# GrafikXxxxxxxYyyyyyyyyyy/StableDiffusion

Hardware: AMD Instinct MI355X
Metric: denoise-loop latents/s (512px, 50-step DDIM, batch 4) (higher is better)
Workload: dtype f16; 1 GPU; SD1.5 512x512, 50-step DDIM, batch 4/GPU, CFG on (UNet batch 8), UNet + VAE decode HIP kernels; global_batch=4, parallelism=dp1

## Files before the change

### include/sd_engine.h

```cpp
#ifndef SD_ENGINE_H
#define SD_ENGINE_H

#include <stdint.h>

#ifdef __cplusplus
extern "C" {
#endif

#define SD_OK 0
#define SD_ERR_INVALID 1
#define SD_ERR_STATE 2
#define SD_ERR_HIP 3
#define SD_ERR_UNSUPPORTED 4

#define SD_DTYPE_F16 0
#define SD_DTYPE_F32 1

#define SD_MAX_BLOCKS 4

typedef struct sd_unet_config {
    int32_t in_channels;
    int32_t out_channels;
    int32_t num_blocks;
    int32_t block_out_channels[SD_MAX_BLOCKS];
    int32_t down_block_has_attn[SD_MAX_BLOCKS];
    int32_t up_block_has_attn[SD_MAX_BLOCKS];
    int32_t num_heads[SD_MAX_BLOCKS];
    int32_t transformer_layers[SD_MAX_BLOCKS];
    int32_t layers_per_block;
    int32_t cross_attention_dim;
    int32_t use_linear_projection;
    int32_t norm_num_groups;
    float   norm_eps;
    int32_t flip_sin_to_cos;
    float   freq_shift;
    int32_t addition_time_embed_dim;
    int32_t projection_class_embeddings_input_dim;
} sd_unet_config;

typedef struct sd_vae_config {
    int32_t in_channels;
    int32_t out_channels;
    int32_t latent_channels;
    int32_t num_blocks;
    int32_t block_out_channels[SD_MAX_BLOCKS];
    int32_t layers_per_block;
    int32_t norm_num_groups;
} sd_vae_config;

typedef struct sd_clip_config {
    int32_t vocab_size;
    int32_t hidden_size;
    int32_t intermediate_size;
    int32_t num_layers;
    int32_t num_heads;
    int32_t max_positions;
    int32_t hidden_act;
    int32_t projection_dim;
    float layer_norm_eps;
} sd_clip_config;

typedef struct sd_unet sd_unet;
typedef struct sd_vae sd_vae;
typedef struct sd_clip sd_clip;
typedef struct sd_ip_adapter sd_ip_adapter;
typedef struct sd_controlnet sd_controlnet;

const char* sd_last_error(void);
int sd_engine_version(void);
const char* sd_engine_arch(void);

int sd_unet_create(const sd_unet_config* cfg, sd_unet** out);
int sd_unet_destroy(sd_unet* u);
int sd_unet_num_weights(const sd_unet* u);
int sd_unet_weight_info(const sd_unet* u, int index, const char** key, int64_t* shape4, int* ndim);
int sd_unet_set_weight(sd_unet* u, const char* diffusers_key, const void* data,
                       const int64_t* shape, int ndim, int dtype);
int sd_unet_finalize(sd_unet* u);
int sd_unet_forward(sd_unet* u, const void* sample, const float* timesteps, const void* ehs,
                    int ehs_len, const void* add_text, const float* add_time_ids, void* out,
                    int B, int H, int W, void* stream);
int sd_unet_use_graph(sd_unet* u, int enable);
int sd_unet_text_kv_cache(sd_unet* u, int enable);
int sd_unet_forward_ex(sd_unet* u, const void* sample, const float* timesteps, const void* ehs, int ehs_len,
                       const void* add_text, const float* add_time_ids, const void* image_embeds, int n_img, void* out,
                       int B, int H, int W, void* stream);
int sd_unet_set_ip_adapter(sd_unet* u, sd_ip_adapter* adapter);
int sd_unet_set_ip_adapter_scale(sd_unet* u, float scale);
int sd_unet_set_controlnet(sd_unet* u, sd_controlnet* cn);
int sd_unet_forward_cn(sd_unet* u, const void* sample, const float* timesteps, const void* ehs, int ehs_len,
                       const void* add_text, const float* add_time_ids, const void* image_embeds, int n_img,
                       const void* control_image, int n_ctrl, float cond_scale, void* out, int B, int H, int W,
                       void* stream);
int sd_unet_memory(const sd_unet* u, int64_t* weight_bytes, int64_t* workspace_bytes);

int sd_ip_adapter_create(const sd_unet* u, int image_embed_dim, int num_tokens, sd_ip_adapter** out);
int sd_ip_adapter_destroy(sd_ip_adapter* a);
int sd_ip_adapter_num_weights(const sd_ip_adapter* a);
int sd_ip_adapter_weight_info(const sd_ip_adapter* a, int index, const char** key, int64_t* shape4, int* ndim);
int sd_ip_adapter_set_weight(sd_ip_adapter* a, const char* key, const void* data, const int64_t* shape, int ndim,
                             int dtype);
int sd_ip_adapter_finalize(sd_ip_adapter* a);

int sd_controlnet_create(const sd_unet* u, const sd_unet_config* cn_cfg, int conditioning_channels, sd_controlnet** out);
int sd_controlnet_destroy(sd_controlnet* cn);
int sd_controlnet_num_weights(const sd_controlnet* cn);
int sd_controlnet_weight_info(const sd_controlnet* cn, int index, const char** key, int64_t* shape4, int* ndim);
int sd_controlnet_set_weight(sd_controlnet* cn, const char* key, const void* data, const int64_t* shape, int ndim,
                             int dtype);
int sd_controlnet_finalize(sd_controlnet* cn);

int sd_vae_create(const sd_vae_config* cfg, sd_vae** out);
int sd_vae_destroy(sd_vae* v);
int sd_vae_num_weights(const sd_vae* v);
int sd_vae_weight_info(const sd_vae* v, int index, const char** key, int64_t* shape4, int* ndim);
int sd_vae_set_weight(sd_vae* v, const char* diffusers_key, const void* data,
                      const int64_t* shape, int ndim, int dtype);
int sd_vae_finalize(sd_vae* v);
int sd_vae_decode(sd_vae* v, const void* z, void* img, int B, int h, int w, void* stream);
int sd_vae_encode(sd_vae* v, const void* img, void* moments, int B, int H, int W, void* stream);
int sd_vae_encode_range_shift(sd_vae* v, int shift);
int sd_vae_memory(const sd_vae* v, int64_t* weight_bytes, int64_t* workspace_bytes);

int sd_clip_create(const sd_clip_config* cfg, sd_clip** out);
int sd_clip_destroy(sd_clip* c);
int sd_clip_num_weights(const sd_clip* c);
int sd_clip_weight_info(const sd_clip* c, int index, const char** key, int64_t* shape4, int* ndim);
int sd_clip_set_weight(sd_clip* c, const char* key, const void* data, const int64_t* shape, int ndim, int dtype);
int sd_clip_finalize(sd_clip* c);
int sd_clip_forward(sd_clip* c, const int32_t* input_ids, const int32_t* eos_index, void* hidden_states,
                    void* last_hidden, void* pooled, void* text_embeds, int B, int T, void* stream);
int sd_clip_final_layer_norm(sd_clip* c, const void* x, void* y, int64_t rows, void* stream);
int sd_clip_memory(const sd_clip* c, int64_t* weight_bytes, int64_t* workspace_bytes);

int sd_cfg_duplicate(const void* latents, void* out2b, int64_t n_per_batch, int B, float in_scale,
                     void* stream);
int sd_cfg_ddim_step(const void* noise_pred_2b, void* latents, int64_t n, float guidance_scale,
                     float c_x, float c_eps, void* stream);

int sd_cfg_linear_step(const void* noise_pred_2b, void* latents, float* hist_f32, int64_t n,
                       float guidance_scale, float c_x, float c_eps, float c_hist, float h_x, float h_eps,
                       void* stream);

int sd_cfg_rescale_linear_step(const void* noise_pred_2b, void* latents, float* hist_f32, int B, int64_t n_per_sample,
                               float guidance_scale, float guidance_rescale, float c_x, float c_eps, float c_hist,
                               float h_x, float h_eps, float* factors_out, void* stream);

int sd_inpaint_blend(void* latents, const void* image_latents, const void* noise, const void* mask,
                     float a, float b, int B, int C, int H, int W, void* stream);

int sd_images_to_uint8(const void* images_nchw_f16, void* out_nhwc_u8, int B, int C, int H, int W, void* stream);

typedef struct sd_prof_entry {
    char kernel[64];
    double flops;
    double bytes;
    double ms;
    int64_t launches;
} sd_prof_entry;
int sd_prof_enable(int on);
int sd_prof_collect(sd_prof_entry* out, int max_entries, int* n_entries);

int sd_probe_mfma(int iters, float* tflops, void* stream);
int sd_probe_copy(int64_t bytes, int iters, float* gbs, void* stream);
int sd_probe_lds_dma(int64_t region_bytes, int passes, int depth, int shared, float* gbs, void* stream);

int sd_igemm_force(int variant, int splits);
int sd_igemm_plan(const int* geom, const int* flags, int64_t* out, char* name);

int sd_op_conv2d(const void* x_nhwc, const void* w_oihw, const void* bias, const void* rowadd,
                 const void* res_nhwc, void* y_nhwc, int N, int H, int W, int Cin, int Cout,
                 int ksize, int stride, int upsample2x, int geglu, void* stream);
int sd_op_conv3x3_small_cout(const void* x_nhwc, const void* w_oihw, const void* bias, void* y_nchw, int N, int H,
                             int W, int Cin, int Cout, void* stream);
int sd_op_conv2d_groupnorm(const void* x_nhwc, const void* w_oihw, const void* bias, const void* rowadd,
                           const void* res_nhwc, void* y_conv_nhwc, const void* gamma, const void* beta,
                           void* y_gn_nhwc, int N, int H, int W, int Cin, int Cout, int ksize, int stride,
                           int upsample2x, int groups, float eps, int silu, int* stats_from_epilogue, void* stream);
int sd_op_groupnorm_conv2d(const void* x_nhwc, const void* gamma, const void* beta, int groups, float eps, int silu,
                           const void* w_oihw, const void* bias, const void* rowadd, const void* res_nhwc, void* y_nhwc,
                           int N, int H, int W, int Cin, int Cout, int ksize, int iters, float* ms_per_launch, int* fused,
                           void* stream);
int sd_op_unet_conv_in(const void* x_nchw, const void* w_oihw, const void* bias, void* y_nhwc, float* gn_summaries, int groups,
                       int N, int Cin, int H, int W, int Cout, int iters, float* ms_per_launch, void* stream);
int sd_op_unet_conv_out(const void* x_nhwc, const void* gamma, const void* beta, int groups, float eps, int silu,
                        const void* w_oihw, const void* bias, void* y_nchw, int N, int H, int W, int C, int Cout, int iters,
                        float* ms_per_launch, void* stream);
int sd_op_ffn_geglu(const void* x, const void* ln_gamma, const void* ln_beta, float ln_eps, const void* w1, const void* b1,
                    const void* w2, const void* b2, void* y, int M, int C, int iters, float* ms_per_launch, int* fused,
                    void* stream);
int sd_op_linear_rowstats(const void* x, const void* w0, const void* b0, const void* res, void* y1, float* stat, int M,
                          int K, int C, int* parts, int* part_w, int* producer, void* stream);
int sd_op_ln_linear(const void* y1, const float* stat, int parts, int part_w, const void* gamma, const void* beta, float eps,
                    const void* w1, const void* b1, void* y2, int M, int C, int O, int geglu, int rows_scaled, float row_scale,
                    int* consumer, void* stream);
int sd_op_ln_ffn_geglu(const void* x, const float* stat, int parts, int part_w, const void* ln_gamma, const void* ln_beta,
                       float ln_eps, const void* w1, const void* b1, const void* w2, const void* b2, void* y, int M, int C,
                       int* fused, void* stream);
int sd_bench_conv2d(const void* x_nhwc, const void* w_oihw, void* y_nhwc, int N, int H, int W, int Cin,
                    int Cout, int ksize, int stride, int upsample2x, int geglu, int iters,
                    float* ms_per_launch, void* stream);
int sd_op_groupnorm(const void* x_nhwc, const void* gamma, const void* beta, void* y_nhwc,
                    int N, int HW, int C, int groups, float eps, int silu, void* stream);
int sd_op_groupnorm_concat(const void* x_nhwc, int Ca, int Cb, const void* gamma, const void* beta, void* y_nhwc, int N, int HW,
                           int groups, float eps, int silu, void* stream);
int sd_bench_groupnorm(const void* x_nhwc, const void* gamma, const void* beta, void* y_nhwc,
                       int N, int HW, int C, int groups, float eps, int silu, int iters,
                       float* ms_per_launch, void* stream);
int sd_op_timestep_sinusoid(const float* t, float* out, int count, int dim, int flip_sin_to_cos, float freq_shift,
                            void* stream);
int sd_op_small_linear(const float* x, const void* w_f16, const float* bias, float* y, int B, int K, int n_out,
                       int silu_in, int silu_out, void* stream);
int sd_op_layernorm(const void* x, const void* gamma, const void* beta, void* y, int rows, int C,
                    float eps, void* stream);
int sd_op_attention(const void* q, const void* k, const void* v, void* out, int B, int Tq, int Tk,
                    int heads, int d, int ldq, int ldk, int ldv, int ldo, void* stream);
int sd_op_attention_ex(const void* q, const void* k, const void* v, void* out, int B, int Tq, int Tk,
                       int heads, int d, int ldq, int ldk, int ldv, int ldo, int causal, int prescaled,
                       void* stream);
int sd_attention_plan(int B, int Tq, int Tk, int heads, int d, int causal, int prescaled, int* out5);
int sd_op_ip_cross_attention(const void* q, const void* k, const void* v, const void* k_ip, const void* v_ip, void* out,
                             int B, int Tq, int L, int T_ip, int heads, int d, int ldq, int ldk, int ldv, int ldk_ip,
                             int ldv_ip, int ldo, float ip_scale, int prescaled, int iters, float* ms_per_launch,
                             void* stream);

typedef struct sd_cn_problem {
    const void* x; int64_t ldx;
    const void* w;
    const float* bias;
    void* y; int64_t ldy;
    int M, C;
} sd_cn_problem;
int sd_op_controlnet_residuals(const sd_cn_problem* problems, int count, float scale, int mode, int iters,
                               float* ms_per_launch, void* stream);
int sd_op_controlnet_cond_embed(sd_controlnet* cn, const void* image, int n, int H, int W, void* out, int iters,
                                float* ms_per_launch, void* stream);

#ifdef __cplusplus
}
#endif
#endif
```

### stablediffusion_amd/_lib.py

```python
from __future__ import annotations

import ctypes as C
import os

_HERE = os.path.dirname(os.path.abspath(__file__))
LIB_PATH = os.path.join(_HERE, "libsd_engine.so")

SD_MAX_BLOCKS = 4
SD_DTYPE_F16 = 0
SD_DTYPE_F32 = 1


class SdUNetConfig(C.Structure):
    _fields_ = [
        ("in_channels", C.c_int32),
        ("out_channels", C.c_int32),
        ("num_blocks", C.c_int32),
        ("block_out_channels", C.c_int32 * SD_MAX_BLOCKS),
        ("down_block_has_attn", C.c_int32 * SD_MAX_BLOCKS),
        ("up_block_has_attn", C.c_int32 * SD_MAX_BLOCKS),
        ("num_heads", C.c_int32 * SD_MAX_BLOCKS),
        ("transformer_layers", C.c_int32 * SD_MAX_BLOCKS),
        ("layers_per_block", C.c_int32),
        ("cross_attention_dim", C.c_int32),
        ("use_linear_projection", C.c_int32),
        ("norm_num_groups", C.c_int32),
        ("norm_eps", C.c_float),
        ("flip_sin_to_cos", C.c_int32),
        ("freq_shift", C.c_float),
        ("addition_time_embed_dim", C.c_int32),
        ("projection_class_embeddings_input_dim", C.c_int32),
    ]


class SdVAEConfig(C.Structure):
    _fields_ = [
        ("in_channels", C.c_int32),
        ("out_channels", C.c_int32),
        ("latent_channels", C.c_int32),
        ("num_blocks", C.c_int32),
        ("block_out_channels", C.c_int32 * SD_MAX_BLOCKS),
        ("layers_per_block", C.c_int32),
        ("norm_num_groups", C.c_int32),
    ]


class SdClipConfig(C.Structure):
    _fields_ = [
        ("vocab_size", C.c_int32),
        ("hidden_size", C.c_int32),
        ("intermediate_size", C.c_int32),
        ("num_layers", C.c_int32),
        ("num_heads", C.c_int32),
        ("max_positions", C.c_int32),
        ("hidden_act", C.c_int32),
        ("projection_dim", C.c_int32),
        ("layer_norm_eps", C.c_float),
    ]


class SdProfEntry(C.Structure):
    _fields_ = [("kernel", C.c_char * 64), ("flops", C.c_double), ("bytes", C.c_double),
                ("ms", C.c_double), ("launches", C.c_int64)]


class SdCnProblem(C.Structure):
    _fields_ = [("x", C.c_void_p), ("ldx", C.c_int64), ("w", C.c_void_p), ("bias", C.c_void_p),
                ("y", C.c_void_p), ("ldy", C.c_int64), ("M", C.c_int), ("C", C.c_int)]


_P = C.c_void_p
_I = C.c_int
_I64 = C.c_int64
_F = C.c_float
SIGNATURES = {
    "sd_last_error": (C.c_char_p, []),
    "sd_engine_version": (_I, []),
    "sd_engine_arch": (C.c_char_p, []),
    "sd_unet_create": (_I, [C.POINTER(SdUNetConfig), C.POINTER(_P)]),
    "sd_unet_destroy": (_I, [_P]),
    "sd_unet_num_weights": (_I, [_P]),
    "sd_unet_weight_info": (_I, [_P, _I, C.POINTER(C.c_char_p), C.POINTER(_I64), C.POINTER(_I)]),
    "sd_unet_set_weight": (_I, [_P, C.c_char_p, _P, C.POINTER(_I64), _I, _I]),
    "sd_unet_finalize": (_I, [_P]),
    "sd_unet_forward": (_I, [_P, _P, _P, _P, _I, _P, _P, _P, _I, _I, _I, _P]),
    "sd_unet_use_graph": (_I, [_P, _I]),
    "sd_unet_text_kv_cache": (_I, [_P, _I]),
    "sd_unet_memory": (_I, [_P, C.POINTER(_I64), C.POINTER(_I64)]),
    "sd_unet_forward_ex": (_I, [_P, _P, _P, _P, _I, _P, _P, _P, _I, _P, _I, _I, _I, _P]),
    "sd_unet_set_ip_adapter": (_I, [_P, _P]),
    "sd_unet_set_ip_adapter_scale": (_I, [_P, _F]),
    "sd_ip_adapter_create": (_I, [_P, _I, _I, C.POINTER(_P)]),
    "sd_ip_adapter_destroy": (_I, [_P]),
    "sd_ip_adapter_num_weights": (_I, [_P]),
    "sd_ip_adapter_weight_info": (_I, [_P, _I, C.POINTER(C.c_char_p), C.POINTER(_I64), C.POINTER(_I)]),
    "sd_ip_adapter_set_weight": (_I, [_P, C.c_char_p, _P, C.POINTER(_I64), _I, _I]),
    "sd_ip_adapter_finalize": (_I, [_P]),
    "sd_unet_set_controlnet": (_I, [_P, _P]),
    "sd_unet_forward_cn": (_I, [_P, _P, _P, _P, _I, _P, _P, _P, _I, _P, _I, _F, _P, _I, _I, _I, _P]),
    "sd_controlnet_create": (_I, [_P, C.POINTER(SdUNetConfig), _I, C.POINTER(_P)]),
    "sd_controlnet_destroy": (_I, [_P]),
    "sd_controlnet_num_weights": (_I, [_P]),
    "sd_controlnet_weight_info": (_I, [_P, _I, C.POINTER(C.c_char_p), C.POINTER(_I64), C.POINTER(_I)]),
    "sd_controlnet_set_weight": (_I, [_P, C.c_char_p, _P, C.POINTER(_I64), _I, _I]),
    "sd_controlnet_finalize": (_I, [_P]),
    "sd_vae_create": (_I, [C.POINTER(SdVAEConfig), C.POINTER(_P)]),
    "sd_vae_destroy": (_I, [_P]),
    "sd_vae_num_weights": (_I, [_P]),
    "sd_vae_weight_info": (_I, [_P, _I, C.POINTER(C.c_char_p), C.POINTER(_I64), C.POINTER(_I)]),
    "sd_vae_set_weight": (_I, [_P, C.c_char_p, _P, C.POINTER(_I64), _I, _I]),
    "sd_vae_finalize": (_I, [_P]),
    "sd_vae_decode": (_I, [_P, _P, _P, _I, _I, _I, _P]),
    "sd_vae_encode": (_I, [_P, _P, _P, _I, _I, _I, _P]),
    "sd_vae_encode_range_shift": (_I, [_P, _I]),
    "sd_vae_memory": (_I, [_P, C.POINTER(_I64), C.POINTER(_I64)]),
    "sd_clip_create": (_I, [C.POINTER(SdClipConfig), C.POINTER(_P)]),
    "sd_clip_destroy": (_I, [_P]),
    "sd_clip_num_weights": (_I, [_P]),
    "sd_clip_weight_info": (_I, [_P, _I, C.POINTER(C.c_char_p), C.POINTER(_I64), C.POINTER(_I)]),
    "sd_clip_set_weight": (_I, [_P, C.c_char_p, _P, C.POINTER(_I64), _I, _I]),
    "sd_clip_finalize": (_I, [_P]),
    "sd_clip_forward": (_I, [_P, _P, _P, _P, _P, _P, _P, _I, _I, _P]),
    "sd_clip_final_layer_norm": (_I, [_P, _P, _P, _I64, _P]),
    "sd_clip_memory": (_I, [_P, C.POINTER(_I64), C.POINTER(_I64)]),
    "sd_op_attention_ex": (_I, [_P, _P, _P, _P, _I, _I, _I, _I, _I, _I, _I, _I, _I, _I, _I, _P]),
    "sd_cfg_duplicate": (_I, [_P, _P, _I64, _I, _F, _P]),
    "sd_cfg_ddim_step": (_I, [_P, _P, _I64, _F, _F, _F, _P]),
    "sd_inpaint_blend": (_I, [_P, _P, _P, _P, _F, _F, _I, _I, _I, _I, _P]),
    "sd_images_to_uint8": (_I, [_P, _P, _I, _I, _I, _I, _P]),
    "sd_cfg_linear_step": (_I, [_P, _P, _P, _I64, _F, _F, _F, _F, _F, _F, _P]),
    "sd_cfg_rescale_linear_step": (_I, [_P, _P, _P, _I, _I64, _F, _F, _F, _F, _F, _F, _F, _P, _P]),
    "sd_igemm_force": (_I, [_I, _I]),
    "sd_igemm_plan": (_I, [C.POINTER(_I), C.POINTER(_I), C.POINTER(_I64), C.c_char_p]),
    "sd_probe_mfma": (_I, [_I, C.POINTER(_F), _P]),
    "sd_probe_lds_dma": (_I, [_I64, _I, _I, _I, C.POINTER(_F), _P]),
    "sd_probe_copy": (_I, [_I64, _I, C.POINTER(_F), _P]),
    "sd_prof_enable": (_I, [_I]),
    "sd_prof_collect": (_I, [C.POINTER(SdProfEntry), _I, C.POINTER(_I)]),
    "sd_op_conv2d": (_I, [_P, _P, _P, _P, _P, _P, _I, _I, _I, _I, _I, _I, _I, _I, _I, _P]),
    "sd_op_conv3x3_small_cout": (_I, [_P, _P, _P, _P, _I, _I, _I, _I, _I, _P]),
    "sd_op_conv2d_groupnorm": (_I, [_P, _P, _P, _P, _P, _P, _P, _P, _P, _I, _I, _I, _I, _I, _I, _I, _I, _I, _F, _I,
                                    C.POINTER(_I), _P]),
    "sd_op_groupnorm_conv2d": (_I, [_P, _P, _P, _I, _F, _I, _P, _P, _P, _P, _P, _I, _I, _I, _I, _I, _I, _I, C.POINTER(_F),
                                    C.POINTER(_I), _P]),
    "sd_op_unet_conv_in": (_I, [_P, _P, _P, _P, _P, _I, _I, _I, _I, _I, _I, _I, C.POINTER(_F), _P]),
    "sd_op_unet_conv_out": (_I, [_P, _P, _P, _I, _F, _I, _P, _P, _P, _I, _I, _I, _I, _I, _I, C.POINTER(_F), _P]),
    "sd_op_ffn_geglu": (_I, [_P, _P, _P, _F, _P, _P, _P, _P, _P, _I, _I, _I, C.POINTER(_F), C.POINTER(_I), _P]),
    "sd_op_linear_rowstats": (_I, [_P, _P, _P, _P, _P, _P, _I, _I, _I, C.POINTER(_I), C.POINTER(_I), C.POINTER(_I), _P]),
    "sd_op_ln_linear": (_I, [_P, _P, _I, _I, _P, _P, _F, _P, _P, _P, _I, _I, _I, _I, _I, _F, C.POINTER(_I), _P]),
    "sd_op_ln_ffn_geglu": (_I, [_P, _P, _I, _I, _P, _P, _F, _P, _P, _P, _P, _P, _I, _I, C.POINTER(_I), _P]),
    "sd_bench_conv2d": (_I, [_P, _P, _P, _I, _I, _I, _I, _I, _I, _I, _I, _I, _I, C.POINTER(_F), _P]),
    "sd_op_groupnorm": (_I, [_P, _P, _P, _P, _I, _I, _I, _I, _F, _I, _P]),
    "sd_op_groupnorm_concat": (_I, [_P, _I, _I, _P, _P, _P, _I, _I, _I, _F, _I, _P]),
    "sd_bench_groupnorm": (_I, [_P, _P, _P, _P, _I, _I, _I, _I, _F, _I, _I, C.POINTER(_F), _P]),
    "sd_op_timestep_sinusoid": (_I, [_P, _P, _I, _I, _I, _F, _P]),
    "sd_op_small_linear": (_I, [_P, _P, _P, _P, _I, _I, _I, _I, _I, _P]),
    "sd_op_layernorm": (_I, [_P, _P, _P, _P, _I, _I, _F, _P]),
    "sd_op_attention": (_I, [_P, _P, _P, _P, _I, _I, _I, _I, _I, _I, _I, _I, _I, _P]),
    "sd_attention_plan": (_I, [_I, _I, _I, _I, _I, _I, _I, C.POINTER(_I)]),
    "sd_op_ip_cross_attention": (_I, [_P, _P, _P, _P, _P, _P, _I, _I, _I, _I, _I, _I, _I, _I, _I, _I, _I, _I, _F, _I, _I,
                                      C.POINTER(_F), _P]),
    "sd_op_controlnet_residuals": (_I, [C.POINTER(SdCnProblem), _I, _F, _I, _I, C.POINTER(_F), _P]),
    "sd_op_controlnet_cond_embed": (_I, [_P, _P, _I, _I, _I, _P, _I, C.POINTER(_F), _P]),
}

_lib = None


class EngineError(RuntimeError):
    pass


def load():
    global _lib
    if _lib is not None:
        return _lib
    if not os.path.exists(LIB_PATH):
        raise EngineError(
            f"{LIB_PATH} not found: build it with `python -m stablediffusion_amd.build` "
            "(hipcc --offload-arch=gfx950). The HIP engine is mandatory; there is no CPU fallback.")
    import torch
    lib = C.CDLL(LIB_PATH)
    for name, (res, args) in SIGNATURES.items():
        fn = getattr(lib, name)
        fn.restype = res
        fn.argtypes = args
    _lib = lib
    return lib


def check(rc: int, what: str = ""):
    if rc != 0:
        msg = load().sd_last_error()
        raise EngineError(f"{what}: error {rc}: {msg.decode() if msg else '?'}")


def require_gpu():
    import torch
    if not torch.cuda.is_available():
        raise EngineError("no HIP device visible: the gfx950 engine cannot run (and nothing else will run in its place)")
```

### stablediffusion_amd/csrc/capi.cpp

```cpp
#include <cstdio>
#include <new>

#include "model.h"
#include <cstdlib>

using namespace sd;

struct sd_unet { UNet impl; explicit sd_unet(const sd_unet_config& c) : impl(c) {} };
struct sd_vae { VAE impl; explicit sd_vae(const sd_vae_config& c) : impl(c) {} };
struct sd_clip { CLIP impl; explicit sd_clip(const sd_clip_config& c) : impl(c) {} };
struct sd_controlnet {
    ControlNet impl;
    sd_controlnet(const sd_unet_config& c, int cc) : impl(c, cc) {}
};
struct sd_ip_adapter {
    IPAdapter impl;
    sd_ip_adapter(const sd_unet_config& c, int d, int n) : impl(c, d, n) {}
    ~sd_ip_adapter() { if (impl.attached) impl.attached->set_ip_adapter(nullptr); }
};

namespace {

int weight_info(const WeightStore& ws, int index, const char** key, int64_t* shape4, int* ndim) {
    if (index < 0 || index >= (int)ws.order.size()) { set_error("weight index out of range"); return SD_ERR_INVALID; }
// ... 2 lines not shown
    *key = k.c_str();
    *ndim = (int)t.shape.size();
    for (int i = 0; i < 4; ++i) shape4[i] = i < *ndim ? t.shape[(size_t)i] : 1;
    return SD_OK;
}

bool bad_cfg(const sd_unet_config* c) {
    if (!c || c->num_blocks < 1 || c->num_blocks > SD_MAX_BLOCKS) return true;
    for (int i = 0; i < c->num_blocks; ++i) {
        if (c->block_out_channels[i] % 64 != 0 || c->block_out_channels[i] % c->norm_num_groups != 0) return true;
        if (c->num_heads[i] <= 0 || c->block_out_channels[i] % c->num_heads[i] != 0) return true;
        if ((c->down_block_has_attn[i] || c->up_block_has_attn[c->num_blocks - 1 - i]) &&
            !attention_supported(c->block_out_channels[i] / c->num_heads[i])) return true;
    }
    if (c->addition_time_embed_dim > 0) {
        const int ad = c->addition_time_embed_dim, pin = c->projection_class_embeddings_input_dim;
        if ((ad & 1) || pin % 64 != 0 || pin - 6 * ad <= 0) return true;
    }
    return c->cross_attention_dim % 64 != 0 || c->in_channels <= 0 || c->in_channels > 16;
}

bool same_topology(const sd_unet_config& a, const sd_unet_config& b) {
    if (a.in_channels != b.in_channels || a.out_channels != b.out_channels || a.num_blocks != b.num_blocks ||
        a.layers_per_block != b.layers_per_block || a.cross_attention_dim != b.cross_attention_dim ||
        a.use_linear_projection != b.use_linear_projection || a.norm_num_groups != b.norm_num_groups ||
        a.norm_eps != b.norm_eps || a.flip_sin_to_cos != b.flip_sin_to_cos || a.freq_shift != b.freq_shift ||
        a.addition_time_embed_dim != b.addition_time_embed_dim ||
        a.projection_class_embeddings_input_dim != b.projection_class_embeddings_input_dim)
        return false;
    for (int i = 0; i < SD_MAX_BLOCKS; ++i)
        if (a.block_out_channels[i] != b.block_out_channels[i] || a.down_block_has_attn[i] != b.down_block_has_attn[i] ||
            a.up_block_has_attn[i] != b.up_block_has_attn[i] || a.num_heads[i] != b.num_heads[i] ||
            a.transformer_layers[i] != b.transformer_layers[i])
            return false;
    return true;
}

bool controlnet_fits(const sd_unet_config& u, const sd_unet_config& n, std::string* why) {
    if (n.num_blocks != u.num_blocks || n.layers_per_block != u.layers_per_block) {
        *why = "num_blocks / layers_per_block differ from the UNet's";
        return false;
    }
    for (int i = 0; i < u.num_blocks; ++i)
        if (n.block_out_channels[i] != u.block_out_channels[i]) { *why = "block_out_channels differ from the UNet's"; return false; }
    if (n.cross_attention_dim != u.cross_attention_dim) { *why = "cross_attention_dim differs from the UNet's"; return false; }
    if (n.in_channels != u.in_channels) { *why = "in_channels differs from the UNet's (9-channel inpaint UNets take no ControlNet)"; return false; }
    if (n.addition_time_embed_dim != u.addition_time_embed_dim ||
        n.projection_class_embeddings_input_dim != u.projection_class_embeddings_input_dim) {
        *why = "text_time conditioning differs from the UNet's";
        return false;
    }
    return true;
}

}

extern "C" {

const char* sd_last_error(void) { return sd::last_error().c_str(); }
int sd_engine_version(void) { return 1; }
const char* sd_engine_arch(void) { return "gfx950"; }

int sd_unet_create(const sd_unet_config* cfg, sd_unet** out) {
    if (!out) { set_error("null out"); return SD_ERR_INVALID; }
    if (bad_cfg(cfg)) {
        set_error("sd_unet_create: unsupported config (channels must be multiples of 64 and of the group "
                  "count, head dims in {32,40,64,80,128,160}, cross_attention_dim % 64 == 0, text_time: even "
                  "addition_time_embed_dim and projection_class_embeddings_input_dim % 64 == 0 and > 6 x it)");
        return SD_ERR_UNSUPPORTED;
    }
    *out = new (std::nothrow) sd_unet(*cfg);
    if (!*out) { set_error("out of host memory"); return SD_ERR_INVALID; }
    return SD_OK;
}
int sd_unet_destroy(sd_unet* u) { delete u; return SD_OK; }
int sd_unet_num_weights(const sd_unet* u) { return u ? (int)u->impl.ws.order.size() : 0; }
int sd_unet_weight_info(const sd_unet* u, int index, const char** key, int64_t* shape4, int* ndim) {
    if (!u) { set_error("null handle"); return SD_ERR_INVALID; }
    return weight_info(u->impl.ws, index, key, shape4, ndim);
}
int sd_unet_set_weight(sd_unet* u, const char* key, const void* data, const int64_t* shape, int ndim, int dtype) {
    if (!u || !key || !data || !shape) { set_error("null argument"); return SD_ERR_INVALID; }
    if (u->impl.finalized) { set_error("set_weight after finalize"); return SD_ERR_STATE; }
    return u->impl.ws.set(key, data, shape, ndim, dtype);
}
int sd_unet_finalize(sd_unet* u) {
    if (!u) { set_error("null handle"); return SD_ERR_INVALID; }
    return u->impl.finalize();
}
int sd_unet_forward(sd_unet* u, const void* sample, const float* timesteps, const void* ehs, int ehs_len,
                    const void* add_text, const float* add_time_ids, void* out, int B, int H, int W,
                    void* stream) {
    if (!u || !sample || !timesteps || !ehs || !out) { set_error("null argument"); return SD_ERR_INVALID; }
    return u->impl.forward(static_cast<const half_t*>(sample), timesteps, static_cast<const half_t*>(ehs),
                           ehs_len, static_cast<const half_t*>(add_text), add_time_ids,
                           static_cast<half_t*>(out), B, H, W, static_cast<hipStream_t>(stream));
}
int sd_unet_use_graph(sd_unet* u, int enable) {
    if (!u) { set_error("null handle"); return SD_ERR_INVALID; }
    u->impl.graph_enabled = enable != 0;
    return SD_OK;
}
int sd_unet_text_kv_cache(sd_unet* u, int enable) {
    if (!u) { set_error("null handle"); return SD_ERR_INVALID; }
    u->impl.kv_cache_on = enable != 0;
    u->impl.kv_valid = false;
    u->impl.ipkv_valid = false;
    u->impl.cond_valid = false;
    u->impl.cnkv_valid = false;
    return SD_OK;
}
int sd_unet_forward_ex(sd_unet* u, const void* sample, const float* timesteps, const void* ehs, int ehs_len,
                       const void* add_text, const float* add_time_ids, const void* image_embeds, int n_img, void* out,
                       int B, int H, int W, void* stream) {
    if (!u || !sample || !timesteps || !ehs || !out) { set_error("null argument"); return SD_ERR_INVALID; }
    return u->impl.forward(static_cast<const half_t*>(sample), timesteps, static_cast<const half_t*>(ehs),
                           ehs_len, static_cast<const half_t*>(add_text), add_time_ids,
                           static_cast<half_t*>(out), B, H, W, static_cast<hipStream_t>(stream),
                           static_cast<const half_t*>(image_embeds), image_embeds ? n_img : 0);
}
int sd_unet_set_ip_adapter(sd_unet* u, sd_ip_adapter* a) {
    if (!u) { set_error("null handle"); return SD_ERR_INVALID; }
    if (a) {
        if (!a->impl.finalized) { set_error("sd_unet_set_ip_adapter: adapter not finalized"); return SD_ERR_STATE; }
        if (!same_topology(a->impl.cfg, u->impl.cfg)) {
            set_error("sd_unet_set_ip_adapter: the adapter was created for another UNet configuration");
            return SD_ERR_INVALID;
        }
    }
    u->impl.set_ip_adapter(a ? &a->impl : nullptr);
    return SD_OK;
}
int sd_unet_set_controlnet(sd_unet* u, sd_controlnet* cn) {
    if (!u) { set_error("null handle"); return SD_ERR_INVALID; }
    if (cn) {
        if (!cn->impl.finalized) { set_error("sd_unet_set_controlnet: ControlNet not finalized"); return SD_ERR_STATE; }
        std::string why;
        if (!controlnet_fits(u->impl.cfg, cn->impl.cfg, &why)) { set_error("sd_unet_set_controlnet: " + why); return SD_ERR_INVALID; }
    }
    u->impl.set_controlnet(cn ? &cn->impl : nullptr);
    return SD_OK;
}
int sd_unet_forward_cn(sd_unet* u, const void* sample, const float* timesteps, const void* ehs, int ehs_len,
                       const void* add_text, const float* add_time_ids, const void* image_embeds, int n_img,
                       const void* control_image, int n_ctrl, float cond_scale, void* out, int B, int H, int W,
                       void* stream) {
    if (!u || !sample || !timesteps || !ehs || !out) { set_error("null argument"); return SD_ERR_INVALID; }
    return u->impl.forward(static_cast<const half_t*>(sample), timesteps, static_cast<const half_t*>(ehs),
                           ehs_len, static_cast<const half_t*>(add_text), add_time_ids,
                           static_cast<half_t*>(out), B, H, W, static_cast<hipStream_t>(stream),
                           static_cast<const half_t*>(image_embeds), image_embeds ? n_img : 0,
                           static_cast<const half_t*>(control_image), control_image ? n_ctrl : 0, cond_scale);
}
int sd_unet_set_ip_adapter_scale(sd_unet* u, float scale) {
    if (!u) { set_error("null handle"); return SD_ERR_INVALID; }
    if (!(scale == scale)) { set_error("sd_unet_set_ip_adapter_scale: NaN"); return SD_ERR_INVALID; }
    u->impl.ip_scale = scale;
    return SD_OK;
}

int sd_ip_adapter_create(const sd_unet* u, int image_embed_dim, int num_tokens, sd_ip_adapter** out) {
    if (!u || !out) { set_error("null argument"); return SD_ERR_INVALID; }
    const sd_unet_config& c = u->impl.cfg;
    if (c.cross_attention_dim % 64 != 0) { set_error("sd_ip_adapter_create: cross_attention_dim % 64 != 0"); return SD_ERR_UNSUPPORTED; }
    if (num_tokens < 1 || num_tokens > 16) { set_error("sd_ip_adapter_create: num_tokens must be in [1, 16]"); return SD_ERR_UNSUPPORTED; }
    if (image_embed_dim <= 0 || image_embed_dim % 64 != 0) {
        set_error("sd_ip_adapter_create: image_embed_dim must be a positive multiple of 64");
        return SD_ERR_UNSUPPORTED;
    }
    for (const auto& site : unet_xattn_sites(c, true)) {
        int heads = 0;
        for (int i = 0; i < c.num_blocks; ++i)
            if (c.block_out_channels[i] == site.second) heads = c.num_heads[i];
        if (heads <= 0 || !ip_attention_supported(site.second / heads)) {
            set_error("sd_ip_adapter_create: head dim of " + site.first + " not in {32, 40, 64, 80, 160}");
            return SD_ERR_UNSUPPORTED;
        }
    }
    *out = new (std::nothrow) sd_ip_adapter(c, image_embed_dim, num_tokens);
    if (!*out) { set_error("out of host memory"); return SD_ERR_INVALID; }
    return SD_OK;
}
int sd_ip_adapter_destroy(sd_ip_adapter* a) { delete a; return SD_OK; }
int sd_ip_adapter_num_weights(const sd_ip_adapter* a) { return a ? (int)a->impl.ws.order.size() : 0; }
int sd_ip_adapter_weight_info(const sd_ip_adapter* a, int index, const char** key, int64_t* shape4, int* ndim) {
    if (!a) { set_error("null handle"); return SD_ERR_INVALID; }
    return weight_info(a->impl.ws, index, key, shape4, ndim);
}
int sd_ip_adapter_set_weight(sd_ip_adapter* a, const char* key, const void* data, const int64_t* shape, int ndim,
                             int dtype) {
    if (!a || !key || !data || !shape) { set_error("null argument"); return SD_ERR_INVALID; }
    if (a->impl.finalized) { set_error("set_weight after finalize"); return SD_ERR_STATE; }
    return a->impl.ws.set(key, data, shape, ndim, dtype);
}
int sd_ip_adapter_finalize(sd_ip_adapter* a) {
    if (!a) { set_error("null handle"); return SD_ERR_INVALID; }
    return a->impl.finalize();
}
int sd_controlnet_create(const sd_unet* u, const sd_unet_config* cn_cfg, int conditioning_channels, sd_controlnet** out) {
    if (!u || !cn_cfg || !out) { set_error("null argument"); return SD_ERR_INVALID; }
    if (conditioning_channels != 3) { set_error("sd_controlnet_create: conditioning_channels must be 3"); return SD_ERR_UNSUPPORTED; }
    sd_unet_config c = *cn_cfg;
    for (int i = 0; i < SD_MAX_BLOCKS; ++i) c.up_block_has_attn[i] = 0;
    if (bad_cfg(&c)) { set_error("sd_controlnet_create: unsupported encoder configuration"); return SD_ERR_UNSUPPORTED; }
    std::string why;
    if (!controlnet_fits(u->impl.cfg, c, &why)) { set_error("sd_controlnet_create: " + why); return SD_ERR_INVALID; }
    if (u->impl.cfg.in_channels != 4) { set_error("sd_controlnet_create: the UNet must take 4 latent channels"); return SD_ERR_INVALID; }
    if (1 + c.num_blocks * c.layers_per_block + (c.num_blocks - 1) + 1 > kCnMaxProblems) {
        set_error("sd_controlnet_create: more residual sites than one grouped launch takes (16)");
        return SD_ERR_UNSUPPORTED;
    }
    *out = new (std::nothrow) sd_controlnet(c, conditioning_channels);
    if (!*out) { set_error("out of host memory"); return SD_ERR_INVALID; }
    return SD_OK;
}
int sd_controlnet_destroy(sd_controlnet* cn) { delete cn; return SD_OK; }
int sd_controlnet_num_weights(const sd_controlnet* cn) { return cn ? (int)cn->impl.ws.order.size() : 0; }
int sd_controlnet_weight_info(const sd_controlnet* cn, int index, const char** key, int64_t* shape4, int* ndim) {
    if (!cn) { set_error("null handle"); return SD_ERR_INVALID; }
    return weight_info(cn->impl.ws, index, key, shape4, ndim);
}
int sd_controlnet_set_weight(sd_controlnet* cn, const char* key, const void* data, const int64_t* shape, int ndim,
                             int dtype) {
    if (!cn || !key || !data || !shape) { set_error("null argument"); return SD_ERR_INVALID; }
    if (cn->impl.finalized) { set_error("set_weight after finalize"); return SD_ERR_STATE; }
    return cn->impl.ws.set(key, data, shape, ndim, dtype);
}
int sd_controlnet_finalize(sd_controlnet* cn) {
    if (!cn) { set_error("null handle"); return SD_ERR_INVALID; }
    return cn->impl.finalize();
}
int sd_unet_memory(const sd_unet* u, int64_t* weight_bytes, int64_t* workspace_bytes) {
    if (!u) { set_error("null handle"); return SD_ERR_INVALID; }
    if (weight_bytes) *weight_bytes = u->impl.ws.packed_bytes();
    if (workspace_bytes) *workspace_bytes = (int64_t)u->impl.arena.capacity();
    return SD_OK;
}

int sd_vae_create(const sd_vae_config* cfg, sd_vae** out) {
    if (!out || !cfg) { set_error("null argument"); return SD_ERR_INVALID; }
    bool bad = cfg->num_blocks < 1 || cfg->num_blocks > SD_MAX_BLOCKS || cfg->latent_channels > 8;
    for (int i = 0; !bad && i < cfg->num_blocks; ++i)
        bad = cfg->block_out_channels[i] % 64 != 0;
    if (!bad) bad = !attention_supported(cfg->block_out_channels[cfg->num_blocks - 1]);
    if (bad) { set_error("sd_vae_create: unsupported config"); return SD_ERR_UNSUPPORTED; }
    *out = new (std::nothrow) sd_vae(*cfg);
    if (!*out) { set_error("out of host memory"); return SD_ERR_INVALID; }
    return SD_OK;
}
int sd_vae_destroy(sd_vae* v) { delete v; return SD_OK; }
int sd_vae_num_weights(const sd_vae* v) { return v ? (int)v->impl.ws.order.size() : 0; }
int sd_vae_weight_info(const sd_vae* v, int index, const char** key, int64_t* shape4, int* ndim) {
    if (!v) { set_error("null handle"); return SD_ERR_INVALID; }
    return weight_info(v->impl.ws, index, key, shape4, ndim);
}
int sd_vae_set_weight(sd_vae* v, const char* key, const void* data, const int64_t* shape, int ndim, int dtype) {
    if (!v || !key || !data || !shape) { set_error("null argument"); return SD_ERR_INVALID; }
    if (v->impl.finalized) { set_error("set_weight after finalize"); return SD_ERR_STATE; }
    return v->impl.ws.set(key, data, shape, ndim, dtype);
}
int sd_vae_finalize(sd_vae* v) {
    if (!v) { set_error("null handle"); return SD_ERR_INVALID; }
    return v->impl.finalize();
}
int sd_vae_decode(sd_vae* v, const void* z, void* img, int B, int h, int w, void* stream) {
    if (!v || !z || !img) { set_error("null argument"); return SD_ERR_INVALID; }
    return v->impl.decode(static_cast<const half_t*>(z), static_cast<half_t*>(img), B, h, w,
                          static_cast<hipStream_t>(stream));
}
int sd_vae_encode(sd_vae* v, const void* img, void* moments, int B, int H, int W, void* stream) {
    if (!v || !img || !moments) { set_error("null argument"); return SD_ERR_INVALID; }
    return v->impl.encode(static_cast<const half_t*>(img), static_cast<half_t*>(moments), B, H, W,
                          static_cast<hipStream_t>(stream));
}
int sd_vae_encode_range_shift(sd_vae* v, int shift) {
    if (!v || shift < 0 || shift > 14) { set_error("sd_vae_encode_range_shift: shift in 0..14"); return SD_ERR_INVALID; }
    v->impl.encode_shift = shift;
    return SD_OK;
}
int sd_vae_memory(const sd_vae* v, int64_t* weight_bytes, int64_t* workspace_bytes) {
    if (!v) { set_error("null handle"); return SD_ERR_INVALID; }
    if (weight_bytes) *weight_bytes = v->impl.ws.packed_bytes();
    if (workspace_bytes) *workspace_bytes = (int64_t)v->impl.arena.capacity();
    return SD_OK;
}

int sd_clip_create(const sd_clip_config* cfg, sd_clip** out) {
    if (!out || !cfg) { set_error("null argument"); return SD_ERR_INVALID; }
    const bool bad = cfg->vocab_size < 1 || cfg->num_layers < 1 || cfg->num_heads < 1 || cfg->max_positions < 1 ||
                     cfg->hidden_size % 64 != 0 || cfg->intermediate_size % 64 != 0 || cfg->hidden_size > 2048 ||
                     cfg->hidden_size % cfg->num_heads != 0 || !attention_supported(cfg->hidden_size / cfg->num_heads) ||
                     (cfg->hidden_act != 0 && cfg->hidden_act != 1) || cfg->projection_dim < 0;
    if (bad) { set_error("sd_clip_create: unsupported config (hidden / intermediate % 64, head dim, activation)"); return SD_ERR_UNSUPPORTED; }
    *out = new (std::nothrow) sd_clip(*cfg);
    if (!*out) { set_error("out of host memory"); return SD_ERR_INVALID; }
    return SD_OK;
}
int sd_clip_destroy(sd_clip* c) { delete c; return SD_OK; }
int sd_clip_num_weights(const sd_clip* c) { return c ? (int)c->impl.ws.order.size() : 0; }
int sd_clip_weight_info(const sd_clip* c, int index, const char** key, int64_t* shape4, int* ndim) {
    if (!c) { set_error("null handle"); return SD_ERR_INVALID; }
    return weight_info(c->impl.ws, index, key, shape4, ndim);
}
int sd_clip_set_weight(sd_clip* c, const char* key, const void* data, const int64_t* shape, int ndim, int dtype) {
    if (!c || !key || !data || !shape) { set_error("null argument"); return SD_ERR_INVALID; }
    if (c->impl.finalized) { set_error("set_weight after finalize"); return SD_ERR_STATE; }
// ... 911 lines not shown
```

### stablediffusion_amd/csrc/kernels.h

```cpp
#pragma once
#include "common.h"

namespace sd {

struct IGemmParams {
    const half_t* x; long ldx;
    const half_t* w;
    const float* bias;
    const float* rowadd; int rowadd_ld;
    const half_t* res; long ldres;
    half_t* y; long ldy;
    int N, H, W, Cin;
    int OH, OW, Cout;
    int KS, stride, pad, up;
    int M, K;
    int geglu;
    int mfast = 0;
    int act = 0;
    float* rowstat_out = nullptr;
    int rowstat_parts = 0;
    const float* ln_stat = nullptr;
    int ln_parts = 0, ln_C = 0, ln_part_w = 0;
    float ln_eps = 0.f;
    const float* ln_wsum = nullptr;
// ... 8 lines not shown
    const float* gni_gb = nullptr;
    int dbg_unchecked = 0;
    float acc_scale = 1.f, bias_scale = 1.f;
};
bool igemm2_gn_fusable(const IGemmParams& p, int groups);
int launch_igemm(const IGemmParams& p, hipStream_t s);
const char* igemm_variant(const IGemmParams& p);
bool igemm2_supported(const IGemmParams& p);
void igemm2_force(int variant, int splits);
struct IGemmRequest {
    float* rowstat = nullptr;
    float* gnstat = nullptr;
    int gn_groups = 0;
    bool no_workspace = false;
};
constexpr int kKindPgemmGeglu = 100;
constexpr int kKindIgemm1 = -1;
constexpr int kKindBadVariant = -2;
struct IGemmPlan {
    int kind = kKindIgemm1;
    int variant = -1;
    int splits = 1;
    long partial_floats = 0;
    int bm = 0, bn = 0;
    bool rowstats = false;
    int rs_parts = 1, rs_part_w = 0;
    bool gnstats = false;
    int gn_rows = 0;
    bool scales_ok = false;
    char name[64] = "";
};
IGemmPlan igemm2_plan(IGemmParams& p, const IGemmRequest& rq = IGemmRequest());
int launch_igemm2(const IGemmParams& p, float* partial, hipStream_t s, const IGemmPlan* plan = nullptr);
bool igemm3_supported(const IGemmParams& p);
int launch_igemm3(const IGemmParams& p, int mfast, hipStream_t s);
constexpr int kWeightRowPad = 256;
bool wsgemm_supported(const IGemmParams& p);
int wsgemm_rowstat_parts(const IGemmParams& p);
int launch_wsgemm(const IGemmParams& p, hipStream_t s);
bool pgemm_geglu_supported(const IGemmParams& p);
int launch_pgemm_geglu(const IGemmParams& p, hipStream_t s);

struct FfnParams {
    const half_t* x; long ldx;
    half_t* y; long ldy;
    const half_t* w1; const float* b1; const float* wsum1; int w1_rows;
    const half_t* w2; const float* b2; int w2_rows;
    const float* ln_stat; int ln_parts; float ln_eps;
    int M, C, hidden;
    int ln_part_w;
};
bool ffn_fused_supported(const FfnParams& p);
int launch_ffn_fused(const FfnParams& p, hipStream_t s);

long gn_scratch_floats(int N, long HW, int C, int G);
struct GnStats {
    const float* part = nullptr;
    int S = 0;
    long rows = 0;
};
bool gn_wants_stats(long HW, int C, int G);
int launch_groupnorm(const half_t* x, long ldx, const float* gamma, const float* beta,
                     half_t* y, long ldy, int N, long HW, int C, int G, float eps, int silu,
                     float* scratch, hipStream_t s, const GnStats* pre = nullptr);
int launch_gn_stats(const half_t* x, long ldx, int N, long HW, int C, int G, float* scratch, GnStats* st, hipStream_t s);
int launch_gn_finalize(GnStats* st, float* out, int N, long HW, int C, int G, hipStream_t s);
int gn_cat_unit(int Ca, int Cb, int G);
int launch_gn_cat_finalize(const GnStats& sa, int Ga, int Ca, const GnStats& sb, int Gb, int Cb, float* out, int N, long HW, int G,
                           hipStream_t s);
int launch_layernorm(const half_t* x, long ldx, const float* gamma, const float* beta,
                     half_t* y, long ldy, long rows, int C, float eps, hipStream_t s);
int launch_row_stats(const half_t* x, long ldx, float* stat, long rows, int C, hipStream_t s);
int launch_ln_fold(half_t* w, long K, int rows, const float* gamma, const float* beta, const float* bias_in,
                   float* bias, float* wsum, int rows_scaled, float row_scale, hipStream_t s);

int launch_attention(const half_t* q, const half_t* k, const half_t* v, half_t* out,
                     int B, int Tq, int Tk, int heads, int d,
                     long ldq, long ldk, long ldv, long ldo, hipStream_t s, int causal = 0, int prescaled = 0);
bool attention_supported(int d);
struct AttnPlan { int D, QT, KT, PRESC, NWV; };
AttnPlan attention_plan(int B, int Tq, int Tk, int heads, int d, int causal, int prescaled);
int launch_ip_attention(const half_t* q, const half_t* k, const half_t* v, const half_t* kip, const half_t* vip,
                        half_t* out, int B, int Tq, int L, int Tip, int heads, int d, long ldq, long ldk, long ldv,
                        long ldki, long ldvi, long ldo, float ip_scale, int prescaled, hipStream_t s);
bool ip_attention_supported(int d);
int launch_axpy_f16(half_t* y, long ldy, const half_t* x, long ldx, long rows, int cols, float a, hipStream_t s);

constexpr int kCnMaxProblems = 16;
struct CnResProblem {
    const half_t* x = nullptr; long ldx = 0;
    const half_t* w = nullptr;
    const float* bias = nullptr;
    half_t* y = nullptr; long ldy = 0;
    int M = 0, C = 0;
    int first = 0;
};
struct CnResParams {
    CnResProblem p[kCnMaxProblems];
    int count = 0, total = 0;
    float scale = 1.f;
};
int cn_residual_tiles(int M, int C);
bool cn_residual_supported(const CnResParams& p);
int launch_cn_residual(const CnResParams& p, hipStream_t s);
struct CnCondConvParams {
    const half_t* x = nullptr; int nchw = 0;
    const float* w = nullptr; const float* bias = nullptr;
    half_t* y = nullptr;
    int N = 0, IH = 0, IW = 0, Cin = 0, OH = 0, OW = 0, Cout = 0, stride = 1, silu = 1;
};
bool cn_cond_conv_supported(const CnCondConvParams& p);
int launch_cn_cond_conv(const CnCondConvParams& p, hipStream_t s);
int launch_cn_pack_cond(const half_t* w_oihw, float* out, int O, int I, hipStream_t s);

int launch_timestep_sinusoid(const float* t, int t_stride, float* out, int count, int dim, int flip, float shift,
                             long out_ld, hipStream_t s);
int launch_small_linear(const float* x, long ldx, const half_t* w, const float* bias, float* y,
                        long ldy, int B, int K, int Nout, int silu_in, int silu_out, hipStream_t s);
int launch_add_f32(float* y, const float* x, long n, int silu, hipStream_t s);
int launch_f16_to_f32(const half_t* x, float* y, long n, hipStream_t s);
int launch_f32_to_f16(const float* x, half_t* y, long n, hipStream_t s);
int launch_im2col_nchw3x3(const half_t* x, half_t* col, int N, int C, int H, int W, int Kpad,
                          hipStream_t s);
int launch_nhwc_to_nchw(const half_t* x, long ldx, half_t* y, int N, long HW, int C, hipStream_t s);
int launch_nchw_to_nhwc(const half_t* x, half_t* y, long ldy, int N, long HW, int C, hipStream_t s);
int launch_pointwise_nchw(const half_t* x, const half_t* w, const float* bias, half_t* y, int N,
                          int Cin, int Cout, long HW, hipStream_t s);
constexpr long kSmallCoutMinPixels = 131072;
int launch_conv3x3_small_cout(const half_t* x, long ldx, const half_t* w, long K, const float* bias, half_t* y_nchw,
                              int N, int H, int W, int Cin, int Cout, hipStream_t s);
struct HeadParams {
    const half_t* x_nchw = nullptr;
    const half_t* w = nullptr; long K = 0;
    const float* bias = nullptr;
    half_t* y = nullptr; long ldy = 0;
    float* gnstat_out = nullptr; int G = 0;
    int N = 0, Cin = 0, H = 0, W = 0, Cout = 0;
};
bool conv_head_supported(const HeadParams& p);
int launch_conv_head(const HeadParams& p, hipStream_t s);
struct TailParams {
    const half_t* x = nullptr; long ldx = 0;
    const float* gn_part = nullptr; int gn_S = 0; long gn_rows = 0;
    int G = 0; float eps = 0.f; const float* gamma = nullptr; const float* beta = nullptr; int silu = 0;
    const half_t* w = nullptr; long K = 0; const float* bias = nullptr;
    half_t* y = nullptr;
    int N = 0, H = 0, W = 0, C = 0, Cout = 0;
};
bool conv_tail_supported(const TailParams& p);
int launch_conv_tail(const TailParams& p, hipStream_t s);
int launch_pack_conv(const half_t* w_oihw, half_t* wp, int O, int I, int KH, int KW, long Kpad,
                     hipStream_t s);
int launch_cfg_duplicate(const half_t* lat, half_t* out, long n_total, float scale, hipStream_t s);
int launch_clip_embed(const int* ids, const half_t* tok, const half_t* pos, half_t* out, int B, int T, int H, int vocab,
                      hipStream_t s);
int launch_gather_rows(const half_t* x, long ldx, const int* idx, half_t* out16, float* out32, int B, int T, int H,
                       hipStream_t s);
int launch_inpaint_blend(half_t* lat, const half_t* img, const half_t* noise, const half_t* mask, float a, float b, int B,
                         int C, long HW, hipStream_t s);
int launch_scale_f16(half_t* x, long n, float scale, hipStream_t s);
int launch_image_to_uint8(const half_t* img, unsigned char* out, int B, int C, long HW, hipStream_t s);
int launch_cfg_linear(const half_t* eps2b, half_t* lat, float* hist, long n, float g, float cx, float ce, float ch,
                      float hx, float he, hipStream_t s);
int launch_cfg_ddim(const half_t* eps2b, half_t* lat, long n, float g, float cx, float ce,
                    hipStream_t s);
int launch_cfg_rescale_linear(const half_t* eps2b, half_t* lat, float* hist, int B, long n, float g, float phi, float cx,
                              float ce, float ch, float hx, float he, float* factors, hipStream_t s);

int probe_mfma(int iters, float* tflops, hipStream_t s);
int probe_copy(long bytes, int iters, float* gbs, hipStream_t s);
int probe_dma(long region_bytes, int passes, int depth, int shared, float* gbs, hipStream_t s);

}
```

### stablediffusion_amd/csrc/misc.hip

```cpp
#include <cstdint>
#include <cstdlib>
#include <map>
#include <mutex>
#include <utility>

#include "kernels.h"

namespace sd {
namespace {

__global__ void sinusoid_kernel(const float* __restrict__ t, int t_stride, float* __restrict__ out, int count,
                                int dim, int flip, float shift, long out_ld) {
    const int half = dim >> 1;
    const int i = blockIdx.x * blockDim.x + threadIdx.x;
    if (i >= count * half) return;
    const int b = i / half, f = i - b * half;
    const float freq = __expf(-9.210340371976184f * (float)f / ((float)half - shift));
    const float ang = t[(long)b * t_stride] * freq;
    float sn, cs;
    sincosf(ang, &sn, &cs);
    float* o = out + (long)b * out_ld;
    if (flip) { o[f] = cs; o[half + f] = sn; } else { o[f] = sn; o[half + f] = cs; }
}

// ... 4 lines not shown
                                                           const float* __restrict__ bias,
                                                           float* __restrict__ y, long ldy, int B,
                                                           int K, int Nout, int silu_in, int silu_out) {
    const int lane = threadIdx.x & 63;
    const int n0 = (blockIdx.x * 4 + (threadIdx.x >> 6)) * SL_COLS;
    if (n0 >= Nout) return;
    for (int b0 = 0; b0 < B; b0 += SL_MAXB) {
        float acc[SL_COLS][SL_MAXB];
#pragma unroll
        for (int c = 0; c < SL_COLS; ++c)
#pragma unroll
            for (int b = 0; b < SL_MAXB; ++b) acc[c][b] = 0.f;
        for (int k0 = lane * 8; k0 < K; k0 += 64 * 8) {
            h8 wv[SL_COLS];
#pragma unroll
            for (int c = 0; c < SL_COLS; ++c) {
                const int n = n0 + c < Nout ? n0 + c : Nout - 1;
                wv[c] = *reinterpret_cast<const h8*>(w + (long)n * K + k0);
            }
#pragma unroll
            for (int b = 0; b < SL_MAXB; ++b) {
                if (b0 + b < B) {
                    const float* xr = x + (long)(b0 + b) * ldx + k0;
                    const f4 x0 = *reinterpret_cast<const f4*>(xr);
                    const f4 x1 = *reinterpret_cast<const f4*>(xr + 4);
                    float a[8];
#pragma unroll
                    for (int e = 0; e < 4; ++e) {
                        a[e] = silu_in ? silu_f(x0[e]) : x0[e];
                        a[e + 4] = silu_in ? silu_f(x1[e]) : x1[e];
                    }
#pragma unroll
                    for (int c = 0; c < SL_COLS; ++c)
#pragma unroll
                        for (int e = 0; e < 8; ++e) acc[c][b] += a[e] * (float)wv[c][e];
                }
            }
        }
#pragma unroll
        for (int c = 0; c < SL_COLS; ++c)
#pragma unroll
            for (int b = 0; b < SL_MAXB; ++b) {
                float a = acc[c][b];
#pragma unroll
                for (int off = 32; off > 0; off >>= 1) a += __shfl_xor(a, off);
                if (lane == 0 && b0 + b < B && n0 + c < Nout) {
                    a += bias ? bias[n0 + c] : 0.f;
                    if (silu_out) a = silu_f(a);
                    y[(long)(b0 + b) * ldy + n0 + c] = a;
                }
            }
    }
}

__global__ void add_f32_kernel(float* y, const float* x, long n, int silu) {
    const long i = (long)blockIdx.x * blockDim.x + threadIdx.x;
    if (i < n) {
        float v = y[i] + (x ? x[i] : 0.f);
        y[i] = silu ? silu_f(v) : v;
    }
}
__global__ void f16_to_f32_kernel(const half_t* x, float* y, long n) {
    const long i = (long)blockIdx.x * blockDim.x + threadIdx.x;
    if (i < n) y[i] = (float)x[i];
}
__global__ void f32_to_f16_kernel(const float* x, half_t* y, long n) {
    const long i = (long)blockIdx.x * blockDim.x + threadIdx.x;
    if (i < n) y[i] = (half_t)x[i];
}

__global__ void im2col_nchw3x3_kernel(const half_t* __restrict__ x, half_t* __restrict__ col, int N,
                                      int C, int H, int W, int Kpad) {
    const long i = (long)blockIdx.x * blockDim.x + threadIdx.x;
    const long total = (long)N * H * W * Kpad;
    if (i >= total) return;
    const int kq = (int)(i % Kpad);
    const long m = i / Kpad;
    half_t val = (half_t)0.f;
    if (kq < 9 * C) {
        const int tap = kq / C, c = kq - tap * C;
        const int kh = tap / 3, kw = tap - kh * 3;
        const int w_ = (int)(m % W);
        const int h_ = (int)((m / W) % H);
        const int n = (int)(m / ((long)W * H));
        const int ih = h_ + kh - 1, iw = w_ + kw - 1;
        if (ih >= 0 && ih < H && iw >= 0 && iw < W) val = x[(((long)n * C + c) * H + ih) * W + iw];
    }
    col[i] = val;
}

__global__ void nhwc_to_nchw_kernel(const half_t* __restrict__ x, long ldx, half_t* __restrict__ y,
                                    int N, long HW, int C) {
    const long i = (long)blockIdx.x * blockDim.x + threadIdx.x;
    if (i >= (long)N * C * HW) return;
    const long pix = i % HW;
    const int c = (int)((i / HW) % C);
    const long n = i / (HW * C);
    y[i] = x[(n * HW + pix) * ldx + c];
}

__global__ void nchw_to_nhwc_kernel(const half_t* __restrict__ x, half_t* __restrict__ y, long ldy,
                                    int N, long HW, int C) {
    const long i = (long)blockIdx.x * blockDim.x + threadIdx.x;
    if (i >= (long)N * C * HW) return;
    const int c = (int)(i % C);
    const long pix = (i / C) % HW;
    const long n = i / (HW * C);
    y[(n * HW + pix) * ldy + c] = x[(n * C + c) * HW + pix];
}

__global__ void pointwise_nchw_kernel(const half_t* __restrict__ x, const half_t* __restrict__ w,
                                      const float* __restrict__ bias, half_t* __restrict__ y, int N,
                                      int Cin, int Cout, long HW) {
    const long i = (long)blockIdx.x * blockDim.x + threadIdx.x;
    if (i >= (long)N * Cout * HW) return;
    const long pix = i % HW;
    const int co = (int)((i / HW) % Cout);
    const long n = i / (HW * Cout);
    float acc = bias ? bias[co] : 0.f;
    for (int ci = 0; ci < Cin; ++ci)
        acc += (float)x[(n * Cin + ci) * HW + pix] * (float)w[co * Cin + ci];
    y[i] = (half_t)acc;
}

__global__ void pack_conv_kernel(const half_t* __restrict__ w, half_t* __restrict__ wp, int O, int I,
                                 int KH, int KW, long Kpad) {
    const long i = (long)blockIdx.x * blockDim.x + threadIdx.x;
    if (i >= (long)O * Kpad) return;
    const long kq = i % Kpad;
    const long o = i / Kpad;
    half_t val = (half_t)0.f;
    if (kq < (long)KH * KW * I) {
        int ci, tap;
        if (I % 64 == 0) {
            const int slab = (int)(kq >> 6), cl = (int)(kq & 63);
            const int cs = slab / (KH * KW);
            tap = slab - cs * (KH * KW);
            ci = cs * 64 + cl;
        } else {
            ci = (int)(kq % I);
            tap = (int)(kq / I);
        }
        const int kh = tap / KW, kw = tap - kh * KW;
        val = w[((o * I + ci) * KH + kh) * KW + kw];
    }
    wp[i] = val;
}

__global__ void cfg_duplicate_kernel(const half_t* __restrict__ lat, half_t* __restrict__ out, long n,
                                     float scale) {
    const long i = (long)blockIdx.x * blockDim.x + threadIdx.x;
    if (i >= n) return;
    const half_t v = (half_t)((float)lat[i] * scale);
    out[i] = v;
    out[n + i] = v;
}
__global__ void cfg_ddim_kernel(const half_t* __restrict__ eps2b, half_t* __restrict__ lat, long n,
                                float g, float cx, float ce) {
    const long i = (long)blockIdx.x * blockDim.x + threadIdx.x;
    if (i >= n) return;
    const float eu = (float)eps2b[i], et = (float)eps2b[n + i];
    const float e = (float)(half_t)(g * (et - eu) + eu);
    lat[i] = (half_t)(cx * (float)lat[i] + ce * e);
}

__global__ void cfg_linear_kernel(const half_t* __restrict__ eps2b, half_t* __restrict__ lat,
                                  float* __restrict__ hist, long n, float g, float cx, float ce, float ch,
                                  float hx, float he) {
    const long i = (long)blockIdx.x * blockDim.x + threadIdx.x;
    if (i >= n) return;
    const float eu = (float)eps2b[i], et = (float)eps2b[n + i];
    const float e = (float)(half_t)(g * (et - eu) + eu);
    const float x = (float)lat[i];
    float out = cx * x + ce * e;
    if (hist) {
        out += ch * hist[i];
        hist[i] = hx * x + he * e;
    }
    lat[i] = (half_t)out;
}

constexpr int RS_MAX_PARTS = 64;
constexpr int RS_MIN_CHUNK = 2048;

struct RsStat { float n, mean, m2; };

__device__ __forceinline__ RsStat rs_merge(const RsStat a, const RsStat b) {
    RsStat r;
    r.n = a.n + b.n;
    const float d = b.mean - a.mean;
    const float w = r.n > 0.f ? b.n / r.n : 0.f;
    r.mean = a.mean + d * w;
    r.m2 = a.m2 + b.m2 + d * d * a.n * w;
    return r;
}
__device__ __forceinline__ RsStat rs_wave_merge(RsStat s) {
#pragma unroll
    for (int off = 1; off < 64; off <<= 1) {
        RsStat o;
        o.n = __shfl_xor(s.n, off);
        o.mean = __shfl_xor(s.mean, off);
        o.m2 = __shfl_xor(s.m2, off);
        s = (threadIdx.x & off) ? rs_merge(o, s) : rs_merge(s, o);
    }
    return s;
}
__device__ __forceinline__ float rs_cfg(float eu, float et, float g) { return (float)(half_t)(g * (et - eu) + eu); }
__device__ __forceinline__ float rs_axpby(float a, float x, float b, float e) { return __builtin_fmaf(a, x, b * e); }

template <bool VEC>
__global__ __launch_bounds__(256) void rs_stats_kernel(const half_t* __restrict__ eps2b, RsStat* __restrict__ part, long n,
                                                       long chunk, long total, float g) {
    const int b = blockIdx.y, p = blockIdx.x;
    const half_t* u = eps2b + (long)b * n;
    const half_t* t = u + total;
    const long lo = (long)p * chunk, hi = lo + chunk < n ? lo + chunk : n;
    RsStat st = {0.f, 0.f, 0.f}, se = {0.f, 0.f, 0.f};
    if (VEC) {
        for (long i = lo + (long)threadIdx.x * 8; i < hi; i += 256 * 8) {
            const h8 vu = *reinterpret_cast<const h8*>(u + i);
            const h8 vt = *reinterpret_cast<const h8*>(t + i);
            float ft[8], fe[8], sumt = 0.f, sume = 0.f;
#pragma unroll
            for (int k = 0; k < 8; ++k) {
                ft[k] = (float)vt[k];
                fe[k] = rs_cfg((float)vu[k], ft[k], g);
                sumt += ft[k];
                sume += fe[k];
            }
            RsStat vt8 = {8.f, sumt * 0.125f, 0.f}, ve8 = {8.f, sume * 0.125f, 0.f};
#pragma unroll
            for (int k = 0; k < 8; ++k) {
                const float dt = ft[k] - vt8.mean, de = fe[k] - ve8.mean;
                vt8.m2 += dt * dt;
                ve8.m2 += de * de;
            }
            st = rs_merge(st, vt8);
            se = rs_merge(se, ve8);
        }
    } else {
        for (long i = lo + threadIdx.x; i < hi; i += 256) {
            const float ft = (float)t[i];
            const RsStat a = {1.f, ft, 0.f}, c = {1.f, rs_cfg((float)u[i], ft, g), 0.f};
            st = rs_merge(st, a);
            se = rs_merge(se, c);
        }
    }
    st = rs_wave_merge(st);
    se = rs_wave_merge(se);
    __shared__ RsStat sh[4][2];
    const int wave = threadIdx.x >> 6;
    if ((threadIdx.x & 63) == 0) { sh[wave][0] = st; sh[wave][1] = se; }
    __syncthreads();
    if (threadIdx.x == 0) {
        RsStat* o = part + ((long)b * gridDim.x + p) * 2;
        o[0] = rs_merge(rs_merge(sh[0][0], sh[1][0]), rs_merge(sh[2][0], sh[3][0]));
        o[1] = rs_merge(rs_merge(sh[0][1], sh[1][1]), rs_merge(sh[2][1], sh[3][1]));
    }
}

template <bool VEC>
__global__ __launch_bounds__(256) void rs_apply_kernel(const half_t* __restrict__ eps2b, half_t* __restrict__ lat,
                                                       float* __restrict__ hist, const RsStat* __restrict__ part, int parts,
                                                       long n, long total, float g, float phi, float cx, float ce, float ch,
                                                       float hx, float he, float* __restrict__ factors) {
    const int b = blockIdx.y, lane = threadIdx.x & 63;
    RsStat st = {0.f, 0.f, 0.f}, se = {0.f, 0.f, 0.f};
    if (lane < parts) {
        const RsStat* q = part + ((long)b * parts + lane) * 2;
        st = q[0];
        se = q[1];
    }
    st = rs_wave_merge(st);
    se = rs_wave_merge(se);
    const float k = 1.f + phi * (sqrtf(st.m2 / se.m2) - 1.f);
    if (factors && blockIdx.x == 0 && threadIdx.x == 0) factors[b] = k;
    const long base = (long)b * n;
    const half_t* u = eps2b + base;
    const half_t* t = u + total;
    half_t* x = lat + base;
    float* h = hist ? hist + base : nullptr;
    if (VEC) {
        const long i = ((long)blockIdx.x * 256 + threadIdx.x) * 8;
        if (i >= n) return;
        const h8 vu = *reinterpret_cast<const h8*>(u + i);
        const h8 vt = *reinterpret_cast<const h8*>(t + i);
        const h8 vx = *reinterpret_cast<const h8*>(x + i);
        float hv[8], x0[8];
        if (h) {
            const f4 h0 = *reinterpret_cast<const f4*>(h + i), h1 = *reinterpret_cast<const f4*>(h + i + 4);
#pragma unroll
            for (int j = 0; j < 4; ++j) { hv[j] = h0[j]; hv[j + 4] = h1[j]; }
        }
        h8 o;
#pragma unroll
        for (int j = 0; j < 8; ++j) {
            const float e = k * rs_cfg((float)vu[j], (float)vt[j], g);
            const float xf = (float)vx[j];
            float out = rs_axpby(cx, xf, ce, e);
            if (h) {
                out = __builtin_fmaf(ch, hv[j], out);
                x0[j] = rs_axpby(hx, xf, he, e);
            }
            o[j] = (half_t)out;
        }
        *reinterpret_cast<h8*>(x + i) = o;
// ... 181 lines not shown
}

inline dim3 grid1d(long n, int block = 256) { return dim3((unsigned)((n + block - 1) / block)); }

}

int launch_timestep_sinusoid(const float* t, int t_stride, float* out, int count, int dim, int flip, float shift,
                             long out_ld, hipStream_t s) {
    hipLaunchKernelGGL(sinusoid_kernel, grid1d((long)count * (dim / 2)), dim3(256), 0, s, t, t_stride, out, count,
                       dim, flip, shift, out_ld);
    SD_HIP_CHECK(hipGetLastError());
    return 0;
}

constexpr int SK_MAXKS = 10;
__global__ __launch_bounds__(256) void skinny_linear_kernel(const float* __restrict__ x, long ldx, const half_t* __restrict__ w,
                                                            const float* __restrict__ bias, float* __restrict__ y, long ldy,
                                                            int B, int K, int Nout, int silu_in, int silu_out) {
    __shared__ float red[2][4][256];
    const int tid = threadIdx.x, lane = tid & 63, wave = tid >> 6;
    const int fr = lane & 15, fq = lane >> 4;
    const int KS = K / 32;
    const int tiles = Nout / 16;
    h8 xh[SK_MAXKS], xl[SK_MAXKS];
#pragma unroll
    for (int j = 0; j < SK_MAXKS; ++j) {
        const int ks = wave + 4 * j;
        h8 hi = {0, 0, 0, 0, 0, 0, 0, 0}, lo = {0, 0, 0, 0, 0, 0, 0, 0};
        if (ks < KS && fr < B) {
            const float* xr = x + (long)fr * ldx + ks * 32 + fq * 8;
            const f4 a = *reinterpret_cast<const f4*>(xr), b = *reinterpret_cast<const f4*>(xr + 4);
#pragma unroll
            for (int e = 0; e < 8; ++e) {
                float v = e < 4 ? a[e] : b[e - 4];
                if (silu_in) v = silu_f(v);
                hi[e] = (half_t)v;
                lo[e] = (half_t)(v - (float)hi[e]);
            }
        }
        xh[j] = hi; xl[j] = lo;
    }
    auto fetch = [&](int t, h8* wf) {
        const int tt = t < tiles ? t : tiles - 1;
        const half_t* wr = w + ((long)tt * 16 + fr) * K + fq * 8;
#pragma unroll
        for (int j = 0; j < SK_MAXKS; ++j) {
            const int ks = wave + 4 * j;
            wf[j] = *reinterpret_cast<const h8*>(wr + (ks < KS ? ks : KS - 1) * 32);
        }
    };
    h8 wcur[SK_MAXKS], wnext[SK_MAXKS];
    int t = blockIdx.x;
    fetch(t, wcur);
    int par = 0;
    for (; t < tiles; t += gridDim.x, par ^= 1) {
        fetch(t + gridDim.x, wnext);
        f4 acc = {0.f, 0.f, 0.f, 0.f};
#pragma unroll
        for (int j = 0; j < SK_MAXKS; ++j) {
            if (wave + 4 * j < KS) {
                acc = __builtin_amdgcn_mfma_f32_16x16x32_f16(wcur[j], xh[j], acc, 0, 0, 0);
                acc = __builtin_amdgcn_mfma_f32_16x16x32_f16(wcur[j], xl[j], acc, 0, 0, 0);
            }
        }
#pragma unroll
        for (int e = 0; e < 4; ++e) red[par][wave][(fq * 4 + e) * 16 + fr] = acc[e];
        __syncthreads();
        {
            const int col = tid >> 4, row = tid & 15;
            if (row < B) {
                float v = red[par][0][tid] + red[par][1][tid] + red[par][2][tid] + red[par][3][tid];
                v += bias ? bias[t * 16 + col] : 0.f;
                if (silu_out) v = silu_f(v);
                y[(long)row * ldy + t * 16 + col] = v;
            }
        }
#pragma unroll
        for (int j = 0; j < SK_MAXKS; ++j) wcur[j] = wnext[j];
    }
}

int launch_small_linear(const float* x, long ldx, const half_t* w, const float* bias, float* y, long ldy,
                        int B, int K, int Nout, int silu_in, int silu_out, hipStream_t s) {
    if (K % 8 != 0 || ldx % 4 != 0) { set_error("small_linear: K%8, ldx%4"); return 1; }
    static const bool no_skinny = getenv("SD_NO_SKINNY_LINEAR") != nullptr;
    if (!no_skinny && B <= 16 && K % 32 == 0 && K <= 4 * SK_MAXKS * 32 && Nout % 16 == 0) {
        const int tiles = Nout / 16;
        hipLaunchKernelGGL(skinny_linear_kernel, dim3(tiles < 512 ? tiles : 512), dim3(256), 0, s, x, ldx, w, bias, y, ldy, B, K, Nout,
                           silu_in, silu_out);
        SD_HIP_CHECK(hipGetLastError());
        return 0;
    }
    hipLaunchKernelGGL(small_linear_kernel, dim3(cdiv(Nout, 4 * SL_COLS)), dim3(256), 0, s, x, ldx, w, bias, y, ldy, B, K,
                       Nout, silu_in, silu_out);
    SD_HIP_CHECK(hipGetLastError());
    return 0;
}

int launch_add_f32(float* y, const float* x, long n, int silu, hipStream_t s) {
    hipLaunchKernelGGL(add_f32_kernel, grid1d(n), dim3(256), 0, s, y, x, n, silu);
    SD_HIP_CHECK(hipGetLastError());
    return 0;
}
int launch_f16_to_f32(const half_t* x, float* y, long n, hipStream_t s) {
    hipLaunchKernelGGL(f16_to_f32_kernel, grid1d(n), dim3(256), 0, s, x, y, n);
    SD_HIP_CHECK(hipGetLastError());
    return 0;
}
int launch_f32_to_f16(const float* x, half_t* y, long n, hipStream_t s) {
    hipLaunchKernelGGL(f32_to_f16_kernel, grid1d(n), dim3(256), 0, s, x, y, n);
    SD_HIP_CHECK(hipGetLastError());
    return 0;
}
int launch_im2col_nchw3x3(const half_t* x, half_t* col, int N, int C, int H, int W, int Kpad, hipStream_t s) {
    hipLaunchKernelGGL(im2col_nchw3x3_kernel, grid1d((long)N * H * W * Kpad), dim3(256), 0, s, x, col, N, C, H,
                       W, Kpad);
    SD_HIP_CHECK(hipGetLastError());
    return 0;
}
int launch_nhwc_to_nchw(const half_t* x, long ldx, half_t* y, int N, long HW, int C, hipStream_t s) {
    hipLaunchKernelGGL(nhwc_to_nchw_kernel, grid1d((long)N * C * HW), dim3(256), 0, s, x, ldx, y, N, HW, C);
    SD_HIP_CHECK(hipGetLastError());
    return 0;
}
int launch_nchw_to_nhwc(const half_t* x, half_t* y, long ldy, int N, long HW, int C, hipStream_t s) {
    hipLaunchKernelGGL(nchw_to_nhwc_kernel, grid1d((long)N * C * HW), dim3(256), 0, s, x, y, ldy, N, HW, C);
    SD_HIP_CHECK(hipGetLastError());
    return 0;
}
int launch_pointwise_nchw(const half_t* x, const half_t* w, const float* bias, half_t* y, int N, int Cin,
                          int Cout, long HW, hipStream_t s) {
    hipLaunchKernelGGL(pointwise_nchw_kernel, grid1d((long)N * Cout * HW), dim3(256), 0, s, x, w, bias, y, N,
                       Cin, Cout, HW);
    SD_HIP_CHECK(hipGetLastError());
    return 0;
}
int launch_conv3x3_small_cout(const half_t* x, long ldx, const half_t* w, long K, const float* bias, half_t* y_nchw,
                              int N, int H, int W, int Cin, int Cout, hipStream_t s) {
    if (Cout < 1 || Cout > 4 || Cin % 64 != 0 || K != 9L * Cin) { set_error("conv3x3_small_cout: Cout in 1..4, Cin % 64 == 0"); return 1; }
    const long tiles = (long)N * ((H + CO_TH - 1) / CO_TH) * ((W + CO_TW - 1) / CO_TW);
    if (tiles == 0) return 0;
    hipLaunchKernelGGL(conv3x3_small_cout_kernel<4>, dim3((unsigned)tiles), dim3(256), 0, s, x, ldx, w, K, bias, y_nchw, N, H, W,
                       Cin, Cout);
    SD_HIP_CHECK(hipGetLastError());
    return 0;
}
int launch_pack_conv(const half_t* w, half_t* wp, int O, int I, int KH, int KW, long Kpad, hipStream_t s) {
    hipLaunchKernelGGL(pack_conv_kernel, grid1d((long)O * Kpad), dim3(256), 0, s, w, wp, O, I, KH, KW, Kpad);
    SD_HIP_CHECK(hipGetLastError());
    return 0;
}
int launch_cfg_duplicate(const half_t* lat, half_t* out, long n, float scale, hipStream_t s) {
    hipLaunchKernelGGL(cfg_duplicate_kernel, grid1d(n), dim3(256), 0, s, lat, out, n, scale);
    SD_HIP_CHECK(hipGetLastError());
    return 0;
}
int launch_cfg_ddim(const half_t* eps2b, half_t* lat, long n, float g, float cx, float ce, hipStream_t s) {
    hipLaunchKernelGGL(cfg_ddim_kernel, grid1d(n), dim3(256), 0, s, eps2b, lat, n, g, cx, ce);
    SD_HIP_CHECK(hipGetLastError());
    return 0;
}
int launch_cfg_linear(const half_t* eps2b, half_t* lat, float* hist, long n, float g, float cx, float ce, float ch,
                      float hx, float he, hipStream_t s) {
    hipLaunchKernelGGL(cfg_linear_kernel, grid1d(n), dim3(256), 0, s, eps2b, lat, hist, n, g, cx, ce, ch, hx, he);
    SD_HIP_CHECK(hipGetLastError());
    return 0;
}
static RsStat* rs_workspace(int B, hipStream_t s) {
    struct Buf { RsStat* p = nullptr; int B = 0; };
    static std::mutex mu;
    static std::map<std::pair<int, hipStream_t>, Buf> bufs;
    int dev = 0;
    if (hipGetDevice(&dev) != hipSuccess) return nullptr;
    std::lock_guard<std::mutex> lock(mu);
    Buf& b = bufs[{dev, s}];
    if (b.B < B) {
        if (b.p) (void)hipFree(b.p);
        b.p = nullptr;
        b.B = 0;
        if (hipMalloc(reinterpret_cast<void**>(&b.p), (size_t)B * RS_MAX_PARTS * 2 * sizeof(RsStat)) != hipSuccess) {
            b.p = nullptr;
            return nullptr;
        }
        b.B = B;
    }
    return b.p;
}
int launch_cfg_rescale_linear(const half_t* eps2b, half_t* lat, float* hist, int B, long n, float g, float phi, float cx,
                              float ce, float ch, float hx, float he, float* factors, hipStream_t s) {
    RsStat* part = rs_workspace(B, s);
    if (!part) { set_error("cfg_rescale_linear: no device memory for the chunk summaries"); return 1; }
    const long total = (long)B * n;
    const bool vec = n % 8 == 0 && ((reinterpret_cast<uintptr_t>(eps2b) | reinterpret_cast<uintptr_t>(lat) |
                                     reinterpret_cast<uintptr_t>(hist)) & 15) == 0;
    long parts = (n + RS_MIN_CHUNK - 1) / RS_MIN_CHUNK;
    if (parts > RS_MAX_PARTS) parts = RS_MAX_PARTS;
    long chunk = (n + parts - 1) / parts;
    chunk = (chunk + 7) / 8 * 8;
    parts = (n + chunk - 1) / chunk;
    const long per_block = vec ? 256 * 8 : 256;
    const long blocks = (n + per_block - 1) / per_block;
    if (blocks > 0x7fffffffL) { set_error("cfg_rescale_linear: sample too large"); return 1; }
    const dim3 gs((unsigned)parts, (unsigned)B), ga((unsigned)blocks, (unsigned)B);
    if (vec) {
        hipLaunchKernelGGL(rs_stats_kernel<true>, gs, dim3(256), 0, s, eps2b, part, n, chunk, total, g);
        hipLaunchKernelGGL(rs_apply_kernel<true>, ga, dim3(256), 0, s, eps2b, lat, hist, part, (int)parts, n, total, g, phi, cx,
                           ce, ch, hx, he, factors);
    } else {
        hipLaunchKernelGGL(rs_stats_kernel<false>, gs, dim3(256), 0, s, eps2b, part, n, chunk, total, g);
        hipLaunchKernelGGL(rs_apply_kernel<false>, ga, dim3(256), 0, s, eps2b, lat, hist, part, (int)parts, n, total, g, phi, cx,
                           ce, ch, hx, he, factors);
    }
    SD_HIP_CHECK(hipGetLastError());
    return 0;
}
int launch_clip_embed(const int* ids, const half_t* tok, const half_t* pos, half_t* out, int B, int T, int H, int vocab,
                      hipStream_t s) {
    if (H % 8 != 0) { set_error("clip_embed: hidden size must be a multiple of 8"); return 1; }
    const long n = (long)B * T * (H / 8);
    hipLaunchKernelGGL(clip_embed_kernel, grid1d(n), dim3(256), 0, s, ids, tok, pos, out, (long)B * T, T, H / 8, vocab);
    SD_HIP_CHECK(hipGetLastError());
    return 0;
}
int launch_gather_rows(const half_t* x, long ldx, const int* idx, half_t* out16, float* out32, int B, int T, int H,
                       hipStream_t s) {
    hipLaunchKernelGGL(gather_rows_kernel, grid1d((long)B * H), dim3(256), 0, s, x, ldx, idx, out16, out32, B, T, H);
    SD_HIP_CHECK(hipGetLastError());
    return 0;
}
int launch_inpaint_blend(half_t* lat, const half_t* img, const half_t* noise, const half_t* mask, float a, float b, int B,
                         int C, long HW, hipStream_t s) {
    const long n = (long)B * C * HW;
    if (n == 0) return 0;
    hipLaunchKernelGGL(inpaint_blend_kernel, grid1d(n), dim3(256), 0, s, lat, img, noise, mask, a, b, C, HW, n);
    SD_HIP_CHECK(hipGetLastError());
    return 0;
}
int launch_ln_fold(half_t* w, long K, int rows, const float* gamma, const float* beta, const float* bias_in,
                   float* bias, float* wsum, int rows_scaled, float row_scale, hipStream_t s) {
    if (rows <= 0) return 0;
    hipLaunchKernelGGL(ln_fold_kernel, dim3((rows + 3) / 4), dim3(256), 0, s, w, K, rows, gamma, beta, bias_in, bias, wsum,
                       rows_scaled, row_scale);
    SD_HIP_CHECK(hipGetLastError());
    return 0;
}
int launch_scale_f16(half_t* x, long n, float scale, hipStream_t s) {
    if (n <= 0) return 0;
    hipLaunchKernelGGL(scale_f16_kernel, grid1d(n), dim3(256), 0, s, x, n, scale);
    SD_HIP_CHECK(hipGetLastError());
    return 0;
}
int launch_image_to_uint8(const half_t* img, unsigned char* out, int B, int C, long HW, hipStream_t s) {
    const long total = (long)B * HW;
    if (total == 0) return 0;
    hipLaunchKernelGGL(image_to_uint8_kernel, grid1d(total), dim3(256), 0, s, img, out, C, HW, total);
    SD_HIP_CHECK(hipGetLastError());
    return 0;
}

}
```

### stablediffusion_amd/csrc/model.h

```cpp
#pragma once
#include "../../include/sd_engine.h"
#include "engine.h"

#include <functional>

namespace sd {

const std::string& last_error();

struct Resnet {
    NormW n1, n2;
    ConvW c1, c2, sc;
    bool has_sc = false;
    int temb_off = -1;
    int cin = 0, cout = 0;
};
struct TBlock {
    NormW ln1, ln2, ln3;
    ConvW qkv, out1, q2, out2, ff1, ff2;
    int kv_off = 0;
    int ip_kv_off = 0;
    bool fold = false;
};
struct Xformer {
    NormW gn;
    ConvW pin, pout;
    std::vector<TBlock> blocks;
    int C = 0, heads = 1;
};
struct VaeAttn {
    NormW gn;
    ConvW qkv, out;
    int C = 0;
};

void run_resnet(Ctx& c, const Resnet& r, View x, int N, int H, int W, View out, int G, float eps,
                const float* tproj, int tproj_ld, const GnStatBuf* x_stats = nullptr, GnStatBuf** out_stats = nullptr,
                float stream_scale = 1.f, GnStatBuf* out_buf = nullptr, int out_groups = 0);
void run_xformer(Ctx& c, const Xformer& t, View x, int N, int H, int W, View out, int G, View text_kv, int L,
                 const GnStatBuf* x_stats = nullptr, GnStatBuf** out_stats = nullptr, GnStatBuf* out_buf = nullptr,
                 int out_groups = 0);

struct UNet;

std::vector<std::pair<std::string, int>> unet_xattn_sites(const sd_unet_config& cfg, bool mid_last);

struct IPAdapter {
    IPAdapter(const sd_unet_config& c, int image_embed_dim, int num_tokens);
    int finalize();

    sd_unet_config cfg;
    int d_img = 0, n_tok = 0;
    WeightStore ws;
    bool finalized = false;
    ConvW proj;
    NormW norm;
    ConvW kv_all;
    int kv_total = 0;
    UNet* attached = nullptr;
};

struct Encoder {
    explicit Encoder(const sd_unet_config& c) : cfg(c) {}

    sd_unet_config cfg;
    WeightStore ws;
    ConvW conv_in, te1, te2, ae1, ae2, temb_stack;
    ConvW kv_all;
    std::vector<std::string> kv_keys;
    std::vector<std::vector<Resnet>> down_res;
    std::vector<std::vector<Xformer>> down_att;
    std::vector<ConvW> down_ds;
    Resnet mid_r0, mid_r1;
    Xformer mid_att;
    int temb_total = 0;
    int kv_total = 0;

    int num_skips() const;
    using SkipDst = std::function<View(int si)>;
    using SkipStat = std::function<GnStatBuf*(int si, long HW, int C)>;

  protected:
    void declare_encoder();
    int pack_encoder(std::vector<std::string>* tw, std::vector<std::string>* tb);
    int pack_resnet(const std::string& p, Resnet* r, std::vector<std::string>* tw, std::vector<std::string>* tb);
    int pack_xformer(const std::string& p, Xformer* x, int heads, int depth);
    int run_temb(Ctx& c, const float* timesteps, const half_t* add_text, const float* add_time_ids, int B, float** tproj);
    void run_conv_in(Ctx& c, const half_t* sample, int B, int H, int W, View y0, GnStatBuf* gb, const View* res,
                     GnStatBuf** xs);
    View run_down(Ctx& c, View x, GnStatBuf*& xs, int B, int& h, int& w, View text_kv, int L, const float* tproj,
                  const SkipDst& dst, const SkipStat& stat);
    void run_mid(Ctx& c, View x, GnStatBuf* xs, int B, int h, int w, View text_kv, int L, const float* tproj, View dst);
};

struct ControlNet : Encoder {
    ControlNet(const sd_unet_config& c, int conditioning_channels);
    ~ControlNet();
    int finalize();

    int cond_channels = 3;
    bool finalized = false;
    static constexpr int kCondLayers = 7;
    float* cond_w[kCondLayers] = {};
    float* cond_b[kCondLayers] = {};
    int cond_cin[kCondLayers] = {}, cond_cout[kCondLayers] = {}, cond_stride[kCondLayers] = {};
    ConvW cond_out;
    std::vector<ConvW> zero;
    ConvW zero_mid;
    UNet* attached = nullptr;

    void run_cond_embed(Ctx& c, const half_t* image, int n, int H, int W, View out);
    int run(Ctx& c, const half_t* sample, const float* timesteps, View text_kv, int L, const half_t* add_text,
            const float* add_time_ids, int B, int H, int W, View emb, const std::vector<View>& sites, View mid);
};

struct UNet : Encoder {
    explicit UNet(const sd_unet_config& c);
    int finalize();
    int forward(const half_t* sample, const float* timesteps, const half_t* ehs, int L,
                const half_t* add_text, const float* add_time_ids, half_t* out, int B, int H, int W,
                hipStream_t stream, const half_t* image_embeds = nullptr, int n_img = 0,
                const half_t* control = nullptr, int n_ctrl = 0, float cn_scale = 0.f);
    void set_ip_adapter(IPAdapter* a);
    void set_controlnet(ControlNet* n);

    Arena arena;
    bool finalized = false;
    long planned_key = -1;
    long planned_cn = -1;

    bool graph_enabled = false;
    hipStream_t gstream = nullptr;
    hipEvent_t ev_in = nullptr, ev_out = nullptr;
    hipGraphExec_t gexec = nullptr;
    long graph_key = -1;
    char* io_slab = nullptr;
    size_t io_cap = 0;
    int forward_graph(const half_t* sample, const float* timesteps, const half_t* ehs, int L, const half_t* add_text,
                      const float* add_time_ids, half_t* out, int B, int H, int W, hipStream_t stream);
    ~UNet();

    bool kv_cache_on = false, kv_valid = false;
    half_t* kv_cache = nullptr;
    size_t kv_cap = 0;
    const half_t* kv_src = nullptr;
    int kv_B = 0, kv_L = 0;

    IPAdapter* ip = nullptr;
    float ip_scale = 1.f;
    bool ipkv_valid = false;
    half_t* ipkv_cache = nullptr;
    size_t ipkv_cap = 0;
    const half_t* ipkv_src = nullptr;
    int ipkv_B = 0, ipkv_n = 0;

    ControlNet* cn = nullptr;
    bool cond_valid = false, cnkv_valid = false;
    half_t* cond_cache = nullptr;
    size_t cond_cap = 0;
    const half_t* cond_src = nullptr;
    int cond_B = 0, cond_n = 0, cond_H = 0, cond_W = 0;
    half_t* cnkv_cache = nullptr;
    size_t cnkv_cap = 0;
    const half_t* cnkv_src = nullptr;
    int cnkv_B = 0, cnkv_L = 0;

    ConvW conv_out;
    NormW norm_out;
    std::vector<std::vector<Resnet>> up_res;
    std::vector<std::vector<Xformer>> up_att;
    std::vector<ConvW> up_us;

  private:
    int run(Ctx& c, const half_t* sample, const float* timesteps, const half_t* ehs, int L,
            const half_t* add_text, const float* add_time_ids, half_t* out, int B, int H, int W,
            const half_t* image_embeds = nullptr, int n_img = 0, const half_t* control = nullptr, int n_ctrl = 0,
            float cn_scale = 0.f);
    int run_controlnet(Ctx& c, const half_t* sample, const float* timesteps, const half_t* ehs, int L,
                       const half_t* add_text, const float* add_time_ids, int B, int H, int W, const half_t* control,
                       int n_ctrl, const std::vector<View>& sites, View mid);
};

struct VAE {
    explicit VAE(const sd_vae_config& c);
    int finalize();
    int decode(const half_t* z, half_t* img, int B, int h, int w, hipStream_t stream);
    int encode(const half_t* img, half_t* moments, int B, int H, int W, hipStream_t stream);
    int encode_shift = 0;

    sd_vae_config cfg;
    WeightStore ws;
    Arena arena;
    bool finalized = false;
    long planned_key = -1;

    half_t* pq_w = nullptr; float* pq_b = nullptr;
    ConvW d_conv_in, d_conv_out;
    NormW d_norm_out;
    Resnet d_mid0, d_mid1;
    VaeAttn d_attn;
    std::vector<std::vector<Resnet>> d_up;
    std::vector<ConvW> d_us;
    half_t* q_w = nullptr; float* q_b = nullptr;
    ConvW e_conv_in, e_conv_out;
    NormW e_norm_out;
    Resnet e_mid0, e_mid1;
    VaeAttn e_attn;
    std::vector<std::vector<Resnet>> e_down;
    std::vector<ConvW> e_ds;

  private:
    int pack_resnet(const std::string& p, Resnet* r);
    int pack_attn(const std::string& p, VaeAttn* a);
    int pack_pointwise(const std::string& p, half_t** w, float** b);
    void run_attn(Ctx& c, const VaeAttn& a, View x, int N, int H, int W, View out, const GnStatBuf* x_stats,
                  GnStatBuf** out_stats, float stream_scale = 1.f);
    int run_decode(Ctx& c, const half_t* z, half_t* img, int B, int h, int w);
    int run_encode(Ctx& c, const half_t* img, half_t* moments, int B, int H, int W, float stream_scale);
};

struct ClipLayer {
    NormW ln1, ln2;
    ConvW qkv, out, fc1, fc2;
};
struct CLIP {
    explicit CLIP(const sd_clip_config& c);
    int finalize();
    int forward(const int* ids, const int* eos_index, half_t* hidden_states, half_t* last_hidden, half_t* pooled,
                half_t* text_embeds, int B, int T, hipStream_t stream);
    int final_layer_norm(const half_t* x, half_t* y, long rows, hipStream_t stream);

    sd_clip_config cfg;
    WeightStore ws;
    Arena arena;
    bool finalized = false;
    long planned_key = -1;
    half_t* tok = nullptr;
    half_t* pos = nullptr;
    half_t* proj = nullptr;
    std::vector<ClipLayer> layers;
    NormW final_ln;

  private:
    int run(Ctx& c, const int* ids, const int* eos_index, half_t* hidden_states, half_t* last_hidden, half_t* pooled,
            half_t* text_embeds, int B, int T);
};

}
```

### stablediffusion_amd/csrc/unet.cpp

```cpp
#include <algorithm>
#include <vector>

#include "model.h"
#include <cmath>
#include <cstdlib>

namespace sd {

void declare_resnet(WeightStore& ws, const std::string& p, int cin, int cout, int temb) {
    ws.declare(p + ".norm1.weight", {cin});
    ws.declare(p + ".norm1.bias", {cin});
    ws.declare(p + ".conv1.weight", {cout, cin, 3, 3});
    ws.declare(p + ".conv1.bias", {cout});
    if (temb) {
        ws.declare(p + ".time_emb_proj.weight", {cout, temb});
        ws.declare(p + ".time_emb_proj.bias", {cout});
    }
    ws.declare(p + ".norm2.weight", {cout});
    ws.declare(p + ".norm2.bias", {cout});
    ws.declare(p + ".conv2.weight", {cout, cout, 3, 3});
    ws.declare(p + ".conv2.bias", {cout});
    if (cin != cout) {
        ws.declare(p + ".conv_shortcut.weight", {cout, cin, 1, 1});
        ws.declare(p + ".conv_shortcut.bias", {cout});
// ... 188 lines not shown
                                   cfg.transformer_layers[i]))) return rc;
        }
        if (i != nb - 1 && (rc = ws.pack_conv(p + ".downsamplers.0.conv", &down_ds[i]))) return rc;
    }
    if ((rc = pack_resnet("mid_block.resnets.0", &mid_r0, tw, tb))) return rc;
    if ((rc = pack_xformer("mid_block.attentions.0", &mid_att, cfg.num_heads[nb - 1], cfg.transformer_layers[nb - 1]))) return rc;
    if ((rc = pack_resnet("mid_block.resnets.1", &mid_r1, tw, tb))) return rc;
    return 0;
}

int UNet::finalize() {
    if (finalized) return 0;
    std::string missing;
    if (!ws.complete(&missing)) { set_error("finalize: weight not set: " + missing); return 2; }
    const int nb = cfg.num_blocks;
    int rc;
    std::vector<std::string> tw, tb;
    temb_total = 0;
    kv_total = 0;
    kv_keys.clear();
    if ((rc = pack_encoder(&tw, &tb))) return rc;
    up_res.assign((size_t)nb, {}); up_att.assign((size_t)nb, {}); up_us.assign((size_t)nb, ConvW());
    for (int i = 0; i < nb; ++i) {
        const std::string p = "up_blocks." + std::to_string(i);
        up_res[i].resize((size_t)cfg.layers_per_block + 1);
        if (cfg.up_block_has_attn[i]) up_att[i].resize((size_t)cfg.layers_per_block + 1);
        for (int j = 0; j < cfg.layers_per_block + 1; ++j) {
            if ((rc = pack_resnet(p + ".resnets." + std::to_string(j), &up_res[i][j], &tw, &tb))) return rc;
            if (cfg.up_block_has_attn[i] &&
                (rc = pack_xformer(p + ".attentions." + std::to_string(j), &up_att[i][j], cfg.num_heads[nb - 1 - i],
                                   cfg.transformer_layers[nb - 1 - i]))) return rc;
        }
        if (i != nb - 1 && (rc = ws.pack_conv(p + ".upsamplers.0.conv", &up_us[i]))) return rc;
    }
    if ((rc = ws.pack_norm("conv_norm_out", &norm_out))) return rc;
    if ((rc = ws.pack_conv("conv_out", &conv_out))) return rc;
    if ((rc = ws.pack_rows(tw, tb, &temb_stack))) return rc;
    if (!kv_keys.empty() && (rc = ws.pack_rows(kv_keys, {}, &kv_all))) return rc;
    kv_keys.clear();
    SD_HIP_CHECK(hipDeviceSynchronize());
    ws.free_raw();
    finalized = true;
    return 0;
}

std::vector<std::pair<std::string, int>> unet_xattn_sites(const sd_unet_config& cfg, bool mid_last) {
    const int nb = cfg.num_blocks;
    const int* boc = cfg.block_out_channels;
    std::vector<std::pair<std::string, int>> down, up, mid;
    auto add = [](std::vector<std::pair<std::string, int>>& v, const std::string& p, int depth, int C) {
        for (int k = 0; k < depth; ++k) v.emplace_back(p + ".transformer_blocks." + std::to_string(k), C);
    };
    for (int i = 0; i < nb; ++i)
        if (cfg.down_block_has_attn[i])
            for (int j = 0; j < cfg.layers_per_block; ++j)
                add(down, "down_blocks." + std::to_string(i) + ".attentions." + std::to_string(j), cfg.transformer_layers[i], boc[i]);
    add(mid, "mid_block.attentions.0", cfg.transformer_layers[nb - 1], boc[nb - 1]);
    for (int i = 0; i < nb; ++i)
        if (cfg.up_block_has_attn[i])
            for (int j = 0; j < cfg.layers_per_block + 1; ++j)
                add(up, "up_blocks." + std::to_string(i) + ".attentions." + std::to_string(j),
                    cfg.transformer_layers[nb - 1 - i], boc[nb - 1 - i]);
    std::vector<std::pair<std::string, int>> all = down;
    const auto& second = mid_last ? up : mid;
    const auto& third = mid_last ? mid : up;
    all.insert(all.end(), second.begin(), second.end());
    all.insert(all.end(), third.begin(), third.end());
    return all;
}

namespace {
const char* kIpProj = "encoder_hid_proj.image_projection_layers.0";
}

IPAdapter::IPAdapter(const sd_unet_config& c, int image_embed_dim, int num_tokens)
    : cfg(c), d_img(image_embed_dim), n_tok(num_tokens) {
    const int ctx = cfg.cross_attention_dim;
    const std::string p = kIpProj;
    ws.declare(p + ".image_embeds.weight", {(int64_t)n_tok * ctx, d_img});
    ws.declare(p + ".image_embeds.bias", {(int64_t)n_tok * ctx});
    ws.declare(p + ".norm.weight", {ctx});
    ws.declare(p + ".norm.bias", {ctx});
    for (const auto& site : unet_xattn_sites(cfg, true)) {
        ws.declare(site.first + ".attn2.processor.to_k_ip.0.weight", {site.second, ctx});
        ws.declare(site.first + ".attn2.processor.to_v_ip.0.weight", {site.second, ctx});
    }
}

int IPAdapter::finalize() {
    if (finalized) return 0;
    std::string missing;
    if (!ws.complete(&missing)) { set_error("ip adapter finalize: weight not set: " + missing); return 2; }
    const std::string p = kIpProj;
    int rc;
    if ((rc = ws.pack_conv(p + ".image_embeds", &proj))) return rc;
    if ((rc = ws.pack_norm(p + ".norm", &norm))) return rc;
    std::vector<std::string> keys;
    kv_total = 0;
    for (const auto& site : unet_xattn_sites(cfg, false)) {
        keys.push_back(site.first + ".attn2.processor.to_k_ip.0.weight");
        keys.push_back(site.first + ".attn2.processor.to_v_ip.0.weight");
        kv_total += 2 * site.second;
    }
    if ((rc = ws.pack_rows(keys, {}, &kv_all))) return rc;
    SD_HIP_CHECK(hipDeviceSynchronize());
    ws.free_raw();
    finalized = true;
    return 0;
}

void UNet::set_ip_adapter(IPAdapter* a) {
    if (ip == a) return;
    if (ip) ip->attached = nullptr;
    if (a) {
        if (a->attached && a->attached != this) a->attached->set_ip_adapter(nullptr);
        a->attached = this;
    }
    ip = a;
    ipkv_valid = false;
    planned_key = -1;
}

void run_resnet(Ctx& c, const Resnet& r, View x, int N, int H, int W, View out, int G, float eps,
                const float* tproj, int tproj_ld, const GnStatBuf* x_stats, GnStatBuf** out_stats, float stream_scale,
                GnStatBuf* out_buf, int out_groups) {
    Arena& a = *c.arena;
    const size_t mk = a.mark();
    const long M = (long)N * H * W;
    const float s = stream_scale, eps_s = eps * s * s;
    View h2(a.alloc_h(M * r.cout), r.cout, r.cout);
    const long HW = (long)H * W;
    ConvFuse f1;
    f1.gn_out = gn_wants_stats(HW, r.cout, G) ? ctx_gnbuf(c) : nullptr;
    f1.gn_groups = G;
    f1.acc_scale = s; f1.bias_scale = s;
    op_gn_conv(c, r.n1, r.c1, x, N, H, W, h2, G, eps_s, 1, x_stats, tproj ? tproj + r.temb_off : nullptr, tproj_ld, nullptr, &f1);
    View res = x;
    if (r.has_sc) {
        res = View(a.alloc_h(M * r.cout), r.cout, r.cout);
        ConvFuse fs;
        fs.bias_scale = s;
        op_conv(c, r.sc, x, N, H, W, res, 1, 0, nullptr, 0, nullptr, 0, -1, 0, s != 1.f ? &fs : nullptr);
    }
    ConvFuse f2;
    f2.gn_out = (out_stats && gn_wants_stats(HW, r.cout, G)) ? (out_buf ? out_buf : ctx_gnbuf(c)) : nullptr;
    f2.gn_groups = out_groups > 0 ? out_groups : G;
    f2.acc_scale = s; f2.bias_scale = s;
    op_gn_conv(c, r.n2, r.c2, h2, N, H, W, out, G, eps_s, 1, f1.gn_out, nullptr, 0, &res, &f2);
    if (out_stats) *out_stats = f2.gn_out;
    a.release(mk);
}

void run_xformer(Ctx& c, const Xformer& t, View x, int N, int H, int W, View out, int G, View text_kv, int L,
                 const GnStatBuf* x_stats, GnStatBuf** out_stats, GnStatBuf* out_buf, int out_groups) {
    Arena& a = *c.arena;
    const size_t mk = a.mark();
    const int C = t.C;
    const int T = H * W;
    const long M = (long)N * T;
    const int d = C / t.heads;
    const bool fold = !t.blocks.empty() && t.blocks[0].fold;
    View hn(a.alloc_h(M * C), C, C);
    op_groupnorm(c, t.gn, x, hn, N, T, G, 1e-6f, 0, x_stats);
    View cur(a.alloc_h(M * C), C, C), nxt(a.alloc_h(M * C), C, C);
    RowStat st_cur, st_t2, st_t3;
    if (fold) {
        st_cur.p = a.alloc_f(rowstat_floats(M, C));
        st_t2.p = a.alloc_f(rowstat_floats(M, C));
        st_t3.p = a.alloc_f(rowstat_floats(M, C));
    }
    ConvFuse f_cur, f_t2, f_t3, f_ln1, f_ln2, f_ln3;
    f_cur.stat_out = &st_cur; f_t2.stat_out = &st_t2; f_t3.stat_out = &st_t3;
    f_ln1.ln_in = &st_cur; f_ln2.ln_in = &st_t2; f_ln3.ln_in = &st_t3;
    f_ln1.ln_eps = f_ln2.ln_eps = f_ln3.ln_eps = 1e-5f;
    op_conv(c, t.pin, hn, N, H, W, cur, 1, 0, nullptr, 0, nullptr, 0, -1, 0, fold ? &f_cur : nullptr);
    for (size_t bi = 0; bi < t.blocks.size(); ++bi) {
        const TBlock& b = t.blocks[bi];
        const bool more = bi + 1 < t.blocks.size();
        const size_t mb = a.mark();
        View n(fold ? nullptr : a.alloc_h(M * C), C, C);
        View qkv(a.alloc_h(M * 3 * C), 3 * C, 3 * C);
        if (fold) {
            op_conv(c, b.qkv, cur, N, H, W, qkv, 1, 0, nullptr, 0, nullptr, 0, -1, 0, &f_ln1);
        } else {
            op_layernorm(c, b.ln1, cur, n, M, 1e-5f);
            op_conv(c, b.qkv, n, N, H, W, qkv);
        }
        View att(a.alloc_h(M * C), C, C);
        op_attention(c, qkv.slice(0, C), qkv.slice(C, C), qkv.slice(2 * C, C), att, N, T, T, t.heads, d, 0, 1);
        View t2(a.alloc_h(M * C), C, C);
        op_conv(c, b.out1, att, N, H, W, t2, 1, 0, nullptr, 0, &cur, 0, -1, 0, fold ? &f_t2 : nullptr);
        View q(a.alloc_h(M * C), C, C);
        if (fold) {
            op_conv(c, b.q2, t2, N, H, W, q, 1, 0, nullptr, 0, nullptr, 0, -1, 0, &f_ln2);
        } else {
            op_layernorm(c, b.ln2, t2, n, M, 1e-5f);
            op_conv(c, b.q2, n, N, H, W, q);
        }
        if (c.ip_kv.p && c.ip_scale != 0.f)
            op_ip_attention(c, q, text_kv.slice(b.kv_off, C), text_kv.slice(b.kv_off + C, C), c.ip_kv.slice(b.ip_kv_off, C),
                            c.ip_kv.slice(b.ip_kv_off + C, C), att, N, T, L, c.ip_T, t.heads, d, c.ip_scale);
        else
            op_attention(c, q, text_kv.slice(b.kv_off, C), text_kv.slice(b.kv_off + C, C), att, N, T, L, t.heads, d, 0, 1);
        View t3(a.alloc_h(M * C), C, C);
        op_conv(c, b.out2, att, N, H, W, t3, 1, 0, nullptr, 0, &t2, 0, -1, 0, fold ? &f_t3 : nullptr);
        if (!(fold && !more && op_ffn_fused(c, b.ff1, b.ff2, t3, st_t3, 1e-5f, M, nxt))) {
            View g(a.alloc_h(M * 4 * C), 4 * C, 4 * C);
            if (fold) {
                op_conv(c, b.ff1, t3, N, H, W, g, 1, 0, nullptr, 0, nullptr, 1, -1, 0, &f_ln3);
            } else {
                op_layernorm(c, b.ln3, t3, n, M, 1e-5f);
                op_conv(c, b.ff1, n, N, H, W, g, 1, 0, nullptr, 0, nullptr, 1);
            }
            op_conv(c, b.ff2, g, N, H, W, nxt, 1, 0, nullptr, 0, &t3, 0, -1, 0, (fold && more) ? &f_cur : nullptr);
        }
        a.release(mb);
        View tmp = cur; cur = nxt; nxt = tmp;
    }
    ConvFuse fo;
    fo.gn_out = (out_stats && gn_wants_stats(T, C, G)) ? (out_buf ? out_buf : ctx_gnbuf(c)) : nullptr;
    fo.gn_groups = out_groups > 0 ? out_groups : G;
    op_conv(c, t.pout, cur, N, H, W, out, 1, 0, nullptr, 0, &x, 0, -1, 0, &fo);
    if (out_stats) *out_stats = fo.gn_out;
    a.release(mk);
}

int Encoder::run_temb(Ctx& c, const float* timesteps, const half_t* add_text, const float* add_time_ids, int B,
                      float** tproj_out) {
    Arena& a = *c.arena;
    const int* boc = cfg.block_out_channels;
    const int temb = boc[0] * 4;
    hipStream_t s = c.stream;
    const bool go = !c.dry;
    float* sinus = a.alloc_f((long)B * boc[0]);
    float* e1 = a.alloc_f((long)B * temb);
    float* emb = a.alloc_f((long)B * temb);
    float* tproj = a.alloc_f((long)B * temb_total);
    *tproj_out = tproj;
    if (go && !c.err) c.err = launch_timestep_sinusoid(timesteps, 1, sinus, B, boc[0], cfg.flip_sin_to_cos, cfg.freq_shift, boc[0], s);
    if (go && !c.err) c.err = launch_small_linear(sinus, boc[0], te1.w, te1.bias, e1, temb, B, boc[0], temb, 0, 1, s);
    const bool aug_path = cfg.addition_time_embed_dim > 0;
    if (go && !c.err) c.err = launch_small_linear(e1, temb, te2.w, te2.bias, emb, temb, B, temb, temb, 0, aug_path ? 0 : 1, s);
    if (aug_path) {
        const int ad = cfg.addition_time_embed_dim;
        const int pin = cfg.projection_class_embeddings_input_dim;
        const int tdim = pin - 6 * ad;
        if (!add_text || !add_time_ids) { set_error("unet: add_text / add_time_ids required for text_time conditioning"); return 1; }
        float* addin = a.alloc_f((long)B * pin);
        float* a1 = a.alloc_f((long)B * temb);
        float* aug = a.alloc_f((long)B * temb);
        float* txt = a.alloc_f((long)B * tdim);
        if (go && !c.err) c.err = launch_f16_to_f32(add_text, txt, (long)B * tdim, s);
        if (go && !c.err) {
            hipError_t e = hipMemcpy2DAsync(addin, (size_t)pin * 4, txt, (size_t)tdim * 4, (size_t)tdim * 4, (size_t)B,
                                            hipMemcpyDeviceToDevice, s);
            if (e != hipSuccess) { set_error(hipGetErrorString(e)); c.err = 3; }
        }
        if (go && !c.err) {
            for (int j = 0; j < 6 && !c.err; ++j)
                c.err = launch_timestep_sinusoid(add_time_ids + j, 6, addin + tdim + j * ad, B, ad,
                                                         cfg.flip_sin_to_cos, cfg.freq_shift, pin, s);
        }
        if (go && !c.err) c.err = launch_small_linear(addin, pin, ae1.w, ae1.bias, a1, temb, B, pin, temb, 0, 1, s);
        if (go && !c.err) c.err = launch_small_linear(a1, temb, ae2.w, ae2.bias, aug, temb, B, temb, temb, 0, 0, s);
        if (go && !c.err) c.err = launch_add_f32(emb, aug, (long)B * temb, 1, s);
    }
    if (go && !c.err) c.err = launch_small_linear(emb, temb, temb_stack.w, temb_stack.bias, tproj, temb_total, B, temb, temb_total, 0, 0, s);

    return c.err;
}

void Encoder::run_conv_in(Ctx& c, const half_t* sample, int B, int H, int W, View y0, GnStatBuf* gb, const View* res,
                          GnStatBuf** xs) {
    Arena& a = *c.arena;
    const int* boc = cfg.block_out_channels;
    const int G = cfg.norm_num_groups;
    hipStream_t s = c.stream;
    const bool go = !c.dry;
    const size_t mk = a.mark();
    const long M = (long)B * H * W;
    HeadParams hp;
    hp.x_nchw = sample; hp.w = conv_in.w; hp.K = conv_in.K; hp.bias = conv_in.bias; hp.y = y0.p; hp.ldy = y0.ld;
    hp.gnstat_out = (gb && gb->buf) ? gb->buf : nullptr; hp.G = G;
    hp.N = B; hp.Cin = cfg.in_channels; hp.H = H; hp.W = W; hp.Cout = boc[0];
    if (!res && conv_head_supported(hp)) {
        if (gb) {
            gb->st = GnStats();
            if (hp.gnstat_out) { gb->st.part = gb->buf; gb->st.rows = 128; gb->st.S = (int)((long)H * W / 128); }
        }
        if (go && !c.err) {
            prof_open(s, "conv_head_kernel", 2.0 * M * boc[0] * 9.0 * cfg.in_channels, 2.0 * M * (boc[0] + cfg.in_channels));
            c.err = launch_conv_head(hp, s);
            prof_close(s);
        }
        *xs = gb;
    } else {
        half_t* col = a.alloc_h(M * conv_in.K);
        if (go && !c.err) c.err = launch_im2col_nchw3x3(sample, col, B, cfg.in_channels, H, W, (int)conv_in.K, s);
        ConvW pw = conv_in; pw.ks = 1;
        ConvFuse f;
        f.gn_out = gb;
        f.gn_groups = G;
        op_conv(c, pw, View(col, conv_in.K, (int)conv_in.K), B, H, W, y0, 1, 0, nullptr, 0, res, 0, -1, 0, &f);
        *xs = f.gn_out;
    }
    a.release(mk);
}

View Encoder::run_down(Ctx& c, View x, GnStatBuf*& xs, int B, int& h, int& w, View text_kv, int L, const float* tproj,
                       const SkipDst& skip_view, const SkipStat& skip_stat) {
    Arena& a = *c.arena;
    const int nb = cfg.num_blocks;
    const int G = cfg.norm_num_groups;
    const float eps = cfg.norm_eps;
    int skip_i = 1;
    for (int i = 0; i < nb; ++i) {
        for (int j = 0; j < cfg.layers_per_block; ++j) {
            const Resnet& r = down_res[i][j];
            if (cfg.down_block_has_attn[i]) {
                const size_t mk = a.mark();
                View tmp(a.alloc_h((long)B * h * w * r.cout), r.cout, r.cout);
                GnStatBuf* rs = nullptr;
                run_resnet(c, r, x, B, h, w, tmp, G, eps, tproj, temb_total, xs, &rs);
                View dst = skip_view(skip_i);
                run_xformer(c, down_att[i][j], tmp, B, h, w, dst, G, text_kv, L, rs, &xs, skip_stat(skip_i, (long)h * w, r.cout));
                a.release(mk);
                x = dst;
            } else {
                View dst = skip_view(skip_i);
                run_resnet(c, r, x, B, h, w, dst, G, eps, tproj, temb_total, xs, &xs, 1.f, skip_stat(skip_i, (long)h * w, r.cout));
                x = dst;
            }
            ++skip_i;
        }
        if (i != nb - 1) {
            ConvFuse f;
            f.gn_out = skip_stat(skip_i, (long)(h / 2) * (w / 2), down_ds[i].cout);
            View dst = skip_view(skip_i++);
            f.gn_groups = G;
            op_conv(c, down_ds[i], x, B, h, w, dst, 2, 0, nullptr, 0, nullptr, 0, -1, 0, &f);
            xs = f.gn_out;
            h /= 2; w /= 2;
            x = dst;
        }
    }

    return x;
}

void Encoder::run_mid(Ctx& c, View x, GnStatBuf* xs, int B, int h, int w, View text_kv, int L, const float* tproj,
                      View dst) {
    Arena& a = *c.arena;
    const int nb = cfg.num_blocks;
    const int* boc = cfg.block_out_channels;
    const int G = cfg.norm_num_groups;
    const float eps = cfg.norm_eps;
    const int C = boc[nb - 1];
    const long M = (long)B * h * w;
    View m0(a.alloc_h(M * C), C, C), m1(a.alloc_h(M * C), C, C);
    GnStatBuf *s0 = nullptr, *s1 = nullptr;
    run_resnet(c, mid_r0, x, B, h, w, m0, G, eps, tproj, temb_total, xs, &s0);
    run_xformer(c, mid_att, m0, B, h, w, m1, G, text_kv, L, s0, &s1);
    run_resnet(c, mid_r1, m1, B, h, w, dst, G, eps, tproj, temb_total, s1);
}

int Encoder::num_skips() const { return 1 + cfg.num_blocks * cfg.layers_per_block + (cfg.num_blocks - 1); }

int UNet::run(Ctx& c, const half_t* sample, const float* timesteps, const half_t* ehs, int L,
              const half_t* add_text, const float* add_time_ids, half_t* out, int B, int H, int W,
              const half_t* image_embeds, int n_img, const half_t* control, int n_ctrl, float cn_scale) {
    Arena& a = *c.arena;
    const int nb = cfg.num_blocks;
    const int* boc = cfg.block_out_channels;
    const int G = cfg.norm_num_groups;
    const float eps = cfg.norm_eps;
    hipStream_t s = c.stream;
    const bool go = !c.dry;

    float* tproj = nullptr;
    if (int rc = run_temb(c, timesteps, add_text, add_time_ids, B, &tproj)) return rc;

    const bool kv_cached = kv_cache_on && !graph_enabled && kv_cache != nullptr;
    View text_kv(kv_cached ? kv_cache : a.alloc_h((long)B * L * kv_total), kv_total, kv_total);
    if (!(kv_cached && kv_valid && kv_src == ehs && kv_B == B && kv_L == L)) {
        op_conv(c, kv_all, View(const_cast<half_t*>(ehs), cfg.cross_attention_dim, cfg.cross_attention_dim), B, L, 1, text_kv);
        if (kv_cached && go && !c.err) { kv_valid = true; kv_src = ehs; kv_B = B; kv_L = L; }
    }

    if (ip && image_embeds) {
        const int ctx = cfg.cross_attention_dim, T_ip = n_img * ip->n_tok;
        const long rows = (long)B * n_img, ntc = (long)ip->n_tok * ctx;
        const bool ip_cached = kv_cache_on && !graph_enabled && ipkv_cache != nullptr;
        View ip_kv(ip_cached ? ipkv_cache : a.alloc_h((long)B * T_ip * ip->kv_total), ip->kv_total, ip->kv_total);
        const bool hit = ip_cached && ipkv_valid && ipkv_src == image_embeds && ipkv_B == B && ipkv_n == n_img;
        if (c.dry || !hit) {
            const size_t mk = a.mark();
            float* e32 = a.alloc_f(rows * ip->d_img);
            float* p32 = a.alloc_f(rows * ntc);
            half_t* p16 = a.alloc_h(rows * ntc);
            half_t* tok = a.alloc_h(rows * ntc);
            if (go && !c.err) c.err = launch_f16_to_f32(image_embeds, e32, rows * ip->d_img, s);
            if (go && !c.err) {
                prof_open(s, "small_linear_kernel", 2.0 * rows * ntc * ip->d_img, 2.0 * ntc * ip->d_img);
                c.err = launch_small_linear(e32, ip->d_img, ip->proj.w, ip->proj.bias, p32, ntc, (int)rows, ip->d_img,
                                            (int)ntc, 0, 0, s);
                prof_close(s);
            }
            if (go && !c.err) c.err = launch_f32_to_f16(p32, p16, rows * ntc, s);
            op_layernorm(c, ip->norm, View(p16, ctx, ctx), View(tok, ctx, ctx), rows * ip->n_tok, 1e-5f);
            op_conv(c, ip->kv_all, View(tok, ctx, ctx), B, T_ip, 1, ip_kv);
            a.release(mk);
            if (ip_cached && go && !c.err) { ipkv_valid = true; ipkv_src = image_embeds; ipkv_B = B; ipkv_n = n_img; }
        }
        c.ip_kv = ip_kv;
        c.ip_T = T_ip;
        c.ip_scale = ip_scale;
    }

    struct Cat { half_t* p; int c1, c2, h, w; };
    std::vector<Cat> cats;
    {
        int out_ch = boc[nb - 1];
        int h = H >> (nb - 1), w = W >> (nb - 1);
        for (int i = 0; i < nb; ++i) {
            const int prev = out_ch;
            out_ch = boc[nb - 1 - i];
            const int in_ch = boc[nb - 1 - (i + 1 < nb ? i + 1 : nb - 1)];
            for (int j = 0; j < cfg.layers_per_block + 1; ++j) {
                Cat ct;
                ct.c2 = (j == cfg.layers_per_block) ? in_ch : out_ch;
                ct.c1 = (j == 0) ? prev : out_ch;
                ct.h = h; ct.w = w;
                ct.p = a.alloc_h((long)B * h * w * (ct.c1 + ct.c2));
                cats.push_back(ct);
            }
            if (i != nb - 1) { h *= 2; w *= 2; }
        }
    }
    const int nskip = (int)cats.size();
    int skip_i = 0;
    auto skip_view = [&](int si) {
        const Cat& ct = cats[(size_t)(nskip - 1 - si)];
        return View(ct.p + ct.c1, ct.c1 + ct.c2, ct.c2);
    };

    ctx_gnpool_init(c, B, (long)H * W, G);
    GnStatBuf* xs = nullptr;
    std::vector<GnStatBuf> sst((size_t)nskip);
    GnStatBuf hid;
    if (c.gnpool[0].buf) {
        for (auto& b : sst) b.buf = a.alloc_f(gnstat_floats(B, (long)H * W, G));
        hid.buf = a.alloc_f(gnstat_floats(B, (long)H * W, 128));
    }
    auto skip_stat = [&](int si, long HWs, int C) -> GnStatBuf* {
        return (sst[(size_t)si].buf && gn_wants_stats(HWs, C, G)) ? &sst[(size_t)si] : nullptr;
    };

    const bool use_cn = cn && control && cn_scale != 0.f;
    const size_t cn_mark = a.mark();
    std::vector<View> cn_sites;
    std::vector<int> cn_rows;
    View cn_mid;
    if (use_cn) {
        int hh = H, ww = W;
        auto site = [&](int C) {
            cn_sites.emplace_back(a.alloc_h((long)B * hh * ww * C), C, C);
            cn_rows.push_back(B * hh * ww);
        };
        site(boc[0]);
        for (int i = 0; i < nb; ++i) {
            for (int j = 0; j < cfg.layers_per_block; ++j) site(boc[i]);
            if (i != nb - 1) { hh /= 2; ww /= 2; site(boc[i]); }
        }
        cn_mid = View(a.alloc_h((long)B * hh * ww * boc[nb - 1]), boc[nb - 1], boc[nb - 1]);
        cn_rows.push_back(B * hh * ww);
        GnStatBuf ring[Ctx::kGnPool];
        for (int i = 0; i < Ctx::kGnPool; ++i) ring[i] = c.gnpool[i];
        const int ring_next = c.gn_next, ring_groups = c.gn_groups;
        if (int rc = run_controlnet(c, sample, timesteps, ehs, L, add_text, add_time_ids, B, H, W, control, n_ctrl, cn_sites,
                                    cn_mid)) return rc;
        for (int i = 0; i < Ctx::kGnPool; ++i) c.gnpool[i] = ring[i];
        c.gn_next = ring_next; c.gn_groups = ring_groups;
    }

    int h = H, w = W;
    run_conv_in(c, sample, B, H, W, skip_view(skip_i), skip_stat(skip_i, (long)H * W, boc[0]), nullptr, &xs);
    View x = skip_view(skip_i++);

    x = run_down(c, x, xs, B, h, w, text_kv, L, tproj, [&](int si) { return skip_view(si); },
                 [&](int si, long HWs, int C) { return skip_stat(si, HWs, C); });

    run_mid(c, x, xs, B, h, w, text_kv, L, tproj, View(cats[0].p, cats[0].c1 + cats[0].c2, cats[0].c1));

    if (use_cn) {
        ConvFuse f;
        f.acc_scale = cn_scale; f.bias_scale = cn_scale;
        for (int si = 0; si <= nskip; ++si) {
            const View xh = si < nskip ? cn_sites[(size_t)si] : cn_mid;
            const View y = si < nskip ? skip_view(si) : View(cats[0].p, cats[0].c1 + cats[0].c2, cats[0].c1);
            const ConvW& zw = si < nskip ? cn->zero[(size_t)si] : cn->zero_mid;
            op_conv(c, zw, xh, 1, cn_rows[(size_t)si], 1, y, 1, 0, nullptr, 0, &y, 0, -1, 0, &f);
        }
    }
    if (use_cn) a.release(cn_mark);

    View final_x;
    int k = 0;
    const GnStatBuf* hid_ready = nullptr;
    int hid_groups = 0;
    static const bool no_cat_env = getenv("SD_GN_CAT") == nullptr;
    const bool no_cat_stats = no_cat_env || use_cn;
    for (int i = 0; i < nb; ++i) {
        for (int j = 0; j < cfg.layers_per_block + 1; ++j, ++k) {
            const Cat& ct = cats[(size_t)k];
            const Resnet& r = up_res[i][j];
            View xin(ct.p, ct.c1 + ct.c2, ct.c1 + ct.c2);
            const bool last_in_block = (j == cfg.layers_per_block);
            const bool last = last_in_block && i == nb - 1;
            View dst;
            const size_t mk = a.mark();
            if (!last_in_block) {
                const Cat& nx = cats[(size_t)k + 1];
                dst = View(nx.p, nx.c1 + nx.c2, nx.c1);
            } else {
                dst = View(a.alloc_h((long)B * h * w * r.cout), r.cout, r.cout);
            }
            const long HWc = (long)h * w;
            const int Ccat = ct.c1 + ct.c2, si = nskip - 1 - k;
            GnStatBuf catst;
            const GnStatBuf* xin_stats = nullptr;
            if (!no_cat_stats && hid_ready && hid_ready->st.part && sst[(size_t)si].st.part && gn_wants_stats(HWc, Ccat, G) &&
                ct.c2 % G == 0 && (Ccat / G) % (ct.c2 / G) == 0 && ct.c1 % (ct.c2 / G) == 0) {
                float* fin = a.alloc_f((long)B * G * 2);
                if (go && !c.err) {
                    prof_open(s, "gn_cat_finalize_kernel", 0.0, 8.0 * B * (hid_ready->st.S * hid_groups + sst[(size_t)si].st.S * G));
                    c.err = launch_gn_cat_finalize(hid_ready->st, hid_groups, ct.c1, sst[(size_t)si].st, G, ct.c2, fin, B, HWc, G, s);
                    prof_close(s);
                }
                catst.buf = fin;
                catst.st.part = fin; catst.st.S = 1; catst.st.rows = HWc;
                xin_stats = &catst;
            }
            hid_ready = nullptr;
            int nx_groups = 0;
            if (!last && hid.buf && !no_cat_stats) {
                const Cat& nx = cats[(size_t)k + 1];
                const int u = gn_cat_unit(nx.c1, nx.c2, G);
                if (gn_wants_stats(last_in_block ? HWc * 4 : HWc, nx.c1 + nx.c2, G) && (u >= 8 || u == 4) && nx.c1 / u <= 128) nx_groups = nx.c1 / u;
            }
            const bool hid_here = nx_groups > 0 && !last_in_block;
            GnStatBuf* outp = nullptr;
            xs = nullptr;
            if (cfg.up_block_has_attn[i]) {
                View tmp(a.alloc_h((long)B * h * w * r.cout), r.cout, r.cout);
                GnStatBuf* rs = nullptr;
                run_resnet(c, r, xin, B, h, w, tmp, G, eps, tproj, temb_total, xin_stats, &rs);
                if (last) run_xformer(c, up_att[i][j], tmp, B, h, w, dst, G, text_kv, L, rs, &xs);
                else if (hid_here) run_xformer(c, up_att[i][j], tmp, B, h, w, dst, G, text_kv, L, rs, &outp, &hid, nx_groups);
                else run_xformer(c, up_att[i][j], tmp, B, h, w, dst, G, text_kv, L, rs, nullptr);
            } else {
                if (last) run_resnet(c, r, xin, B, h, w, dst, G, eps, tproj, temb_total, xin_stats, &xs);
                else if (hid_here) run_resnet(c, r, xin, B, h, w, dst, G, eps, tproj, temb_total, xin_stats, &outp, 1.f, &hid, nx_groups);
                else run_resnet(c, r, xin, B, h, w, dst, G, eps, tproj, temb_total, xin_stats, nullptr);
            }
            if (last) {
                final_x = dst;
            } else {
                if (last_in_block) {
                    const Cat& nx = cats[(size_t)k + 1];
                    View up_dst(nx.p, nx.c1 + nx.c2, nx.c1);
                    ConvFuse fu;
                    fu.gn_out = nx_groups > 0 ? &hid : nullptr;
                    fu.gn_groups = nx_groups;
                    op_conv(c, up_us[i], dst, B, h, w, up_dst, 1, 1, nullptr, 0, nullptr, 0, -1, 0, nx_groups > 0 ? &fu : nullptr);
                    outp = fu.gn_out;
                    h *= 2; w *= 2;
                }
                hid_ready = outp;
                hid_groups = nx_groups;
                a.release(mk);
            }
        }
    }

    {
        const int C = boc[0];
        const long M = (long)B * h * w;
        TailParams tp;
        tp.x = final_x.p; tp.ldx = final_x.ld;
        if (xs && xs->st.part) { tp.gn_part = xs->st.part; tp.gn_S = xs->st.S; tp.gn_rows = xs->st.rows; }
        tp.G = G; tp.eps = eps; tp.gamma = norm_out.gamma; tp.beta = norm_out.beta; tp.silu = 1;
        tp.w = conv_out.w; tp.K = conv_out.K; tp.bias = conv_out.bias; tp.y = out;
        tp.N = B; tp.H = h; tp.W = w; tp.C = C; tp.Cout = cfg.out_channels;
        if (go && !c.err && conv_tail_supported(tp)) {
            prof_open(s, "conv_tail_kernel", 2.0 * M * cfg.out_channels * 9.0 * C, 2.0 * M * (C + cfg.out_channels));
            c.err = launch_conv_tail(tp, s);
            prof_close(s);
            return c.err;
        }
        View hn(a.alloc_h(M * C), C, C);
        op_groupnorm(c, norm_out, final_x, hn, B, (long)h * w, G, eps, 1, xs);
        if (cfg.out_channels <= 4 && conv_out.ks == 3 && conv_out.K == 9L * C && M >= kSmallCoutMinPixels) {
            if (go && !c.err) {
                prof_open(s, "conv3x3_small_cout_kernel", 2.0 * M * cfg.out_channels * 9.0 * C, 2.0 * M * (C + cfg.out_channels));
                c.err = launch_conv3x3_small_cout(hn.p, hn.ld, conv_out.w, conv_out.K, conv_out.bias, out, B, h, w, C,
                                                  cfg.out_channels, s);
                prof_close(s);
            }
        } else {
            View y(a.alloc_h(M * cfg.out_channels), cfg.out_channels, cfg.out_channels);
            op_conv(c, conv_out, hn, B, h, w, y);
            if (go && !c.err) c.err = launch_nhwc_to_nchw(y.p, y.ld, out, B, (long)h * w, cfg.out_channels, s);
        }
    }
    return c.err;
}

UNet::~UNet() {
    if (gexec) (void)hipGraphExecDestroy(gexec);
    if (ev_in) (void)hipEventDestroy(ev_in);
    if (ev_out) (void)hipEventDestroy(ev_out);
    if (gstream) (void)hipStreamDestroy(gstream);
    if (io_slab) (void)hipFree(io_slab);
    if (kv_cache) (void)hipFree(kv_cache);
    if (ipkv_cache) (void)hipFree(ipkv_cache);
    if (cond_cache) (void)hipFree(cond_cache);
    if (cnkv_cache) (void)hipFree(cnkv_cache);
    if (ip) ip->attached = nullptr;
    if (cn) cn->attached = nullptr;
}

int UNet::forward_graph(const half_t* sample, const float* timesteps, const half_t* ehs, int L,
                        const half_t* add_text, const float* add_time_ids, half_t* out, int B, int H, int W,
                        hipStream_t stream) {
    const bool sdxl = cfg.addition_time_embed_dim > 0;
    const int pdim = sdxl ? cfg.projection_class_embeddings_input_dim - 6 * cfg.addition_time_embed_dim : 0;
    auto up = [](size_t v) { return (v + 255) & ~size_t(255); };
    const size_t n_sample = up((size_t)B * cfg.in_channels * H * W * 2), n_t = up((size_t)B * 4);
    const size_t n_ehs = up((size_t)B * L * cfg.cross_attention_dim * 2), n_text = up((size_t)B * pdim * 2);
    const size_t n_ids = up((size_t)B * 6 * 4), n_out = up((size_t)B * cfg.out_channels * H * W * 2);
    const size_t need = n_sample + n_t + n_ehs + n_text + n_ids + n_out;
    if (!gstream) {
        SD_HIP_CHECK(hipStreamCreateWithFlags(&gstream, hipStreamNonBlocking));
        SD_HIP_CHECK(hipEventCreateWithFlags(&ev_in, hipEventDisableTiming));
        SD_HIP_CHECK(hipEventCreateWithFlags(&ev_out, hipEventDisableTiming));
    }
    if (need > io_cap) {
        SD_HIP_CHECK(hipDeviceSynchronize());
        if (io_slab) (void)hipFree(io_slab);
        io_slab = nullptr; io_cap = 0; graph_key = -1;
        SD_HIP_CHECK(hipMalloc(reinterpret_cast<void**>(&io_slab), need));
        io_cap = need;
    }
    char* ptr = io_slab;
    half_t* g_sample = reinterpret_cast<half_t*>(ptr); ptr += n_sample;
    float* g_t = reinterpret_cast<float*>(ptr); ptr += n_t;
    half_t* g_ehs = reinterpret_cast<half_t*>(ptr); ptr += n_ehs;
    half_t* g_text = sdxl ? reinterpret_cast<half_t*>(ptr) : nullptr; ptr += n_text;
    float* g_ids = sdxl ? reinterpret_cast<float*>(ptr) : nullptr; ptr += n_ids;
    half_t* g_out = reinterpret_cast<half_t*>(ptr);
    SD_HIP_CHECK(hipMemcpyAsync(g_sample, sample, (size_t)B * cfg.in_channels * H * W * 2, hipMemcpyDeviceToDevice, stream));
    SD_HIP_CHECK(hipMemcpyAsync(g_t, timesteps, (size_t)B * 4, hipMemcpyDeviceToDevice, stream));
    SD_HIP_CHECK(hipMemcpyAsync(g_ehs, ehs, (size_t)B * L * cfg.cross_attention_dim * 2, hipMemcpyDeviceToDevice, stream));
    if (sdxl) {
        if (!add_text || !add_time_ids) { set_error("unet: add_text / add_time_ids required for text_time conditioning"); return 1; }
        SD_HIP_CHECK(hipMemcpyAsync(g_text, add_text, (size_t)B * pdim * 2, hipMemcpyDeviceToDevice, stream));
        SD_HIP_CHECK(hipMemcpyAsync(g_ids, add_time_ids, (size_t)B * 6 * 4, hipMemcpyDeviceToDevice, stream));
    }
    const long key = ((long)B << 40) ^ ((long)H << 20) ^ (long)W ^ ((long)L << 52);
    int rc = 0;
    if (key != graph_key || !gexec) {
        graph_enabled = false;
        rc = forward(g_sample, g_t, g_ehs, L, g_text, g_ids, g_out, B, H, W, stream);
        graph_enabled = true;
        if (rc) return rc;
        if (gexec) { (void)hipGraphExecDestroy(gexec); gexec = nullptr; }
        hipGraph_t graph = nullptr;
        SD_HIP_CHECK(hipStreamBeginCapture(gstream, hipStreamCaptureModeRelaxed));
        Ctx ctx{&arena, gstream, false};
        arena.begin(false);
        rc = run(ctx, g_sample, g_t, g_ehs, L, g_text, g_ids, g_out, B, H, W);
        hipError_t e = hipStreamEndCapture(gstream, &graph);
        if (rc) { if (graph) (void)hipGraphDestroy(graph); return rc; }
        if (e != hipSuccess) { set_error(std::string("hipStreamEndCapture: ") + hipGetErrorString(e)); return 3; }
        e = hipGraphInstantiate(&gexec, graph, nullptr, nullptr, 0);
        (void)hipGraphDestroy(graph);
        if (e != hipSuccess) { gexec = nullptr; set_error(std::string("hipGraphInstantiate: ") + hipGetErrorString(e)); return 3; }
        graph_key = key;
    } else {
        SD_HIP_CHECK(hipEventRecord(ev_in, stream));
        SD_HIP_CHECK(hipStreamWaitEvent(gstream, ev_in, 0));
        SD_HIP_CHECK(hipGraphLaunch(gexec, gstream));
        SD_HIP_CHECK(hipEventRecord(ev_out, gstream));
        SD_HIP_CHECK(hipStreamWaitEvent(stream, ev_out, 0));
    }
    SD_HIP_CHECK(hipMemcpyAsync(out, g_out, (size_t)B * cfg.out_channels * H * W * 2, hipMemcpyDeviceToDevice, stream));
    return 0;
}

int UNet::forward(const half_t* sample, const float* timesteps, const half_t* ehs, int L, const half_t* add_text,
                  const float* add_time_ids, half_t* out, int B, int H, int W, hipStream_t stream,
                  const half_t* image_embeds, int n_img, const half_t* control, int n_ctrl, float cn_scale) {
    if (!finalized) { set_error("unet: forward before finalize"); return 2; }
    const int div = 1 << (cfg.num_blocks - 1);
    if (B <= 0 || H % div != 0 || W % div != 0) { set_error("unet: H and W must be divisible by 2^(blocks-1)"); return 1; }
    if (ip && !image_embeds) { set_error("unet: an IP-Adapter is attached: image_embeds required"); return 1; }
    if (!ip && image_embeds) { set_error("unet: image_embeds given but no IP-Adapter is attached"); return 1; }
    if (ip) {
        if (n_img < 1 || n_img * ip->n_tok > 64) { set_error("unet: images per prompt x adapter tokens must be in [1, 64]"); return 4; }
        if (L < 1 || L > 160) { set_error("unet: with an IP-Adapter the text length must be in [1, 160]"); return 4; }
        if (graph_enabled) { set_error("unet: graph replay with an IP-Adapter attached is not supported"); return 4; }
    } else {
        n_img = 0;
    }
    if (cn && !control) { set_error("unet: a ControlNet is attached: control image required"); return 1; }
    if (!cn && control) { set_error("unet: control image given but no ControlNet is attached"); return 1; }
    if (cn) {
        if (n_ctrl < 1 || B % n_ctrl != 0) { set_error("unet: the control image count must divide the batch"); return 1; }
        if (!(cn_scale == cn_scale)) { set_error("unet: conditioning scale is NaN"); return 1; }
        if (graph_enabled) { set_error("unet: graph replay with a ControlNet attached is not supported"); return 4; }
    } else {
        n_ctrl = 0;
        cn_scale = 0.f;
    }
    const bool use_cn = cn && cn_scale != 0.f;
    if (graph_enabled && !prof_enabled())
        return forward_graph(sample, timesteps, ehs, L, add_text, add_time_ids, out, B, H, W, stream);
    if (kv_cache_on) {
        const size_t need = (size_t)B * L * kv_total * sizeof(half_t);
        if (need > kv_cap) {
            SD_HIP_CHECK(hipDeviceSynchronize());
            if (kv_cache) (void)hipFree(kv_cache);
            kv_cache = nullptr; kv_cap = 0; kv_valid = false;
            SD_HIP_CHECK(hipMalloc(reinterpret_cast<void**>(&kv_cache), need));
            kv_cap = need;
        }
        if (ip) {
            const size_t ineed = (size_t)B * n_img * ip->n_tok * ip->kv_total * sizeof(half_t);
            if (ineed > ipkv_cap) {
                SD_HIP_CHECK(hipDeviceSynchronize());
                if (ipkv_cache) (void)hipFree(ipkv_cache);
                ipkv_cache = nullptr; ipkv_cap = 0; ipkv_valid = false;
                SD_HIP_CHECK(hipMalloc(reinterpret_cast<void**>(&ipkv_cache), ineed));
                ipkv_cap = ineed;
            }
        }
        if (use_cn) {
            const size_t cneed = (size_t)B * H * W * cn->cfg.block_out_channels[0] * sizeof(half_t);
            if (cneed > cond_cap) {
                SD_HIP_CHECK(hipDeviceSynchronize());
                if (cond_cache) (void)hipFree(cond_cache);
                cond_cache = nullptr; cond_cap = 0; cond_valid = false;
                SD_HIP_CHECK(hipMalloc(reinterpret_cast<void**>(&cond_cache), cneed));
                cond_cap = cneed;
            }
            const size_t kneed = (size_t)B * L * cn->kv_total * sizeof(half_t);
            if (kneed > cnkv_cap) {
                SD_HIP_CHECK(hipDeviceSynchronize());
                if (cnkv_cache) (void)hipFree(cnkv_cache);
                cnkv_cache = nullptr; cnkv_cap = 0; cnkv_valid = false;
                SD_HIP_CHECK(hipMalloc(reinterpret_cast<void**>(&cnkv_cache), kneed));
                cnkv_cap = kneed;
            }
        }
    }
    const long key = ((long)B << 40) ^ ((long)H << 20) ^ (long)W ^ ((long)L << 52) ^ (kv_cache_on ? (1L << 62) : 0) ^
                     (ip ? (long)(n_img * ip->n_tok) << 32 : 0);
    const long cn_key = use_cn ? n_ctrl : 0;
    if (key != planned_key || cn_key != planned_cn) {
        Ctx dry{&arena, stream, true};
        arena.begin(true);
        int rc = run(dry, sample, timesteps, ehs, L, add_text, add_time_ids, out, B, H, W, image_embeds, n_img, control,
                     n_ctrl, cn_scale);
        if (rc) return rc;
        if (arena.peak() > arena.capacity()) {
            SD_HIP_CHECK(hipDeviceSynchronize());
            rc = arena.reserve(arena.peak());
            if (rc) return rc;
        }
        planned_key = key;
        planned_cn = cn_key;
    }
    Ctx ctx{&arena, stream, false};
    arena.begin(false);
    int rc = run(ctx, sample, timesteps, ehs, L, add_text, add_time_ids, out, B, H, W, image_embeds, n_img, control, n_ctrl,
                 cn_scale);
    if (!rc && arena.overflow()) { set_error("unet: workspace overflow (planner bug)"); return 2; }
    return rc;
}

}
```

### stablediffusion_amd/models.py

```python
from __future__ import annotations

import ctypes as C
import weakref
from types import SimpleNamespace
from typing import Dict, Optional

import torch

from . import _lib
from .config import UNetConfig, VAEConfig


def _stream_ptr() -> int:
    return torch.cuda.current_stream().cuda_stream


def _as_f16(x: torch.Tensor, device) -> torch.Tensor:
    return x.to(device=device, dtype=torch.float16).contiguous()


class _Config(SimpleNamespace):
    def get(self, k, d=None):
        return getattr(self, k, d)

# ... 104 lines not shown
    def text_kv_cache(self, enable: bool = True):
        _lib.check(self._lib.sd_unet_text_kv_cache(self._h, int(bool(enable))), "sd_unet_text_kv_cache")
        return self

    def attach_ip_adapter(self, adapter: Optional["HipIPAdapter"]):
        if adapter is not None and adapter.cfg.to_dict() != self.cfg.to_dict():
            raise ValueError("IP-Adapter was built for another UNet configuration")
        _lib.check(self._lib.sd_unet_set_ip_adapter(self._h, adapter._h if adapter is not None else None),
                   "sd_unet_set_ip_adapter")
        if self._ip is not None and self._ip is not adapter:
            self._ip._unet = None
        if adapter is not None:
            old = adapter._unet() if adapter._unet is not None else None
            if old is not None and old is not self:
                old._ip = None
            adapter._unet = weakref.ref(self)
        self._ip = adapter
        return self

    def make_ip_adapter(self, state_dict: Dict[str, torch.Tensor], image_embed_dim: int, num_tokens: int):
        return HipIPAdapter(self, image_embed_dim, num_tokens).load_state_dict(state_dict)

    @property
    def ip_adapter(self):
        return self._ip

    def set_ip_adapter_scale(self, scale: float):
        _lib.check(self._lib.sd_unet_set_ip_adapter_scale(self._h, float(scale)), "sd_unet_set_ip_adapter_scale")
        self._ip_scale = float(scale)
        return self

    def attach_controlnet(self, controlnet: Optional["HipControlNetModel"]):
        _lib.check(self._lib.sd_unet_set_controlnet(self._h, controlnet._h if controlnet is not None else None),
                   "sd_unet_set_controlnet")
        if self._cn is not None and self._cn is not controlnet:
            self._cn._unet = None
        if controlnet is not None:
            old = controlnet._unet() if controlnet._unet is not None else None
            if old is not None and old is not self:
                old._cn = None
            controlnet._unet = weakref.ref(self)
        self._cn = controlnet
        return self

    def make_controlnet(self, cn_config: UNetConfig, state_dict: Dict[str, torch.Tensor]):
        return HipControlNetModel(self, cn_config).load_state_dict(state_dict)

    @property
    def controlnet(self):
        return self._cn

    def _control(self, controlnet_cond, scale, B, H, W, dev):
        if self._cn is None:
            if controlnet_cond is not None or scale is not None:
                raise ValueError("controlnet_cond / controlnet_conditioning_scale given but no ControlNet is attached")
            return None, 0.0
        if controlnet_cond is None or scale is None:
            raise ValueError("a ControlNet is attached: controlnet_cond and controlnet_conditioning_scale are required")
        if isinstance(controlnet_cond, (list, tuple)) or isinstance(scale, (list, tuple)):
            raise NotImplementedError("MultiControlNet (lists of control images / scales) is not supported")
        cond = _as_f16(controlnet_cond, dev)
        n = cond.shape[0]
        if cond.ndim != 4 or cond.shape[1] != 3 or cond.shape[2] != 8 * H or cond.shape[3] != 8 * W:
            raise ValueError(f"controlnet_cond: expected [n, 3, {8 * H}, {8 * W}], got {tuple(cond.shape)}")
        if n < 1 or B % n:
            raise ValueError(f"controlnet_cond: {n} images do not divide the batch {B}")
        return cond, float(scale)

    def _image_embeds(self, added_cond_kwargs, B, dev):
        embeds = (added_cond_kwargs or {}).get("image_embeds")
        if self._ip is None:
            if embeds is not None:
                raise ValueError("added_cond_kwargs['image_embeds'] given but no IP-Adapter is attached")
            return None
        if embeds is None:
            raise ValueError("an IP-Adapter is attached: added_cond_kwargs['image_embeds'] is required")
        if isinstance(embeds, (list, tuple)):
            if len(embeds) != 1:
                raise ValueError(f"one IP-Adapter is attached, got image_embeds for {len(embeds)}")
            embeds = embeds[0]
        if embeds.ndim == 2:
            embeds = embeds[:, None]
        if embeds.ndim != 3 or embeds.shape[0] != B or embeds.shape[2] != self._ip.image_embed_dim:
            raise ValueError(f"image_embeds: expected [{B}, n_img, {self._ip.image_embed_dim}], got {tuple(embeds.shape)}")
        return _as_f16(embeds, dev)

    def to(self, device=None, dtype=None):
        if device is not None and torch.device(device).type != "cuda":
            raise _lib.EngineError("HipUNet2DConditionModel lives on the HIP device only")
        return self

    def eval(self):
        return self

    def __call__(self, sample, timestep, encoder_hidden_states, cross_attention_kwargs=None,
                 added_cond_kwargs=None, return_dict=False, controlnet_cond=None, controlnet_conditioning_scale=None,
                 **unused):
        for k in ("down_block_additional_residuals", "mid_block_additional_residual", "down_intrablock_additional_residuals",
                  "guess_mode"):
            v = unused.get(k)
            if v is not None and v is not False:
                raise NotImplementedError(f"HipUNet2DConditionModel: {k} is not supported; attach the ControlNet to the "
                                          "engine (attach_controlnet) and pass controlnet_cond=")
        if not self._finalized:
            raise _lib.EngineError("weights not loaded")
        dev = self.device
        sample = _as_f16(sample, dev)
        B, _, H, W = sample.shape
        ehs = _as_f16(encoder_hidden_states, dev)
        if ehs.shape[0] != B:
            raise ValueError(f"encoder_hidden_states batch {ehs.shape[0]} != sample batch {B}")
        if ehs.shape[2] != self.cfg.cross_attention_dim:
            raise ValueError("encoder_hidden_states width != cross_attention_dim")
        if isinstance(timestep, (int, float)):
            t = torch.full((B,), float(timestep), device=dev, dtype=torch.float32)
        else:
            t = torch.as_tensor(timestep, device=dev).to(torch.float32).reshape(-1)
            t = t.expand(B).contiguous() if t.numel() == 1 else t.contiguous()
        add_text = add_ids = None
        pt = pi = None
        if self.cfg.addition_embed_type == "text_time":
            if not added_cond_kwargs or "text_embeds" not in added_cond_kwargs or "time_ids" not in added_cond_kwargs:
                raise ValueError("added_cond_kwargs needs text_embeds and time_ids for text_time conditioning")
            add_text = _as_f16(added_cond_kwargs["text_embeds"], dev)
            add_ids = added_cond_kwargs["time_ids"].to(device=dev, dtype=torch.float32).contiguous()
            pt, pi = C.c_void_p(add_text.data_ptr()), C.c_void_p(add_ids.data_ptr())
        img = self._image_embeds(added_cond_kwargs, B, dev)
        ctrl, cscale = self._control(controlnet_cond, controlnet_conditioning_scale, B, H, W, dev)
        out = torch.empty((B, self.cfg.out_channels, H, W), device=dev, dtype=torch.float16)
        with torch.cuda.device(dev):
            if ctrl is not None:
                rc = self._lib.sd_unet_forward_cn(self._h, C.c_void_p(sample.data_ptr()), C.c_void_p(t.data_ptr()),
                                                  C.c_void_p(ehs.data_ptr()), ehs.shape[1], pt, pi,
                                                  C.c_void_p(img.data_ptr()) if img is not None else None,
                                                  img.shape[1] if img is not None else 0,
                                                  C.c_void_p(ctrl.data_ptr()), ctrl.shape[0], cscale,
                                                  C.c_void_p(out.data_ptr()), B, H, W, C.c_void_p(_stream_ptr()))
            elif img is None:
                rc = self._lib.sd_unet_forward(self._h, C.c_void_p(sample.data_ptr()), C.c_void_p(t.data_ptr()),
                                               C.c_void_p(ehs.data_ptr()), ehs.shape[1], pt, pi,
                                               C.c_void_p(out.data_ptr()), B, H, W, C.c_void_p(_stream_ptr()))
            else:
                rc = self._lib.sd_unet_forward_ex(self._h, C.c_void_p(sample.data_ptr()), C.c_void_p(t.data_ptr()),
                                                  C.c_void_p(ehs.data_ptr()), ehs.shape[1], pt, pi,
                                                  C.c_void_p(img.data_ptr()), img.shape[1],
                                                  C.c_void_p(out.data_ptr()), B, H, W, C.c_void_p(_stream_ptr()))
        _lib.check(rc, "sd_unet_forward")
        if return_dict:
            return SimpleNamespace(sample=out)
        return (out,)

    forward = __call__

    def set_adapters(self, *a, **k):
        raise NotImplementedError("fuse LoRA weights on load (stablediffusion_amd.weights.fuse_lora)")

    delete_adapters = add_adapter = set_adapters

    def parameters(self):
        return iter(())

    def __del__(self):
        try:
            if getattr(self, "_h", None):
                self._lib.sd_unet_destroy(self._h)
                self._h = None
        except Exception:
            pass


class HipIPAdapter:

    def __init__(self, unet: HipUNet2DConditionModel, image_embed_dim: int, num_tokens: int = 4):
        self._lib = _lib.load()
        self.cfg = unet.cfg
        self.device = unet.device
        self.image_embed_dim = int(image_embed_dim)
        self.num_tokens = int(num_tokens)
        self._unet = None
        self._h = C.c_void_p()
        _lib.check(self._lib.sd_ip_adapter_create(unet._h, self.image_embed_dim, self.num_tokens, C.byref(self._h)),
                   "sd_ip_adapter_create")
        self._finalized = False

    def load_state_dict(self, state_dict: Dict[str, torch.Tensor], strict: bool = True):
        _lib.require_gpu()
        with torch.cuda.device(self.device):
            _load_weights(self._lib, self._h, "ip_adapter", state_dict, strict)
            _lib.check(self._lib.sd_ip_adapter_finalize(self._h), "sd_ip_adapter_finalize")
        self._finalized = True
        return self

    def __del__(self):
        try:
            if getattr(self, "_h", None):
                u = self._unet() if self._unet is not None else None
                if u is not None:
                    u._ip = None
                self._lib.sd_ip_adapter_destroy(self._h)
                self._h = None
        except Exception:
            pass


class HipControlNetModel:

    def __init__(self, unet: HipUNet2DConditionModel, cn_config: UNetConfig, conditioning_channels: int = 3):
        self._lib = _lib.load()
        self.cfg = cn_config
        self.device = unet.device
        self._unet = None
        c = _unet_config_struct(cn_config)
        self._h = C.c_void_p()
        _lib.check(self._lib.sd_controlnet_create(unet._h, C.byref(c), int(conditioning_channels), C.byref(self._h)),
                   "sd_controlnet_create")
        self._finalized = False

    def load_state_dict(self, state_dict: Dict[str, torch.Tensor], strict: bool = True):
        _lib.require_gpu()
        with torch.cuda.device(self.device):
            _load_weights(self._lib, self._h, "controlnet", state_dict, strict)
            _lib.check(self._lib.sd_controlnet_finalize(self._h), "sd_controlnet_finalize")
        self._finalized = True
        return self

    def cond_embedding(self, image: torch.Tensor) -> torch.Tensor:
        x = _as_f16(image, self.device)
        n, _, H8, W8 = x.shape
        if H8 % 8 or W8 % 8:
            raise ValueError("control image height and width must be multiples of 8")
        c0 = self.cfg.block_out_channels[0]
        out = torch.empty((n, H8 // 8, W8 // 8, c0), device=self.device, dtype=torch.float16)
        with torch.cuda.device(self.device):
            rc = self._lib.sd_op_controlnet_cond_embed(self._h, C.c_void_p(x.data_ptr()), n, H8 // 8, W8 // 8,
                                                       C.c_void_p(out.data_ptr()), 0, None, C.c_void_p(_stream_ptr()))
        _lib.check(rc, "sd_op_controlnet_cond_embed")
        return out.permute(0, 3, 1, 2)

    def __del__(self):
        try:
            if getattr(self, "_h", None):
                u = self._unet() if self._unet is not None else None
                if u is not None:
                    u._cn = None
                self._lib.sd_controlnet_destroy(self._h)
                self._h = None
        except Exception:
            pass


class _LatentDist:

    def __init__(self, moments: torch.Tensor):
        self.mean, logvar = moments.float().chunk(2, dim=1)
        self.logvar = logvar.clamp(-30.0, 20.0)
        self.std = torch.exp(0.5 * self.logvar)

    def sample(self, generator=None):
        noise = torch.randn(self.mean.shape, generator=generator, device=self.mean.device, dtype=self.mean.dtype)
        return (self.mean + self.std * noise).to(torch.float16)

    def mode(self):
        return self.mean.to(torch.float16)


class HipAutoencoderKL:

    def __init__(self, config: VAEConfig, device: str = "cuda"):
        self._lib = _lib.load()
        self.cfg = config
        self.device = torch.device(device)
        self.dtype = torch.float16
        c = _lib.SdVAEConfig()
        c.in_channels = config.in_channels
        c.out_channels = config.out_channels
        c.latent_channels = config.latent_channels
        c.num_blocks = len(config.block_out_channels)
        for i, ch in enumerate(config.block_out_channels):
            c.block_out_channels[i] = ch
        c.layers_per_block = config.layers_per_block
        c.norm_num_groups = config.norm_num_groups
        self._h = C.c_void_p()
        _lib.check(self._lib.sd_vae_create(C.byref(c), C.byref(self._h)), "sd_vae_create")
        self.config = _Config(**config.to_dict())
        self._finalized = False
        self._enc_shift = 0

    def load_state_dict(self, state_dict: Dict[str, torch.Tensor], strict: bool = True):
        _lib.require_gpu()
        with torch.cuda.device(self.device):
            _load_weights(self._lib, self._h, "vae", state_dict, strict)
            _lib.check(self._lib.sd_vae_finalize(self._h), "sd_vae_finalize")
        self._finalized = True
        return self

    def memory(self):
        w, s = C.c_int64(), C.c_int64()
        _lib.check(self._lib.sd_vae_memory(self._h, C.byref(w), C.byref(s)), "sd_vae_memory")
        return w.value, s.value

    def to(self, device=None, dtype=None):
        if device is not None and not isinstance(device, torch.dtype) and torch.device(device).type != "cuda":
            raise _lib.EngineError("HipAutoencoderKL lives on the HIP device only")
        return self

    def eval(self):
# ... 189 lines not shown
```

### stablediffusion_amd/pipeline.py

```python
from __future__ import annotations

from typing import Any, Dict, List, Optional, Union

import torch

from . import schedulers as _sched
from .image_processor import VaeImageProcessor


class SDModelWrapper:

    def __init__(self, base=None, vae=None, text_encoder=None, tokenizer=None, scheduler=None,
                 text_encoder_2=None, tokenizer_2=None, model_type: str = "sd15", device: str = "cuda",
                 model_name: Optional[str] = None, unet_state_dict: Optional[Dict[str, torch.Tensor]] = None,
                 text_encoder_state_dict: Optional[Dict[str, torch.Tensor]] = None,
                 text_encoder_2_state_dict: Optional[Dict[str, torch.Tensor]] = None,
                 image_encoder=None, feature_extractor=None, prediction_type: Optional[str] = None):
        self.base = base
        self.image_encoder = image_encoder
        self.feature_extractor = feature_extractor
        self._ip = None
        self._ip_scale = 1.0
        self._cn = None
        self._lora = None
# ... 53 lines not shown
        fused = self._lora.fused("unet")
        old = self.base
        graph = bool(getattr(old, "_graph_on", False))
        self.base = None
        del old
        self.base = self._rebuild_from(fused, graph)
        for part in ("text_encoder", "text_encoder_2"):
            if self._te_sd[part] is not None and (self._lora.touches(part) or self._lora_applied is not None):
                enc = getattr(self, part, None)
                sd = self._lora.fused(part)
                if hasattr(enc, "rebuild"):
                    setattr(self, part, enc.rebuild(sd))
                elif hasattr(enc, "load_state_dict"):
                    enc.load_state_dict(sd, strict=False)
                else:
                    raise ValueError(f"{type(enc).__name__} cannot take fused text-encoder LoRA weights")
        self._lora_applied = sig

    def _rebuild_from(self, fused, graph):
        base = self._base_factory(fused)
        if graph and hasattr(base, "use_graph"):
            base.use_graph(True)
        if self._ip is not None:
            self._attach_ip(base)
        if self._cn is not None:
            self._attach_cn(base)
        return base

    def _attach_cn(self, base):
        cfg, sd = self._cn
        base.attach_controlnet(base.make_controlnet(cfg, sd))

    def load_controlnet(self, pretrained_model_name_or_path_or_dict):
        from . import controlnet
        if isinstance(pretrained_model_name_or_path_or_dict, (list, tuple)):
            raise NotImplementedError("MultiControlNet (a list of ControlNets) is not supported")
        cfg, sd = controlnet.load(pretrained_model_name_or_path_or_dict, self.base.cfg)
        self._cn = (cfg, sd)
        self._attach_cn(self.base)

    def unload_controlnet(self):
        if self._cn is not None:
            self.base.attach_controlnet(None)
        self._cn = None

    @property
    def has_controlnet(self) -> bool:
        return self._cn is not None

    def _attach_ip(self, base):
        sd, d_img, n_tok = self._ip
        base.attach_ip_adapter(base.make_ip_adapter(sd, d_img, n_tok))
        base.set_ip_adapter_scale(self._ip_scale)

    def load_ip_adapter(self, pretrained_model_name_or_path_or_dict):
        from . import ip_adapter
        sd, d_img, n_tok = ip_adapter.convert(pretrained_model_name_or_path_or_dict, self.base.cfg)
        self._ip = (sd, d_img, n_tok)
        self._ip_scale = 1.0
        self._attach_ip(self.base)

    def set_ip_adapter_scale(self, scale: float):
        self._ip_scale = float(scale)
        if self._ip is not None:
            self.base.set_ip_adapter_scale(self._ip_scale)

    def unload_ip_adapter(self):
        if self._ip is not None:
            self.base.attach_ip_adapter(None)
            self.base.set_ip_adapter_scale(1.0)
        self._ip = None
        self._ip_scale = 1.0

    def _refuse(self):
        self.apply_adapters()

    def load_lora_weights(self, pretrained_model_name_or_path_or_dict, adapter_name: Optional[str] = None, **kwargs):
        self._adapters().load(pretrained_model_name_or_path_or_dict, adapter_name)

    def set_adapters(self, adapter_names, adapter_weights=None):
        self._adapters().set(adapter_names, adapter_weights)

    def delete_adapters(self, adapter_names):
        self._adapters().delete(adapter_names)

    def get_list_adapters(self):
        return {"base": self._lora.names()} if self._lora is not None and self._lora.names() else {}

    def set_lora_scale(self, scale: float):
        if self._lora is None:
            return
        self._lora.scale = float(scale)

    def configure_scheduler(self, **fields):
        self.scheduler = type(self.scheduler).from_config(self.scheduler.config, **fields)

    def load_scheduler_config(self, folder):
        from . import checkpoints
        self.configure_scheduler(**checkpoints.read_scheduler_config(folder))

    def set_scheduler(self, scheduler_name):
        if getattr(self, "scheduler_name", None) == scheduler_name:
            return
        if scheduler_name not in _sched.REGISTRY:
            raise ValueError(f"Unknown scheduler name: {scheduler_name}")
        self.scheduler = _sched.REGISTRY[scheduler_name](self.scheduler.config)
        self.scheduler_name = scheduler_name


def convert_pt_to_numpy(images: torch.Tensor):
    if images.is_cuda and images.dtype == torch.float16 and images.dim() == 4 and images.shape[1] <= 4:
        import ctypes as C
        from . import _lib
        lib = _lib.load()
        images = images.contiguous()
        B, Cc, H, W = images.shape
        out = torch.empty(B, H, W, Cc, dtype=torch.uint8, device=images.device)
        rc = lib.sd_images_to_uint8(C.c_void_p(images.data_ptr()), C.c_void_p(out.data_ptr()), B, Cc, H, W,
                                    C.c_void_p(torch.cuda.current_stream().cuda_stream))
        if rc:
            raise RuntimeError(lib.sd_last_error().decode())
        host = out.cpu().numpy()
        return [host[i] for i in range(B)]
    np_images = []
    for idx in range(len(images)):
        img = (images[idx] / 2 + 0.5).clamp(0, 1)
        np_images.append((img.permute(1, 2, 0) * 255).to(torch.uint8).cpu().numpy())
    return np_images


def rescale_noise_cfg(noise_cfg, noise_pred_text, guidance_rescale=0.0):
    dims = list(range(1, noise_pred_text.ndim))
    std_text = noise_pred_text.std(dim=dims, keepdim=True)
    std_cfg = noise_cfg.std(dim=dims, keepdim=True)
    rescaled = noise_cfg * (std_text / std_cfg)
    return guidance_rescale * rescaled + (1 - guidance_rescale) * noise_cfg


def retrieve_timesteps(scheduler, num_inference_steps=None, device=None, **kwargs):
    scheduler.set_timesteps(num_inference_steps, device=device, **kwargs)
    return scheduler.timesteps, num_inference_steps


def denoising_value_valid(dnv):
    return isinstance(dnv, float) and 0 < dnv < 1


class StableDiffusionUnifiedPipeline:
    def __init__(self, do_cfg: bool = True, device: Optional[str] = None, output_type: Optional[str] = None):
        self.do_classifier_free_guidance = bool(do_cfg)
        self.device = torch.device(device) if device is not None else torch.device("cpu")
        self.output_type = output_type if output_type is not None else "pt"
        self.model: Optional[SDModelWrapper] = None

    @torch.no_grad()
    def __call__(
        self,
        model: SDModelWrapper,
        prompt: Union[str, List[str], None] = None,
        prompt_2=None,
        negative_prompt=None,
        negative_prompt_2=None,
        height: Optional[int] = None,
        width: Optional[int] = None,
        num_images_per_prompt: Optional[int] = 1,
        num_inference_steps: int = 50,
        denoising_end: Optional[float] = None,
        guidance_scale: float = 5.0,
        latents: Optional[torch.Tensor] = None,
        output_type: Optional[str] = "pt",
        cross_attention_kwargs: Optional[Dict[str, Any]] = None,
        guidance_rescale: float = 0.0,
        clip_skip: Optional[int] = None,
        seed: Optional[int] = None,
        image=None,
        strength: float = 1.0,
        denoising_start: Optional[float] = None,
        mask_image=None,
        masked_image_latents=None,
        padding_mask_crop: Optional[int] = None,
        prompt_embeds: Optional[torch.Tensor] = None,
        negative_prompt_embeds: Optional[torch.Tensor] = None,
        pooled_prompt_embeds: Optional[torch.Tensor] = None,
        negative_pooled_prompt_embeds: Optional[torch.Tensor] = None,
        ip_adapter_image=None,
        ip_adapter_image_embeds: Optional[List[torch.Tensor]] = None,
        control_image=None,
        controlnet_conditioning_scale: float = 1.0,
        control_guidance_start: float = 0.0,
        control_guidance_end: float = 1.0,
        guess_mode: bool = False,
    ):
        if guess_mode:
            raise NotImplementedError("ControlNet guess_mode is not supported")
        if not 0.0 <= float(guidance_rescale) <= 1.0:
            raise ValueError(f"guidance_rescale must lie in [0, 1], got {guidance_rescale}")
        guidance_rescale = float(guidance_rescale) if self.do_classifier_free_guidance else 0.0
        has_cn = bool(getattr(model, "has_controlnet", False))
        if control_image is not None and not has_cn:
            raise ValueError("control_image given but no ControlNet is loaded (SDModelWrapper.load_controlnet)")
        if has_cn and control_image is None:
            raise ValueError("a ControlNet is loaded: control_image is required (or unload_controlnet)")
        if has_cn:
            if any(isinstance(v, (list, tuple)) for v in (controlnet_conditioning_scale, control_guidance_start,
                                                          control_guidance_end)):
                raise NotImplementedError("MultiControlNet (lists of scales / guidance windows) is not supported")
            if not 0.0 <= control_guidance_start < control_guidance_end <= 1.0:
                raise ValueError("need 0 <= control_guidance_start < control_guidance_end <= 1")
        if model.device != self.device:
            model.to(self.device)
        self.model = model
        if hasattr(model, "set_lora_scale"):
            lora_scale = cross_attention_kwargs.get("scale", None) if cross_attention_kwargs is not None else None
            model.set_lora_scale(1.0 if lora_scale is None else lora_scale)
        if hasattr(model, "apply_adapters"):
            model.apply_adapters()
        if image is not None and mask_image is None:
            image = model.image_processor.preprocess(image)
            if image.shape[1] != 4:
                height, width = image.shape[-2], image.shape[-1]
        if has_cn and image is None and (height is None or width is None):
            ci = self.control_image_processor(model).preprocess(control_image, height=height, width=width)
            height, width = ci.shape[-2], ci.shape[-1]
        height = height or model.base.config.sample_size * model.vae_scale_factor
        width = width or model.base.config.sample_size * model.vae_scale_factor

        if prompt is not None and isinstance(prompt, str):
            batch_size = 1
        elif prompt is not None and isinstance(prompt, list):
            batch_size = len(prompt)
        elif prompt_embeds is not None:
            batch_size = prompt_embeds.shape[0]
        else:
            raise ValueError("either `prompt` or `prompt_embeds` is required")

        if prompt_embeds is None:
            prompt_embeds, negative_prompt_embeds, pooled_prompt_embeds, negative_pooled_prompt_embeds = \
                self.encode_prompt(prompt, prompt_2, negative_prompt, negative_prompt_2,
                                   num_images_per_prompt, None, clip_skip)
        else:
            prompt_embeds = prompt_embeds.to(self.device)
            if self.do_classifier_free_guidance:
                if negative_prompt_embeds is None:
                    raise ValueError("negative_prompt_embeds is required with prompt_embeds when CFG is on")
                negative_prompt_embeds = negative_prompt_embeds.to(self.device)

        timesteps, num_inference_steps = retrieve_timesteps(model.scheduler, num_inference_steps, self.device)

        self.is_inpaint = False
        mask = masked_image_latents_2b = image_latents = noise = None
        num_channels_unet = model.base.config.in_channels
        if image is None:
            shape = (batch_size * num_images_per_prompt, model.base.config.in_channels,
                     height // model.vae_scale_factor, width // model.vae_scale_factor)
            latents = self.prepare_latents_txt2img(shape, prompt_embeds.dtype, seed, latents)
        elif mask_image is not None:
            if padding_mask_crop is not None:
                crops_coords = model.mask_processor.get_crop_region(mask_image, width, height, pad=padding_mask_crop)
                resize_mode = "fill"
            else:
                crops_coords, resize_mode = None, "default"
            latent_input = isinstance(image, torch.Tensor) and image.ndim == 4 and image.shape[1] == 4
            init_image = model.image_processor.preprocess(
                image, height=None if latent_input else height, width=None if latent_input else width,
                crops_coords=crops_coords, resize_mode=resize_mode).to(torch.float32)
            mask = model.mask_processor.preprocess(mask_image, height=height, width=width, resize_mode=resize_mode,
                                                   crops_coords=crops_coords)
            if masked_image_latents is not None:
                masked_image = masked_image_latents
            elif init_image.shape[1] == 4:
                masked_image = None
            else:
                masked_image = init_image * (mask < 0.5)
            timesteps, num_inference_steps = self.get_timesteps(
                num_inference_steps, strength, denoising_start if denoising_value_valid(denoising_start) else None)
            if num_inference_steps < 1:
                raise ValueError(f"After adjusting the num_inference_steps by strength parameter: {strength}, the "
                                 f"number of pipeline steps is {num_inference_steps} which is < 1.")
            latent_timestep = timesteps[:1].repeat(batch_size * num_images_per_prompt)
            is_strength_max = strength == 1.0
            num_channels_latents = model.vae.config.latent_channels
            return_image_latents = num_channels_unet == 4
            shape = (batch_size * num_images_per_prompt, num_channels_latents,
                     height // model.vae_scale_factor, width // model.vae_scale_factor)
            latents, noise, image_latents = self.prepare_latents_inpaint(
                shape, prompt_embeds.dtype, seed, latents, init_image, latent_timestep, is_strength_max,
                add_noise=denoising_start is None, return_image_latents=return_image_latents)
            mask, masked_image_latents_2b = self.prepare_mask_latents(
                mask, masked_image, batch_size * num_images_per_prompt, height // model.vae_scale_factor,
                width // model.vae_scale_factor, prompt_embeds.dtype, seed)
            if num_channels_unet == 9:
                if masked_image_latents_2b is None:
                    raise ValueError("a 9-channel inpaint UNet needs a pixel-space image (or masked_image_latents)")
                if num_channels_latents + mask.shape[1] + masked_image_latents_2b.shape[1] != num_channels_unet:
                    raise ValueError("Incorrect configuration settings! latents + mask + masked image channels "
                                     f"!= unet in_channels ({num_channels_unet})")
            elif num_channels_unet != 4:
                raise ValueError(f"The unet {model.base.__class__} should have either 4 or 9 input channels, "
                                 f"not {num_channels_unet}.")
            height, width = (d * model.vae_scale_factor for d in latents.shape[-2:])
            self.is_inpaint = True
        else:
            timesteps, num_inference_steps = self.get_timesteps(num_inference_steps, strength, denoising_start)
            latent_timestep = timesteps[:1].repeat(batch_size * num_images_per_prompt)
            add_noise = denoising_start is None
            latents = self.prepare_latents_img2img(image, latent_timestep, batch_size, num_images_per_prompt,
                                                   prompt_embeds.dtype, seed, add_noise)

        if (denoising_end is not None and denoising_start is not None and denoising_value_valid(denoising_end)
                and denoising_value_valid(denoising_start) and denoising_start >= denoising_end):
            raise ValueError(f"`denoising_start`: {denoising_start} cannot be larger than or equal to "
                             f"`denoising_end`:  {denoising_end} when using type float.")
        elif denoising_end is not None and denoising_value_valid(denoising_end):
            cutoff = int(round(model.scheduler.config.num_train_timesteps
                               - denoising_end * model.scheduler.config.num_train_timesteps))
            num_inference_steps = len([ts for ts in timesteps if ts >= cutoff])
            timesteps = timesteps[:num_inference_steps]

        if getattr(model.base.config, "addition_embed_type", None) == "text_time":
            add_text_embeds = pooled_prompt_embeds
            add_time_ids = self._get_add_time_ids((height, width), (0, 0), (height, width), prompt_embeds.dtype)
            add_time_ids = add_time_ids.repeat(batch_size * num_images_per_prompt, 1)
            if self.do_classifier_free_guidance:
                add_text_embeds = torch.cat([negative_pooled_prompt_embeds, add_text_embeds], dim=0)
                add_time_ids = torch.cat([add_time_ids, add_time_ids], dim=0)
            added_cond_kwargs = {"text_embeds": add_text_embeds.to(self.device),
                                 "time_ids": add_time_ids.to(self.device)}
        else:
            added_cond_kwargs = None

        if ip_adapter_image is not None or ip_adapter_image_embeds is not None:
            image_embeds = self.prepare_ip_adapter_image_embeds(ip_adapter_image, ip_adapter_image_embeds, self.device,
                                                                batch_size * num_images_per_prompt,
                                                                self.do_classifier_free_guidance)
            if self.device.type == "cuda":
                image_embeds = [e.to(torch.float16).contiguous() for e in image_embeds]
            added_cond_kwargs = dict(added_cond_kwargs or {}, image_embeds=image_embeds)

        control = None
        if has_cn:
            if num_channels_unet != 4:
                raise ValueError("ControlNet needs a 4-channel UNet (9-channel inpaint UNets are not supported)")
            control = self.prepare_control_image(model, control_image, height, width, batch_size, num_images_per_prompt)

        if self.do_classifier_free_guidance:
            prompt_embeds = torch.cat([negative_prompt_embeds, prompt_embeds], dim=0)
        prompt_embeds = prompt_embeds.to(self.device)

        timesteps_host = [float(v) for v in timesteps.tolist()]
        cn_scales = None
        if control is not None:
            n = len(timesteps_host)
            cn_scales = [float(controlnet_conditioning_scale) *
                         (1.0 - float(i / n < control_guidance_start or (i + 1) / n > control_guidance_end))
                         for i in range(n)]
        kv_cache = getattr(model.base, "text_kv_cache", None)
        if kv_cache is not None:
            if prompt_embeds.device.type == "cuda" and (prompt_embeds.dtype != torch.float16 or not prompt_embeds.is_contiguous()):
                prompt_embeds = prompt_embeds.to(torch.float16).contiguous()
            kv_cache(True)
        fused_step = self._fused_step_available(model, latents, num_channels_unet)
        fused_hist = None
        blend = None
        if fused_step and self.is_inpaint:
            f16 = lambda x: x.to(device=latents.device, dtype=torch.float16).contiguous()
            m1 = mask.chunk(2)[0] if self.do_classifier_free_guidance else mask
            blend = (f16(image_latents), f16(noise), f16(m1.expand(latents.shape[0], 1, *latents.shape[2:])))
        try:
            for i, t in enumerate(timesteps_host):
                cn_kwargs = {} if control is None else dict(controlnet_cond=control,
                                                            controlnet_conditioning_scale=cn_scales[i])
                if fused_step:
                    latents, fused_hist = self._fused_cfg_iteration(model, latents, fused_hist, t, prompt_embeds,
                                                                    cross_attention_kwargs, added_cond_kwargs,
                                                                    guidance_scale, guidance_rescale=guidance_rescale,
                                                                    **cn_kwargs)
                    if blend is not None:
                        last = i == len(timesteps_host) - 1
                        a, b = (1.0, 0.0) if last else model.scheduler.add_noise_coefficients(timesteps_host[i + 1])
                        self._device_inpaint_blend(model, latents, blend, a, b, with_noise=not last)
                    continue
                latent_model_input = torch.cat([latents] * 2) if self.do_classifier_free_guidance else latents
                latent_model_input = model.scheduler.scale_model_input(latent_model_input, t)
                if self.is_inpaint and num_channels_unet == 9:
                    latent_model_input = torch.cat([latent_model_input, mask.to(latent_model_input.dtype),
                                                    masked_image_latents_2b.to(latent_model_input.dtype)], dim=1)
                noise_pred = model.base(latent_model_input, t, prompt_embeds,
                                        cross_attention_kwargs=cross_attention_kwargs,
                                        added_cond_kwargs=added_cond_kwargs, return_dict=False, **cn_kwargs)[0]
                if self.do_classifier_free_guidance:
                    noise_pred_uncond, noise_pred_text = noise_pred.chunk(2)
                    noise_pred = guidance_scale * (noise_pred_text - noise_pred_uncond) + noise_pred_uncond
                    if guidance_rescale > 0.0:
                        noise_pred = rescale_noise_cfg(noise_pred, noise_pred_text, guidance_rescale)
                latents = model.scheduler.step(noise_pred, t, latents, return_dict=False)[0]
                if self.is_inpaint and num_channels_unet == 4:
                    init_latents_proper = image_latents
                    init_mask = mask.chunk(2)[0] if self.do_classifier_free_guidance else mask
                    if i < len(timesteps_host) - 1:
                        init_latents_proper = model.scheduler.add_noise(init_latents_proper, noise,
                                                                        torch.as_tensor([timesteps_host[i + 1]]))
                    latents = ((1 - init_mask) * init_latents_proper.float() + init_mask * latents.float()).to(latents.dtype)

        finally:
            if kv_cache is not None:
                kv_cache(False)

        if self.output_type == "pt":
            cfg = model.vae.config
            mean = getattr(cfg, "latents_mean", None)
            std = getattr(cfg, "latents_std", None)
            if mean is not None and std is not None:
                m = torch.tensor(mean).view(1, -1, 1, 1).to(latents.device, latents.dtype)
                s = torch.tensor(std).view(1, -1, 1, 1).to(latents.device, latents.dtype)
                latents = latents * s / cfg.scaling_factor + m
            else:
                latents = latents / cfg.scaling_factor
            images = model.vae.decode(latents, return_dict=False)[0]
        elif self.output_type == "latents":
            images = latents
        else:
            raise ValueError(f"Unknown output_type = '{self.output_type}'")
        return images

    def _device_inpaint_blend(self, model, latents, blend, a, b, with_noise):
        import ctypes as C
        lib = model.base._lib
        img, noise, m = blend
        B, Cc, H, W = latents.shape
        rc = lib.sd_inpaint_blend(C.c_void_p(latents.data_ptr()), C.c_void_p(img.data_ptr()),
                                  C.c_void_p(noise.data_ptr()) if with_noise else None, C.c_void_p(m.data_ptr()),
                                  float(a), float(b), B, Cc, H, W, C.c_void_p(torch.cuda.current_stream().cuda_stream))
        if rc:
            raise RuntimeError(lib.sd_last_error().decode())

    def _fused_step_available(self, model, latents, num_channels_unet=4) -> bool:
        return (self.do_classifier_free_guidance and (not self.is_inpaint or num_channels_unet == 4)
                and hasattr(model.scheduler, "fused_plan") and getattr(model.scheduler, "supports_fused", True)
                and hasattr(model.scheduler, "add_noise_coefficients")
                and hasattr(model.base, "_lib") and latents.is_cuda and latents.dtype == torch.float16)

    def _fused_cfg_iteration(self, model, latents, hist, t, prompt_embeds, cross_attention_kwargs, added_cond_kwargs,
                             guidance_scale, guidance_rescale=0.0, **unet_kwargs):
        import ctypes as C
        lib = model.base._lib
        plan = model.scheduler.fused_plan(t)
        latents = latents.contiguous()
        B = latents.shape[0]
        st = C.c_void_p(torch.cuda.current_stream().cuda_stream)
        lat2 = torch.empty((2 * B,) + tuple(latents.shape[1:]), device=latents.device, dtype=latents.dtype)
        rc = lib.sd_cfg_duplicate(C.c_void_p(latents.data_ptr()), C.c_void_p(lat2.data_ptr()),
                                  latents[0].numel(), B, plan.in_scale, st)
        if rc:
            raise RuntimeError(lib.sd_last_error().decode())
        noise_pred = model.base(lat2, t, prompt_embeds, cross_attention_kwargs=cross_attention_kwargs,
                                added_cond_kwargs=added_cond_kwargs, return_dict=False, **unet_kwargs)[0]
        if plan.use_hist and hist is None:
            hist = torch.zeros(latents.shape, device=latents.device, dtype=torch.float32)
        out = latents.clone()
        hist_p = C.c_void_p(hist.data_ptr()) if plan.use_hist else None
        if guidance_rescale > 0.0:
            rc = lib.sd_cfg_rescale_linear_step(C.c_void_p(noise_pred.data_ptr()), C.c_void_p(out.data_ptr()), hist_p, B,
                                                out[0].numel(), float(guidance_scale), float(guidance_rescale), plan.c_x,
                                                plan.c_eps, plan.c_hist, plan.h_x, plan.h_eps, None, st)
        else:
            rc = lib.sd_cfg_linear_step(C.c_void_p(noise_pred.data_ptr()), C.c_void_p(out.data_ptr()), hist_p, out.numel(),
                                        float(guidance_scale), plan.c_x, plan.c_eps, plan.c_hist, plan.h_x, plan.h_eps, st)
        if rc:
            raise RuntimeError(lib.sd_last_error().decode())
        model.scheduler.fused_commit()
        return out, hist

    @staticmethod
    def control_image_processor(model):
        return VaeImageProcessor(vae_scale_factor=model.vae_scale_factor, do_convert_rgb=True, do_normalize=False)

    def prepare_control_image(self, model, image, height, width, batch_size, num_images_per_prompt):
        if isinstance(image, (list, tuple)) and image and isinstance(image[0], (list, tuple)):
            raise NotImplementedError("MultiControlNet (a list of control-image lists) is not supported")
        img = self.control_image_processor(model).preprocess(image, height=height, width=width).to(torch.float32)
        if img.shape[1] != 3:
            raise ValueError(f"control_image must have 3 channels, got {img.shape[1]}")
        repeat_by = batch_size * num_images_per_prompt if img.shape[0] == 1 else num_images_per_prompt
        img = img.repeat_interleave(repeat_by, dim=0)
        if img.shape[0] != batch_size * num_images_per_prompt:
            raise ValueError(f"control_image batch {img.shape[0] // repeat_by} does not match the prompt batch {batch_size}")
        img = img.to(self.device)
        if img.is_cuda:
            img = img.to(torch.float16).contiguous()
        return img

    def encode_image(self, image, device, num_images_per_prompt):
        m = self.model
        if m.image_encoder is None:
            raise ValueError("ip_adapter_image needs model.image_encoder (or pass ip_adapter_image_embeds)")
        p = next(iter(m.image_encoder.parameters()), None)
        enc_device = p.device if p is not None else torch.device("cpu")
        dtype = p.dtype if p is not None else torch.float32
        if not isinstance(image, torch.Tensor):
            if m.feature_extractor is None:
                raise ValueError("ip_adapter_image needs model.feature_extractor for non-tensor images")
            image = m.feature_extractor(image, return_tensors="pt").pixel_values
        image = image.to(device=enc_device, dtype=dtype)
        image_embeds = m.image_encoder(image).image_embeds
        image_embeds = image_embeds.repeat_interleave(num_images_per_prompt, dim=0)
        return image_embeds.to(device), torch.zeros_like(image_embeds).to(device)

    def prepare_ip_adapter_image_embeds(self, ip_adapter_image, ip_adapter_image_embeds, device, num_images_per_prompt,
                                        do_classifier_free_guidance):
        if ip_adapter_image_embeds is None:
            if isinstance(ip_adapter_image, list) and len(ip_adapter_image) == 1:
                ip_adapter_image = ip_adapter_image[0]
            pos, neg = self.encode_image(ip_adapter_image, device, 1)
            pos = torch.stack([pos] * num_images_per_prompt, dim=0)
            neg = torch.stack([neg] * num_images_per_prompt, dim=0)
            return [torch.cat([neg, pos]).to(device) if do_classifier_free_guidance else pos.to(device)]
        if isinstance(ip_adapter_image_embeds, torch.Tensor):
            ip_adapter_image_embeds = [ip_adapter_image_embeds]
        if len(ip_adapter_image_embeds) != 1:
            raise ValueError(f"one IP-Adapter is supported, got image embeds for {len(ip_adapter_image_embeds)}")
        e = ip_adapter_image_embeds[0]
        if e.ndim != 3:
            raise ValueError(f"ip_adapter_image_embeds: expected [batch, n_img, D_img], got {tuple(e.shape)}")
        halves = e.chunk(2) if do_classifier_free_guidance else (e,)
        rows = halves[0].shape[0]
        if rows == num_images_per_prompt:
            return [e.to(device)]
        if num_images_per_prompt % rows != 0 or any(h.shape[0] != rows for h in halves):
            raise ValueError(f"ip_adapter_image_embeds: {rows} rows per half do not divide the batch {num_images_per_prompt}")
        rep = num_images_per_prompt // rows
        return [torch.cat([h.repeat(rep, 1, 1) for h in halves]).to(device)]

    def encode_prompt(self, prompt, prompt_2=None, negative_prompt=None, negative_prompt_2=None,
                      num_images_per_prompt=1, lora_scale=None, clip_skip=None):
        m = self.model
        if m.tokenizer is None or m.text_encoder is None:
            raise ValueError("model has no tokenizer / text_encoder: pass prompt_embeds instead")
        sdxl = hasattr(m, "text_encoder_2") and hasattr(m, "tokenizer_2")
        prompt = [prompt] if isinstance(prompt, str) else prompt
        batch_size = len(prompt)
        toks, encs, prompts = [m.tokenizer], [m.text_encoder], [prompt]
        if sdxl:
            prompt_2 = prompt_2 or prompt
            prompt_2 = [prompt_2] if isinstance(prompt_2, str) else prompt_2
            toks, encs, prompts = [m.tokenizer, m.tokenizer_2], [m.text_encoder, m.text_encoder_2], [prompt, prompt_2]

        def run(texts_list):
            embeds, pooled = [], None
            for texts, tok, enc in zip(texts_list, toks, encs):
                ids = tok(texts, padding="max_length", max_length=tok.model_max_length, truncation=True,
                          return_tensors="pt").input_ids.to(self.device)
                out = enc(ids, output_hidden_states=True)
                pooled = out[0]
                if clip_skip is None:
                    e = out.hidden_states[-2] if sdxl else out[0]
                else:
                    final_ln = getattr(enc, "text_model", enc).final_layer_norm
                    e = (out.hidden_states[-(clip_skip + 2)] if sdxl
                         else final_ln(out.hidden_states[-(clip_skip + 1)]))
                embeds.append(e)
            return torch.concat(embeds, dim=-1), pooled

        prompt_embeds, pooled = run(prompts)
        neg_embeds = neg_pooled = None
        if self.do_classifier_free_guidance:
            negative_prompt = negative_prompt or ""
            negative_prompt_2 = negative_prompt_2 or negative_prompt
            negative_prompt = batch_size * [negative_prompt] if isinstance(negative_prompt, str) else negative_prompt
            negative_prompt_2 = (batch_size * [negative_prompt_2] if isinstance(negative_prompt_2, str)
                                 else negative_prompt_2)
            if batch_size != len(negative_prompt):
                raise ValueError("`negative_prompt` batch size does not match `prompt`")
            neg_embeds, neg_pooled = run([negative_prompt, negative_prompt_2])
        dt = m.base.dtype
        bs, seq, _ = prompt_embeds.shape
        prompt_embeds = prompt_embeds.to(dtype=dt, device=self.device).repeat(1, num_images_per_prompt, 1)
        prompt_embeds = prompt_embeds.view(bs * num_images_per_prompt, seq, -1)
        if neg_embeds is not None:
            neg_embeds = neg_embeds.to(dtype=dt, device=self.device).repeat(1, num_images_per_prompt, 1)
            neg_embeds = neg_embeds.view(batch_size * num_images_per_prompt, seq, -1)
        if sdxl:
            pooled = pooled.repeat(1, num_images_per_prompt).view(bs * num_images_per_prompt, -1)
            if neg_pooled is not None:
                neg_pooled = neg_pooled.repeat(1, num_images_per_prompt).view(bs * num_images_per_prompt, -1)
        return prompt_embeds, neg_embeds, pooled, neg_pooled

    def get_timesteps(self, num_inference_steps, strength, denoising_start=None):
        sch = self.model.scheduler
        if denoising_start is None:
            init_timestep = min(int(num_inference_steps * strength), num_inference_steps)
            t_start = max(num_inference_steps - init_timestep, 0)
        else:
            t_start = 0
        timesteps = sch.timesteps[t_start * sch.order:]
        if denoising_start is not None:
            cutoff = int(round(sch.config.num_train_timesteps - denoising_start * sch.config.num_train_timesteps))
            n = int((timesteps < cutoff).sum().item())
            if sch.order == 2 and n % 2 == 0:
                n += 1
            return timesteps[-n:], n
        return timesteps, num_inference_steps - t_start

    def prepare_latents_txt2img(self, shape, dtype, seed=None, latents=None):
        generator = None
        if seed is not None:
            generator = torch.Generator(device=self.device).manual_seed(int(seed))
        if latents is None:
            latents = torch.randn(shape, generator=generator, device=self.device, dtype=dtype)
        else:
# ... 93 lines not shown
```

Baseline: 7.690 latents/s.

## Share unconditional/conditional UNet compute until first cross-attention in CFG

Adds a forward_cfg path that runs the UNet on only the B unique latents instead of the duplicated 2B batch. It stays at half batch through conv_in, the first down resnet(s), the time embedding and the first transformer's self-attention. Just before the first cross-attention, a multi-segment row_dup kernel copies the live activations (q, residuals, skip tensors) into the second half of the batch. This removes the redundant first-stage work at the highest resolution, at the cost of extra duplicate copies, and it only applies when graphs, ControlNet and SDXL text-time conditioning are all off.

```diff
diff --git a/include/sd_engine.h b/include/sd_engine.h
--- a/include/sd_engine.h
+++ b/include/sd_engine.h
@@ -92,6 +92,10 @@
                        const void* add_text, const float* add_time_ids, const void* image_embeds, int n_img,
                        const void* control_image, int n_ctrl, float cond_scale, void* out, int B, int H, int W,
                        void* stream);
+int sd_unet_forward_cfg(sd_unet* u, const void* latents, const float* timesteps, const void* ehs, int ehs_len,
+                        const void* add_text, const float* add_time_ids, const void* image_embeds, int n_img,
+                        float in_scale, int share, void* out, int B, int H, int W, void* stream);
+int sd_unet_cfg_share(const sd_unet_config* cfg);
 int sd_unet_memory(const sd_unet* u, int64_t* weight_bytes, int64_t* workspace_bytes);
 
 int sd_ip_adapter_create(const sd_unet* u, int image_embed_dim, int num_tokens, sd_ip_adapter** out);
diff --git a/stablediffusion_amd/_lib.py b/stablediffusion_amd/_lib.py
--- a/stablediffusion_amd/_lib.py
+++ b/stablediffusion_amd/_lib.py
@@ -88,6 +88,8 @@
     "sd_unet_text_kv_cache": (_I, [_P, _I]),
     "sd_unet_memory": (_I, [_P, C.POINTER(_I64), C.POINTER(_I64)]),
     "sd_unet_forward_ex": (_I, [_P, _P, _P, _P, _I, _P, _P, _P, _I, _P, _I, _I, _I, _P]),
+    "sd_unet_forward_cfg": (_I, [_P, _P, _P, _P, _I, _P, _P, _P, _I, _F, _I, _P, _I, _I, _I, _P]),
+    "sd_unet_cfg_share": (_I, [C.POINTER(SdUNetConfig)]),
     "sd_unet_set_ip_adapter": (_I, [_P, _P]),
     "sd_unet_set_ip_adapter_scale": (_I, [_P, _F]),
     "sd_ip_adapter_create": (_I, [_P, _I, _I, C.POINTER(_P)]),
diff --git a/stablediffusion_amd/csrc/capi.cpp b/stablediffusion_amd/csrc/capi.cpp
--- a/stablediffusion_amd/csrc/capi.cpp
+++ b/stablediffusion_amd/csrc/capi.cpp
@@ -178,6 +178,17 @@
                            static_cast<const half_t*>(image_embeds), image_embeds ? n_img : 0,
                            static_cast<const half_t*>(control_image), control_image ? n_ctrl : 0, cond_scale);
 }
+int sd_unet_forward_cfg(sd_unet* u, const void* latents, const float* timesteps, const void* ehs, int ehs_len,
+                        const void* add_text, const float* add_time_ids, const void* image_embeds, int n_img,
+                        float in_scale, int share, void* out, int B, int H, int W, void* stream) {
+    if (!u || !latents || !timesteps || !ehs || !out) { set_error("null argument"); return SD_ERR_INVALID; }
+    if (!(in_scale == in_scale)) { set_error("sd_unet_forward_cfg: in_scale is NaN"); return SD_ERR_INVALID; }
+    return u->impl.forward_cfg(static_cast<const half_t*>(latents), timesteps, static_cast<const half_t*>(ehs), ehs_len,
+                               static_cast<const half_t*>(add_text), add_time_ids,
+                               static_cast<const half_t*>(image_embeds), image_embeds ? n_img : 0, in_scale, share != 0,
+                               static_cast<half_t*>(out), B, H, W, static_cast<hipStream_t>(stream));
+}
+int sd_unet_cfg_share(const sd_unet_config* cfg) { return cfg && sd::unet_cfg_share_eligible(*cfg) ? 1 : 0; }
 int sd_unet_set_ip_adapter_scale(sd_unet* u, float scale) {
     if (!u) { set_error("null handle"); return SD_ERR_INVALID; }
     if (!(scale == scale)) { set_error("sd_unet_set_ip_adapter_scale: NaN"); return SD_ERR_INVALID; }
diff --git a/stablediffusion_amd/csrc/kernels.h b/stablediffusion_amd/csrc/kernels.h
--- a/stablediffusion_amd/csrc/kernels.h
+++ b/stablediffusion_amd/csrc/kernels.h
@@ -184,6 +184,15 @@
 int launch_pack_conv(const half_t* w_oihw, half_t* wp, int O, int I, int KH, int KW, long Kpad,
                      hipStream_t s);
 int launch_cfg_duplicate(const half_t* lat, half_t* out, long n_total, float scale, hipStream_t s);
+constexpr int kRowDupMax = 8;
+struct RowDupSeg {
+    const void* src = nullptr;
+    void* dst = nullptr;
+    long ld_bytes = 0, row_bytes = 0, rows = 0;
+};
+int launch_row_dup(const RowDupSeg* segs, int count, hipStream_t s);
+int launch_scale_copy_f16(const half_t* x, half_t* out, long n, float scale, hipStream_t s);
+int launch_dup_f32(const float* x, float* out, long n, hipStream_t s);
 int launch_clip_embed(const int* ids, const half_t* tok, const half_t* pos, half_t* out, int B, int T, int H, int vocab,
                       hipStream_t s);
 int launch_gather_rows(const half_t* x, long ldx, const int* idx, half_t* out16, float* out32, int B, int T, int H,
diff --git a/stablediffusion_amd/csrc/misc.hip b/stablediffusion_amd/csrc/misc.hip
--- a/stablediffusion_amd/csrc/misc.hip
+++ b/stablediffusion_amd/csrc/misc.hip
@@ -180,6 +180,49 @@
     const long i = (long)blockIdx.x * blockDim.x + threadIdx.x;
     if (i >= n) return;
     const half_t v = (half_t)((float)lat[i] * scale);
+    out[i] = v;
+    out[n + i] = v;
+}
+constexpr int RD_PER_THREAD = 4;
+constexpr int RD_UNITS = 256 * RD_PER_THREAD;
+struct RowDupDev {
+    const uint4* src[kRowDupMax];
+    uint4* dst[kRowDupMax];
+    long ld16[kRowDupMax], w16[kRowDupMax], units[kRowDupMax];
+    int first[kRowDupMax + 1];
+    int count;
+};
+__global__ __launch_bounds__(256) void row_dup_kernel(RowDupDev p) {
+    int sg = 0;
+    while (sg + 1 < p.count && (int)blockIdx.x >= p.first[sg + 1]) ++sg;
+    const uint4* __restrict__ src = p.src[sg];
+    uint4* __restrict__ dst = p.dst[sg];
+    const long ld = p.ld16[sg], w = p.w16[sg], n = p.units[sg];
+    const long base = (long)((int)blockIdx.x - p.first[sg]) * RD_UNITS + threadIdx.x;
+    uint4 v[RD_PER_THREAD];
+    long off[RD_PER_THREAD];
+#pragma unroll
+    for (int j = 0; j < RD_PER_THREAD; ++j) {
+        const long i = base + j * 256;
+        off[j] = -1;
+        if (i < n) {
+            const long r = i / w;
+            off[j] = r * ld + (i - r * w);
+            v[j] = src[off[j]];
+        }
+    }
+#pragma unroll
+    for (int j = 0; j < RD_PER_THREAD; ++j)
+        if (off[j] >= 0) dst[off[j]] = v[j];
+}
+__global__ void scale_copy_f16_kernel(const half_t* __restrict__ lat, half_t* __restrict__ out, long n, float scale) {
+    const long i = (long)blockIdx.x * blockDim.x + threadIdx.x;
+    if (i < n) out[i] = (half_t)((float)lat[i] * scale);
+}
+__global__ void dup_f32_kernel(const float* __restrict__ x, float* __restrict__ out, long n) {
+    const long i = (long)blockIdx.x * blockDim.x + threadIdx.x;
+    if (i >= n) return;
+    const float v = x[i];
     out[i] = v;
     out[n + i] = v;
 }
@@ -667,6 +710,48 @@
 }
 int launch_cfg_duplicate(const half_t* lat, half_t* out, long n, float scale, hipStream_t s) {
     hipLaunchKernelGGL(cfg_duplicate_kernel, grid1d(n), dim3(256), 0, s, lat, out, n, scale);
+    SD_HIP_CHECK(hipGetLastError());
+    return 0;
+}
+int launch_row_dup(const RowDupSeg* segs, int count, hipStream_t s) {
+    if (count < 0 || count > kRowDupMax) { set_error("row_dup: too many segments"); return 1; }
+    RowDupDev p;
+    int blocks = 0, k = 0;
+    for (int i = 0; i < count; ++i) {
+        const RowDupSeg& g = segs[i];
+        if (g.rows <= 0 || g.row_bytes <= 0) continue;
+        if (((reinterpret_cast<uintptr_t>(g.src) | reinterpret_cast<uintptr_t>(g.dst) | (uintptr_t)g.ld_bytes |
+              (uintptr_t)g.row_bytes) & 15) != 0 || g.row_bytes > g.ld_bytes) {
+            set_error("row_dup: segments must be 16-byte aligned with row_bytes <= ld_bytes");
+            return 1;
+        }
+        p.src[k] = static_cast<const uint4*>(g.src);
+        p.dst[k] = static_cast<uint4*>(g.dst);
+        p.ld16[k] = g.ld_bytes / 16;
+        p.w16[k] = g.row_bytes / 16;
+        p.units[k] = g.rows * p.w16[k];
+        p.first[k] = blocks;
+        const long nb = (p.units[k] + RD_UNITS - 1) / RD_UNITS;
+        if (nb + blocks > 0x7fffffffL) { set_error("row_dup: too large"); return 1; }
+        blocks += (int)nb;
+        ++k;
+    }
+    if (k == 0) return 0;
+    p.first[k] = blocks;
+    p.count = k;
+    hipLaunchKernelGGL(row_dup_kernel, dim3((unsigned)blocks), dim3(256), 0, s, p);
+    SD_HIP_CHECK(hipGetLastError());
+    return 0;
+}
+int launch_scale_copy_f16(const half_t* x, half_t* out, long n, float scale, hipStream_t s) {
+    if (n <= 0) return 0;
+    hipLaunchKernelGGL(scale_copy_f16_kernel, grid1d(n), dim3(256), 0, s, x, out, n, scale);
+    SD_HIP_CHECK(hipGetLastError());
+    return 0;
+}
+int launch_dup_f32(const float* x, float* out, long n, hipStream_t s) {
+    if (n <= 0) return 0;
+    hipLaunchKernelGGL(dup_f32_kernel, grid1d(n), dim3(256), 0, s, x, out, n);
     SD_HIP_CHECK(hipGetLastError());
     return 0;
 }
diff --git a/stablediffusion_amd/csrc/model.h b/stablediffusion_amd/csrc/model.h
--- a/stablediffusion_amd/csrc/model.h
+++ b/stablediffusion_amd/csrc/model.h
@@ -34,12 +34,16 @@
     int C = 0;
 };
 
+struct CfgShare {
+    std::vector<RowDupSeg> segs;
+};
+
 void run_resnet(Ctx& c, const Resnet& r, View x, int N, int H, int W, View out, int G, float eps,
                 const float* tproj, int tproj_ld, const GnStatBuf* x_stats = nullptr, GnStatBuf** out_stats = nullptr,
                 float stream_scale = 1.f, GnStatBuf* out_buf = nullptr, int out_groups = 0);
 void run_xformer(Ctx& c, const Xformer& t, View x, int N, int H, int W, View out, int G, View text_kv, int L,
                  const GnStatBuf* x_stats = nullptr, GnStatBuf** out_stats = nullptr, GnStatBuf* out_buf = nullptr,
-                 int out_groups = 0);
+                 int out_groups = 0, const CfgShare* share = nullptr);
 
 struct UNet;
 
@@ -85,11 +89,12 @@
     int pack_encoder(std::vector<std::string>* tw, std::vector<std::string>* tb);
     int pack_resnet(const std::string& p, Resnet* r, std::vector<std::string>* tw, std::vector<std::string>* tb);
     int pack_xformer(const std::string& p, Xformer* x, int heads, int depth);
-    int run_temb(Ctx& c, const float* timesteps, const half_t* add_text, const float* add_time_ids, int B, float** tproj);
+    int run_temb(Ctx& c, const float* timesteps, const half_t* add_text, const float* add_time_ids, int B, float** tproj,
+                 int rows_alloc = 0);
     void run_conv_in(Ctx& c, const half_t* sample, int B, int H, int W, View y0, GnStatBuf* gb, const View* res,
                      GnStatBuf** xs);
     View run_down(Ctx& c, View x, GnStatBuf*& xs, int B, int& h, int& w, View text_kv, int L, const float* tproj,
-                  const SkipDst& dst, const SkipStat& stat);
+                  const SkipDst& dst, const SkipStat& stat, const CfgShare* share = nullptr);
     void run_mid(Ctx& c, View x, GnStatBuf* xs, int B, int h, int w, View text_kv, int L, const float* tproj, View dst);
 };
 
@@ -114,13 +119,26 @@
             const float* add_time_ids, int B, int H, int W, View emb, const std::vector<View>& sites, View mid);
 };
 
+bool unet_cfg_share_eligible(const sd_unet_config& cfg);
+
+struct CfgIn {
+    const half_t* latents = nullptr;
+    float in_scale = 1.f;
+};
+
 struct UNet : Encoder {
     explicit UNet(const sd_unet_config& c);
     int finalize();
+    int forward_cfg(const half_t* latents, const float* timesteps, const half_t* ehs, int L, const half_t* add_text,
+                    const float* add_time_ids, const half_t* image_embeds, int n_img, float in_scale, bool share,
+                    half_t* out, int B, int H, int W, hipStream_t stream);
+    bool cfg_share_active(bool share) const;
+    char* cfg_slab = nullptr;
+    size_t cfg_cap = 0;
     int forward(const half_t* sample, const float* timesteps, const half_t* ehs, int L,
                 const half_t* add_text, const float* add_time_ids, half_t* out, int B, int H, int W,
                 hipStream_t stream, const half_t* image_embeds = nullptr, int n_img = 0,
-                const half_t* control = nullptr, int n_ctrl = 0, float cn_scale = 0.f);
+                const half_t* control = nullptr, int n_ctrl = 0, float cn_scale = 0.f, const CfgIn* cfg_in = nullptr);
     void set_ip_adapter(IPAdapter* a);
     void set_controlnet(ControlNet* n);
 
@@ -175,7 +193,7 @@
     int run(Ctx& c, const half_t* sample, const float* timesteps, const half_t* ehs, int L,
             const half_t* add_text, const float* add_time_ids, half_t* out, int B, int H, int W,
             const half_t* image_embeds = nullptr, int n_img = 0, const half_t* control = nullptr, int n_ctrl = 0,
-            float cn_scale = 0.f);
+            float cn_scale = 0.f, const CfgIn* cfg_in = nullptr);
     int run_controlnet(Ctx& c, const half_t* sample, const float* timesteps, const half_t* ehs, int L,
                        const half_t* add_text, const float* add_time_ids, int B, int H, int W, const half_t* control,
                        int n_ctrl, const std::vector<View>& sites, View mid);
diff --git a/stablediffusion_amd/csrc/unet.cpp b/stablediffusion_amd/csrc/unet.cpp
--- a/stablediffusion_amd/csrc/unet.cpp
+++ b/stablediffusion_amd/csrc/unet.cpp
@@ -364,7 +364,7 @@
 }
 
 void run_xformer(Ctx& c, const Xformer& t, View x, int N, int H, int W, View out, int G, View text_kv, int L,
-                 const GnStatBuf* x_stats, GnStatBuf** out_stats, GnStatBuf* out_buf, int out_groups) {
+                 const GnStatBuf* x_stats, GnStatBuf** out_stats, GnStatBuf* out_buf, int out_groups, const CfgShare* share) {
     Arena& a = *c.arena;
     const size_t mk = a.mark();
     const int C = t.C;
@@ -372,8 +372,10 @@
     const long M = (long)N * T;
     const int d = C / t.heads;
     const bool fold = !t.blocks.empty() && t.blocks[0].fold;
+    int Np = share ? N / 2 : N;
+    long Mp = (long)Np * T;
     View hn(a.alloc_h(M * C), C, C);
-    op_groupnorm(c, t.gn, x, hn, N, T, G, 1e-6f, 0, x_stats);
+    op_groupnorm(c, t.gn, x, hn, Np, T, G, 1e-6f, 0, x_stats);
     View cur(a.alloc_h(M * C), C, C), nxt(a.alloc_h(M * C), C, C);
     RowStat st_cur, st_t2, st_t3;
     if (fold) {
@@ -385,7 +387,7 @@
     f_cur.stat_out = &st_cur; f_t2.stat_out = &st_t2; f_t3.stat_out = &st_t3;
     f_ln1.ln_in = &st_cur; f_ln2.ln_in = &st_t2; f_ln3.ln_in = &st_t3;
     f_ln1.ln_eps = f_ln2.ln_eps = f_ln3.ln_eps = 1e-5f;
-    op_conv(c, t.pin, hn, N, H, W, cur, 1, 0, nullptr, 0, nullptr, 0, -1, 0, fold ? &f_cur : nullptr);
+    op_conv(c, t.pin, hn, Np, H, W, cur, 1, 0, nullptr, 0, nullptr, 0, -1, 0, fold ? &f_cur : nullptr);
     for (size_t bi = 0; bi < t.blocks.size(); ++bi) {
         const TBlock& b = t.blocks[bi];
         const bool more = bi + 1 < t.blocks.size();
@@ -393,21 +395,38 @@
         View n(fold ? nullptr : a.alloc_h(M * C), C, C);
         View qkv(a.alloc_h(M * 3 * C), 3 * C, 3 * C);
         if (fold) {
-            op_conv(c, b.qkv, cur, N, H, W, qkv, 1, 0, nullptr, 0, nullptr, 0, -1, 0, &f_ln1);
+            op_conv(c, b.qkv, cur, Np, H, W, qkv, 1, 0, nullptr, 0, nullptr, 0, -1, 0, &f_ln1);
         } else {
-            op_layernorm(c, b.ln1, cur, n, M, 1e-5f);
-            op_conv(c, b.qkv, n, N, H, W, qkv);
+            op_layernorm(c, b.ln1, cur, n, Mp, 1e-5f);
+            op_conv(c, b.qkv, n, Np, H, W, qkv);
         }
         View att(a.alloc_h(M * C), C, C);
-        op_attention(c, qkv.slice(0, C), qkv.slice(C, C), qkv.slice(2 * C, C), att, N, T, T, t.heads, d, 0, 1);
+        op_attention(c, qkv.slice(0, C), qkv.slice(C, C), qkv.slice(2 * C, C), att, Np, T, T, t.heads, d, 0, 1);
         View t2(a.alloc_h(M * C), C, C);
-        op_conv(c, b.out1, att, N, H, W, t2, 1, 0, nullptr, 0, &cur, 0, -1, 0, fold ? &f_t2 : nullptr);
+        op_conv(c, b.out1, att, Np, H, W, t2, 1, 0, nullptr, 0, &cur, 0, -1, 0, fold ? &f_t2 : nullptr);
         View q(a.alloc_h(M * C), C, C);
         if (fold) {
-            op_conv(c, b.q2, t2, N, H, W, q, 1, 0, nullptr, 0, nullptr, 0, -1, 0, &f_ln2);
+            op_conv(c, b.q2, t2, Np, H, W, q, 1, 0, nullptr, 0, nullptr, 0, -1, 0, &f_ln2);
         } else {
-            op_layernorm(c, b.ln2, t2, n, M, 1e-5f);
-            op_conv(c, b.q2, n, N, H, W, q);
+            op_layernorm(c, b.ln2, t2, n, Mp, 1e-5f);
+            op_conv(c, b.q2, n, Np, H, W, q);
+        }
+        if (Np != N) {
+            std::vector<RowDupSeg> segs = share->segs;
+            for (const View& v : {q, t2, x}) {
+                RowDupSeg g;
+                g.src = v.p; g.dst = v.p + Mp * v.ld;
+                g.ld_bytes = v.ld * 2; g.row_bytes = (long)v.C * 2; g.rows = Mp;
+                segs.push_back(g);
+            }
+            if (!c.dry && !c.err) {
+                double bytes = 0;
+                for (const RowDupSeg& g : segs) bytes += 2.0 * g.rows * g.row_bytes;
+                prof_open(c.stream, "row_dup_kernel", 0.0, bytes);
+                c.err = launch_row_dup(segs.data(), (int)segs.size(), c.stream);
+                prof_close(c.stream);
+            }
+            Np = N; Mp = M;
         }
         if (c.ip_kv.p && c.ip_scale != 0.f)
             op_ip_attention(c, q, text_kv.slice(b.kv_off, C), text_kv.slice(b.kv_off + C, C), c.ip_kv.slice(b.ip_kv_off, C),
@@ -438,7 +457,7 @@
 }
 
 int Encoder::run_temb(Ctx& c, const float* timesteps, const half_t* add_text, const float* add_time_ids, int B,
-                      float** tproj_out) {
+                      float** tproj_out, int rows_alloc) {
     Arena& a = *c.arena;
     const int* boc = cfg.block_out_channels;
     const int temb = boc[0] * 4;
@@ -447,7 +466,7 @@
     float* sinus = a.alloc_f((long)B * boc[0]);
     float* e1 = a.alloc_f((long)B * temb);
     float* emb = a.alloc_f((long)B * temb);
-    float* tproj = a.alloc_f((long)B * temb_total);
+    float* tproj = a.alloc_f((long)std::max(B, rows_alloc) * temb_total);
     *tproj_out = tproj;
     if (go && !c.err) c.err = launch_timestep_sinusoid(timesteps, 1, sinus, B, boc[0], cfg.flip_sin_to_cos, cfg.freq_shift, boc[0], s);
     if (go && !c.err) c.err = launch_small_linear(sinus, boc[0], te1.w, te1.bias, e1, temb, B, boc[0], temb, 0, 1, s);
@@ -520,7 +539,7 @@
 }
 
 View Encoder::run_down(Ctx& c, View x, GnStatBuf*& xs, int B, int& h, int& w, View text_kv, int L, const float* tproj,
-                       const SkipDst& skip_view, const SkipStat& skip_stat) {
+                       const SkipDst& skip_view, const SkipStat& skip_stat, const CfgShare* share) {
     Arena& a = *c.arena;
     const int nb = cfg.num_blocks;
     const int G = cfg.norm_num_groups;
@@ -533,9 +552,11 @@
                 const size_t mk = a.mark();
                 View tmp(a.alloc_h((long)B * h * w * r.cout), r.cout, r.cout);
                 GnStatBuf* rs = nullptr;
-                run_resnet(c, r, x, B, h, w, tmp, G, eps, tproj, temb_total, xs, &rs);
+                const CfgShare* sh = (i == 0 && j == 0) ? share : nullptr;
+                run_resnet(c, r, x, sh ? B / 2 : B, h, w, tmp, G, eps, tproj, temb_total, xs, &rs);
                 View dst = skip_view(skip_i);
-                run_xformer(c, down_att[i][j], tmp, B, h, w, dst, G, text_kv, L, rs, &xs, skip_stat(skip_i, (long)h * w, r.cout));
+                run_xformer(c, down_att[i][j], tmp, B, h, w, dst, G, text_kv, L, rs, &xs, skip_stat(skip_i, (long)h * w, r.cout),
+                            0, sh);
                 a.release(mk);
                 x = dst;
             } else {
@@ -580,7 +601,7 @@
 
 int UNet::run(Ctx& c, const half_t* sample, const float* timesteps, const half_t* ehs, int L,
               const half_t* add_text, const float* add_time_ids, half_t* out, int B, int H, int W,
-              const half_t* image_embeds, int n_img, const half_t* control, int n_ctrl, float cn_scale) {
+              const half_t* image_embeds, int n_img, const half_t* control, int n_ctrl, float cn_scale, const CfgIn* cfg_in) {
     Arena& a = *c.arena;
     const int nb = cfg.num_blocks;
     const int* boc = cfg.block_out_channels;
@@ -589,8 +610,26 @@
     hipStream_t s = c.stream;
     const bool go = !c.dry;
 
+    const int Bp = cfg_in ? B / 2 : B;
+    CfgShare share;
+    if (cfg_in) {
+        const long n = (long)Bp * cfg.in_channels * H * W;
+        half_t* scaled = a.alloc_h(n);
+        sample = cfg_in->latents;
+        if (cfg_in->in_scale != 1.f) {
+            if (go && !c.err) c.err = launch_scale_copy_f16(cfg_in->latents, scaled, n, cfg_in->in_scale, s);
+            sample = scaled;
+        }
+    }
+
     float* tproj = nullptr;
-    if (int rc = run_temb(c, timesteps, add_text, add_time_ids, B, &tproj)) return rc;
+    if (int rc = run_temb(c, timesteps, add_text, add_time_ids, Bp, &tproj, B)) return rc;
+    if (cfg_in) {
+        RowDupSeg g;
+        g.src = tproj; g.dst = tproj + (long)Bp * temb_total;
+        g.ld_bytes = g.row_bytes = (long)Bp * temb_total * 4; g.rows = 1;
+        share.segs.push_back(g);
+    }
 
     const bool kv_cached = kv_cache_on && !graph_enabled && kv_cache != nullptr;
     View text_kv(kv_cached ? kv_cache : a.alloc_h((long)B * L * kv_total), kv_total, kv_total);
@@ -668,7 +707,7 @@
         return (sst[(size_t)si].buf && gn_wants_stats(HWs, C, G)) ? &sst[(size_t)si] : nullptr;
     };
 
-    const bool use_cn = cn && control && cn_scale != 0.f;
+    const bool use_cn = cn && control && cn_scale != 0.f && !cfg_in;
     const size_t cn_mark = a.mark();
     std::vector<View> cn_sites;
     std::vector<int> cn_rows;
@@ -696,11 +735,17 @@
     }
 
     int h = H, w = W;
-    run_conv_in(c, sample, B, H, W, skip_view(skip_i), skip_stat(skip_i, (long)H * W, boc[0]), nullptr, &xs);
+    run_conv_in(c, sample, Bp, H, W, skip_view(skip_i), skip_stat(skip_i, (long)H * W, boc[0]), nullptr, &xs);
     View x = skip_view(skip_i++);
+    if (cfg_in) {
+        RowDupSeg g;
+        g.src = x.p; g.dst = x.p + (long)Bp * H * W * x.ld;
+        g.ld_bytes = x.ld * 2; g.row_bytes = (long)x.C * 2; g.rows = (long)Bp * H * W;
+        share.segs.push_back(g);
+    }
 
     x = run_down(c, x, xs, B, h, w, text_kv, L, tproj, [&](int si) { return skip_view(si); },
-                 [&](int si, long HWs, int C) { return skip_stat(si, HWs, C); });
+                 [&](int si, long HWs, int C) { return skip_stat(si, HWs, C); }, cfg_in ? &share : nullptr);
 
     run_mid(c, x, xs, B, h, w, text_kv, L, tproj, View(cats[0].p, cats[0].c1 + cats[0].c2, cats[0].c1));
 
@@ -838,6 +883,7 @@
     if (ipkv_cache) (void)hipFree(ipkv_cache);
     if (cond_cache) (void)hipFree(cond_cache);
     if (cnkv_cache) (void)hipFree(cnkv_cache);
+    if (cfg_slab) (void)hipFree(cfg_slab);
     if (ip) ip->attached = nullptr;
     if (cn) cn->attached = nullptr;
 }
@@ -912,8 +958,12 @@
 
 int UNet::forward(const half_t* sample, const float* timesteps, const half_t* ehs, int L, const half_t* add_text,
                   const float* add_time_ids, half_t* out, int B, int H, int W, hipStream_t stream,
-                  const half_t* image_embeds, int n_img, const half_t* control, int n_ctrl, float cn_scale) {
+                  const half_t* image_embeds, int n_img, const half_t* control, int n_ctrl, float cn_scale, const CfgIn* cfg_in) {
     if (!finalized) { set_error("unet: forward before finalize"); return 2; }
+    if (cfg_in && (B % 2 != 0 || graph_enabled || control || !unet_cfg_share_eligible(cfg))) {
+        set_error("unet: shared CFG prefix not available for this call");
+        return 2;
+    }
     const int div = 1 << (cfg.num_blocks - 1);
     if (B <= 0 || H % div != 0 || W % div != 0) { set_error("unet: H and W must be divisible by 2^(blocks-1)"); return 1; }
     if (ip && !image_embeds) { set_error("unet: an IP-Adapter is attached: image_embeds required"); return 1; }
@@ -977,13 +1027,13 @@
         }
     }
     const long key = ((long)B << 40) ^ ((long)H << 20) ^ (long)W ^ ((long)L << 52) ^ (kv_cache_on ? (1L << 62) : 0) ^
-                     (ip ? (long)(n_img * ip->n_tok) << 32 : 0);
+                     (ip ? (long)(n_img * ip->n_tok) << 32 : 0) ^ (cfg_in ? (1L << 61) : 0);
     const long cn_key = use_cn ? n_ctrl : 0;
     if (key != planned_key || cn_key != planned_cn) {
         Ctx dry{&arena, stream, true};
         arena.begin(true);
         int rc = run(dry, sample, timesteps, ehs, L, add_text, add_time_ids, out, B, H, W, image_embeds, n_img, control,
-                     n_ctrl, cn_scale);
+                     n_ctrl, cn_scale, cfg_in);
         if (rc) return rc;
         if (arena.peak() > arena.capacity()) {
             SD_HIP_CHECK(hipDeviceSynchronize());
@@ -996,9 +1046,48 @@
     Ctx ctx{&arena, stream, false};
     arena.begin(false);
     int rc = run(ctx, sample, timesteps, ehs, L, add_text, add_time_ids, out, B, H, W, image_embeds, n_img, control, n_ctrl,
-                 cn_scale);
+                 cn_scale, cfg_in);
     if (!rc && arena.overflow()) { set_error("unet: workspace overflow (planner bug)"); return 2; }
     return rc;
 }
 
-}
+bool unet_cfg_share_eligible(const sd_unet_config& cfg) {
+    return cfg.addition_time_embed_dim == 0 && cfg.num_blocks >= 1 && cfg.down_block_has_attn[0] != 0 &&
+           cfg.transformer_layers[0] >= 1;
+}
+
+bool UNet::cfg_share_active(bool share) const {
+    static const bool off = getenv("SD_NO_CFG_SHARE") != nullptr;
+    static const bool gn_cat = getenv("SD_GN_CAT") != nullptr;
+    return share && !off && !gn_cat && !graph_enabled && !cn && unet_cfg_share_eligible(cfg);
+}
+
+int UNet::forward_cfg(const half_t* latents, const float* timesteps, const half_t* ehs, int L, const half_t* add_text,
+                      const float* add_time_ids, const half_t* image_embeds, int n_img, float in_scale, bool share,
+                      half_t* out, int B, int H, int W, hipStream_t stream) {
+    if (!finalized) { set_error("unet: forward before finalize"); return 2; }
+    if (B <= 0 || H <= 0 || W <= 0) { set_error("unet: forward_cfg: empty batch"); return 1; }
+    if (cfg_share_active(share)) {
+        CfgIn in;
+        in.latents = latents;
+        in.in_scale = in_scale;
+        return forward(nullptr, timesteps, ehs, L, add_text, add_time_ids, out, 2 * B, H, W, stream, image_embeds, n_img,
+                       nullptr, 0, 0.f, &in);
+    }
+    const size_t n = (size_t)B * cfg.in_channels * H * W;
+    const size_t lat_bytes = (2 * n * sizeof(half_t) + 255) & ~size_t(255), need = lat_bytes + 2 * (size_t)B * sizeof(float);
+    if (need > cfg_cap) {
+        SD_HIP_CHECK(hipDeviceSynchronize());
+        if (cfg_slab) (void)hipFree(cfg_slab);
+        cfg_slab = nullptr; cfg_cap = 0;
+        SD_HIP_CHECK(hipMalloc(reinterpret_cast<void**>(&cfg_slab), need));
+        cfg_cap = need;
+    }
+    half_t* lat2 = reinterpret_cast<half_t*>(cfg_slab);
+    float* ts2 = reinterpret_cast<float*>(cfg_slab + lat_bytes);
+    if (int rc = launch_cfg_duplicate(latents, lat2, (long)n, in_scale, stream)) return rc;
+    if (int rc = launch_dup_f32(timesteps, ts2, B, stream)) return rc;
+    return forward(lat2, ts2, ehs, L, add_text, add_time_ids, out, 2 * B, H, W, stream, image_embeds, n_img);
+}
+
+}
diff --git a/stablediffusion_amd/models.py b/stablediffusion_amd/models.py
--- a/stablediffusion_amd/models.py
+++ b/stablediffusion_amd/models.py
@@ -280,6 +280,52 @@
 
     forward = __call__
 
+    @property
+    def cfg_share_eligible(self) -> bool:
+        c = _unet_config_struct(self.cfg)
+        return bool(self._lib.sd_unet_cfg_share(C.byref(c)))
+
+    def forward_cfg(self, latents, timestep, encoder_hidden_states, added_cond_kwargs=None, in_scale: float = 1.0,
+                    share: bool = True):
+        if not self._finalized:
+            raise _lib.EngineError("weights not loaded")
+        if self._cn is not None:
+            raise ValueError("forward_cfg takes no ControlNet: duplicate the latents and call the model")
+        dev = self.device
+        latents = _as_f16(latents, dev)
+        B, _, H, W = latents.shape
+        ehs = _as_f16(encoder_hidden_states, dev)
+        if ehs.shape[0] != 2 * B:
+            raise ValueError(f"encoder_hidden_states batch {ehs.shape[0]} != 2 x latents batch {B}")
+        if ehs.shape[2] != self.cfg.cross_attention_dim:
+            raise ValueError("encoder_hidden_states width != cross_attention_dim")
+        if isinstance(timestep, (int, float)):
+            t = torch.full((B,), float(timestep), device=dev, dtype=torch.float32)
+        else:
+            t = torch.as_tensor(timestep, device=dev).to(torch.float32).reshape(-1)
+            if t.numel() not in (1, B):
+                raise ValueError(f"timestep: expected a scalar or {B} values (one per latent), got {t.numel()}")
+            t = t.expand(B).contiguous() if t.numel() == 1 else t.contiguous()
+        pt = pi = None
+        if self.cfg.addition_embed_type == "text_time":
+            if not added_cond_kwargs or "text_embeds" not in added_cond_kwargs or "time_ids" not in added_cond_kwargs:
+                raise ValueError("added_cond_kwargs needs text_embeds and time_ids for text_time conditioning")
+            add_text = _as_f16(added_cond_kwargs["text_embeds"], dev)
+            add_ids = added_cond_kwargs["time_ids"].to(device=dev, dtype=torch.float32).contiguous()
+            if add_text.shape[0] != 2 * B or add_ids.shape[0] != 2 * B:
+                raise ValueError("text_embeds / time_ids must hold 2 x latents batch rows")
+            pt, pi = C.c_void_p(add_text.data_ptr()), C.c_void_p(add_ids.data_ptr())
+        img = self._image_embeds(added_cond_kwargs, 2 * B, dev)
+        out = torch.empty((2 * B, self.cfg.out_channels, H, W), device=dev, dtype=torch.float16)
+        with torch.cuda.device(dev):
+            rc = self._lib.sd_unet_forward_cfg(self._h, C.c_void_p(latents.data_ptr()), C.c_void_p(t.data_ptr()),
+                                               C.c_void_p(ehs.data_ptr()), ehs.shape[1], pt, pi,
+                                               C.c_void_p(img.data_ptr()) if img is not None else None,
+                                               img.shape[1] if img is not None else 0, float(in_scale), int(bool(share)),
+                                               C.c_void_p(out.data_ptr()), B, H, W, C.c_void_p(_stream_ptr()))
+        _lib.check(rc, "sd_unet_forward_cfg")
+        return (out,)
+
     def set_adapters(self, *a, **k):
         raise NotImplementedError("fuse LoRA weights on load (stablediffusion_amd.weights.fuse_lora)")
 
diff --git a/stablediffusion_amd/pipeline.py b/stablediffusion_amd/pipeline.py
--- a/stablediffusion_amd/pipeline.py
+++ b/stablediffusion_amd/pipeline.py
@@ -229,6 +229,7 @@
         self.device = torch.device(device) if device is not None else torch.device("cpu")
         self.output_type = output_type if output_type is not None else "pt"
         self.model: Optional[SDModelWrapper] = None
+        self.cfg_share = True
 
     @torch.no_grad()
     def __call__(
@@ -525,13 +526,17 @@
         latents = latents.contiguous()
         B = latents.shape[0]
         st = C.c_void_p(torch.cuda.current_stream().cuda_stream)
-        lat2 = torch.empty((2 * B,) + tuple(latents.shape[1:]), device=latents.device, dtype=latents.dtype)
-        rc = lib.sd_cfg_duplicate(C.c_void_p(latents.data_ptr()), C.c_void_p(lat2.data_ptr()),
-                                  latents[0].numel(), B, plan.in_scale, st)
-        if rc:
-            raise RuntimeError(lib.sd_last_error().decode())
-        noise_pred = model.base(lat2, t, prompt_embeds, cross_attention_kwargs=cross_attention_kwargs,
-                                added_cond_kwargs=added_cond_kwargs, return_dict=False, **unet_kwargs)[0]
+        if not unet_kwargs and hasattr(model.base, "forward_cfg") and getattr(model.base, "controlnet", None) is None:
+            noise_pred = model.base.forward_cfg(latents, t, prompt_embeds, added_cond_kwargs=added_cond_kwargs,
+                                                in_scale=plan.in_scale, share=self.cfg_share)[0]
+        else:
+            lat2 = torch.empty((2 * B,) + tuple(latents.shape[1:]), device=latents.device, dtype=latents.dtype)
+            rc = lib.sd_cfg_duplicate(C.c_void_p(latents.data_ptr()), C.c_void_p(lat2.data_ptr()),
+                                      latents[0].numel(), B, plan.in_scale, st)
+            if rc:
+                raise RuntimeError(lib.sd_last_error().decode())
+            noise_pred = model.base(lat2, t, prompt_embeds, cross_attention_kwargs=cross_attention_kwargs,
+                                    added_cond_kwargs=added_cond_kwargs, return_dict=False, **unet_kwargs)[0]
         if plan.use_hist and hist is None:
             hist = torch.zeros(latents.shape, device=latents.device, dtype=torch.float32)
         out = latents.clone()
```

Measured after the change: 7.820 latents/s (median of 6 runs). 1.7% higher.
